# pdeljanov/Symphonia

Hardware: AMD Instinct MI355X
Metric: decoded audio frames/sec (batch IMDCT+OLA) (higher is better)
Workload: dtype f32

## Files before the change

### bindings/rust/symaccel_sys.rs

```rust
#![allow(non_camel_case_types, dead_code)]

#[repr(C)]
pub struct SymaccelCtx {
    _private: [u8; 0],
}

#[repr(C)]
pub struct SymaccelBatcher {
    _private: [u8; 0],
}

pub const SYMACCEL_OK: i32 = 0;
pub const SYMACCEL_ERR_INVALID_ARG: i32 = -1;
pub const SYMACCEL_ERR_UNSUPPORTED: i32 = -2;
pub const SYMACCEL_ERR_DEVICE: i32 = -3;
pub const SYMACCEL_ERR_OOM: i32 = -4;
pub const SYMACCEL_ERR_DECODE: i32 = -5;
pub const SYMACCEL_TABLE_AAC_KBD_LONG: u32 = 0;
pub const SYMACCEL_TABLE_AAC_KBD_SHORT: u32 = 1;
pub const SYMACCEL_TABLE_AAC_SINE_LONG: u32 = 2;
pub const SYMACCEL_TABLE_AAC_SINE_SHORT: u32 = 3;
pub const SYMACCEL_TABLE_MP3_SYNTH_D: u32 = 4;
pub const SYMACCEL_TABLE_MP3_IMDCT_WIN: u32 = 5;
pub const SYMACCEL_TABLE_VORBIS_FLOOR1_DB: u32 = 6;
// ... 334 lines not shown
    pub fn symaccel_vorbis_synth_fr_device(ctx: *mut SymaccelCtx, bs0_exp: i32, bs1_exp: i32, d_floor: *const f32, d_residue: *const f32, spec_stride: usize, d_block_flag: *const u8, d_prev_flag_io: *mut i32, d_overlap_io: *mut f32, d_pcm: *mut f32, pcm_stride: usize, n_chains: usize, blocks_per_chain: usize) -> i32;
    pub fn symaccel_vorbis_synth(ctx: *mut SymaccelCtx, bs0_exp: i32, bs1_exp: i32, h_spectra: *const f32, spec_stride: usize, h_block_flag: *const u8, h_prev_flag_io: *mut i32, h_overlap_io: *mut f32, h_pcm: *mut f32, pcm_stride: usize, n_chains: usize, blocks_per_chain: usize) -> i32;
    pub fn symaccel_vorbis_synth_pp_device(ctx: *mut SymaccelCtx, bs0_exp: i32, bs1_exp: i32, d_spectra: *const f32, d_residue: *const f32, spec_stride: usize, d_block_flag: *const u8, d_prev_flag_in: *const i32, d_prev_flag_out: *mut i32, d_overlap_in: *const f32, d_overlap_out: *mut f32, d_pcm: *mut f32, pcm_stride: usize, n_chains: usize, blocks_per_chain: usize) -> i32;
    pub fn symaccel_vorbis_synth_fy_pp_device(ctx: *mut SymaccelCtx, bs0_exp: i32, bs1_exp: i32, d_floor_y: *const u8, d_residue: *const f32, spec_stride: usize, d_block_flag: *const u8, d_prev_flag_in: *const i32, d_prev_flag_out: *mut i32, d_overlap_in: *const f32, d_overlap_out: *mut f32, d_pcm: *mut f32, pcm_stride: usize, n_chains: usize, blocks_per_chain: usize) -> i32;
    pub fn symaccel_vorbis_synth_fy_device(ctx: *mut SymaccelCtx, bs0_exp: i32, bs1_exp: i32, d_floor_y: *const u8, d_residue: *const f32, spec_stride: usize, d_block_flag: *const u8, d_prev_flag_io: *mut i32, d_overlap_io: *mut f32, d_pcm: *mut f32, pcm_stride: usize, n_chains: usize, blocks_per_chain: usize) -> i32;
    pub fn symaccel_vorbis_decode(ctx: *mut SymaccelCtx, bs0_exp: i32, bs1_exp: i32, h_residue: *const f32, spec_stride: usize, h_block_flag: *const u8, h_floor: *const u8, h_posts: *const u32, posts_stride: usize, h_floors: *const SymaccelVorbisFloor1Cfg, n_floors: usize, channels_per_stream: usize, h_coupling: *const u8, h_coupling_first: *const u32, h_prev_flag_io: *mut i32, h_overlap_io: *mut f32, h_pcm: *mut f32, pcm_stride: usize, n_chains: usize, blocks_per_chain: usize) -> i32;
    pub fn symaccel_vorbis_inverse_coupling_device(ctx: *mut SymaccelCtx, d_residue: *mut f32, n: usize, mag_index: *const u32, ang_index: *const u32, n_pairs: usize) -> i32;
    pub fn symaccel_vorbis_dot_product_device(ctx: *mut SymaccelCtx, d_floor: *mut f32, d_residue: *const f32, total: usize) -> i32;
    pub fn symaccel_vorbis_deinterleave2_device(ctx: *mut SymaccelCtx, d_type2: *const f32, d_planar: *mut f32, n_ch: i32, n2: usize, count: usize) -> i32;
    pub fn symaccel_vorbis_floor1_device(ctx: *mut SymaccelCtx, x_list: *const u32, n_posts: i32, multiplier: i32, d_y: *const u32, n: u32, d_floor: *mut f32, count: usize) -> i32;
    pub fn symaccel_vorbis_floor1_dot_device(ctx: *mut SymaccelCtx, x_list: *const u32, n_posts: i32, multiplier: i32, d_y: *const u32, n: u32, d_residue: *const f32, d_spectrum: *mut f32, count: usize) -> i32;
    pub fn symaccel_vorbis_floor1_dot_at_device(ctx: *mut SymaccelCtx, x_list: *const u32, n_posts: i32, multiplier: i32, d_y: *const u32, n: u32, d_line_offsets: *const u32, d_residue: *const f32, d_spectrum: *mut f32, count: usize) -> i32;
    pub fn symaccel_vorbis_floor1_y_device(ctx: *mut SymaccelCtx, x_list: *const u32, n_posts: i32, multiplier: i32, d_y: *const u32, n: u32, d_line_offsets: *const u32, d_floor_y: *mut u8, count: usize) -> i32;
    pub fn symaccel_vorbis_floor1_y_jobs_device(ctx: *mut SymaccelCtx, jobs: *const SymaccelVorbisFloor1Job, n_jobs: usize, d_floor_y: *mut u8) -> i32;
    pub fn symaccel_vorbis_floor1_status_device(ctx: *mut SymaccelCtx, n_posts: i32, d_y: *const u32, count: usize, d_status: *mut i8) -> i32;
    pub fn symaccel_host_vorbis_bark_map(n: u32, floor0_rate: u16, floor0_bark_map_size: u16, h_map: *mut i32) -> i32;
    pub fn symaccel_host_vorbis_floor0_coeffs(h_coeffs: *mut f32, order: i32) -> i32;
    pub fn symaccel_host_vorbis_floor0(h_coeffs: *const f32, order: i32, h_map: *const i32, n: u32, floor0_bark_map_size: u16, amplitude_bits: u8, amplitude_offset: u8, amplitude: u64, h_floor: *mut f32) -> i32;
    pub fn symaccel_flac_restore_device(ctx: *mut SymaccelCtx, d_buf: *mut i32, d_desc: *const SymaccelFlacDesc, d_coeffs: *const i32, n_blocks: usize, blocksize: usize) -> i32;
    pub fn symaccel_flac_restore(ctx: *mut SymaccelCtx, h_buf: *mut i32, h_desc: *const SymaccelFlacDesc, h_coeffs: *const i32, n_blocks: usize, blocksize: usize) -> i32;
    pub fn symaccel_flac_restore_pipelined(ctx: *mut SymaccelCtx, h_buf: *mut i32, h_desc: *const SymaccelFlacDesc, h_coeffs: *const i32, n_blocks: usize, blocksize: usize, chunk_blocks: usize) -> i32;
    pub fn symaccel_flac_block_status_device(ctx: *mut SymaccelCtx, d_desc: *const SymaccelFlacDesc, n_blocks: usize, blocksize: usize, d_status: *mut i8) -> i32;
    pub fn symaccel_flac_restore_stereo_device(ctx: *mut SymaccelCtx, d_buf: *mut i32, d_desc: *const SymaccelFlacDesc, d_coeffs: *const i32, d_pair_mode: *const u8, out_shift: u32, n_blocks: usize, blocksize: usize) -> i32;
    pub fn symaccel_flac_restore_strided_device(ctx: *mut SymaccelCtx, d_buf: *mut i32, d_desc: *const SymaccelFlacDesc, d_coeffs: *const i32, d_pair_mode: *const u8, out_shift: u32, n_blocks: usize, blocksize: usize, stride: usize) -> i32;
    pub fn symaccel_row_stride(blocksize: usize) -> usize;
    pub fn symaccel_flac_decorrelate_device(ctx: *mut SymaccelCtx, d_mode: *const u8, d_ch0: *mut i32, d_ch1: *mut i32, n_pairs: usize, blocksize: usize, out_shift: u32) -> i32;
    pub fn symaccel_flac_decorrelate(ctx: *mut SymaccelCtx, h_mode: *const u8, h_ch0: *mut i32, h_ch1: *mut i32, n_pairs: usize, blocksize: usize, out_shift: u32) -> i32;
    pub fn symaccel_md5_init(state: *mut SymaccelMd5State) -> i32;
    pub fn symaccel_md5_update(state: *mut SymaccelMd5State, bytes: *const core::ffi::c_void, n: usize) -> i32;
    pub fn symaccel_md5_digest(state: *const SymaccelMd5State, digest: *mut u8) -> i32;
    pub fn symaccel_flac_md5_device(ctx: *mut SymaccelCtx, d_jobs: *const SymaccelFlacMd5Job, n_jobs: usize) -> i32;
    pub fn symaccel_flac_md5_finish_device(ctx: *mut SymaccelCtx, d_jobs: *const SymaccelFlacMd5Job, n_jobs: usize, out_shift: u32) -> i32;
    pub fn symaccel_flac_md5(ctx: *mut SymaccelCtx, h_rows: *const i32, row_pitch: usize, h_frames: *const SymaccelFlacMd5Frame, n_frames: usize, nch: i32, bytes_per_sample: i32, h_state_io: *mut SymaccelMd5State, h_checkpoints: *mut SymaccelMd5State) -> i32;
    pub fn symaccel_alac_predict_device(ctx: *mut SymaccelCtx, d_buf: *mut i32, d_desc: *const SymaccelAlacDesc, d_coeffs: *const i32, n_blocks: usize, blocksize: usize) -> i32;
    pub fn symaccel_alac_predict(ctx: *mut SymaccelCtx, h_buf: *mut i32, h_desc: *const SymaccelAlacDesc, h_coeffs: *const i32, n_blocks: usize, blocksize: usize) -> i32;
    pub fn symaccel_alac_block_status_device(ctx: *mut SymaccelCtx, d_desc: *const SymaccelAlacDesc, n_blocks: usize, d_status: *mut i8) -> i32;
    pub fn symaccel_alac_predict_stereo_device(ctx: *mut SymaccelCtx, d_buf: *mut i32, d_desc: *const SymaccelAlacDesc, d_coeffs: *const i32, d_pair_weight: *const i32, d_pair_shift: *const u8, n_blocks: usize, blocksize: usize) -> i32;
    pub fn symaccel_alac_predict_strided_device(ctx: *mut SymaccelCtx, d_buf: *mut i32, d_desc: *const SymaccelAlacDesc, d_coeffs: *const i32, d_pair_weight: *const i32, d_pair_shift: *const u8, n_blocks: usize, blocksize: usize, stride: usize) -> i32;
    pub fn symaccel_alac_mid_side_device(ctx: *mut SymaccelCtx, d_weight: *const i32, d_shift: *const u8, d_ch0: *mut i32, d_ch1: *mut i32, n_pairs: usize, blocksize: usize) -> i32;
    pub fn symaccel_alac_mid_side(ctx: *mut SymaccelCtx, h_weight: *const i32, h_shift: *const u8, h_ch0: *mut i32, h_ch1: *mut i32, n_pairs: usize, blocksize: usize) -> i32;
    pub fn symaccel_sample_bytes(fmt: i32) -> usize;
    pub fn symaccel_pcm_convert_device(ctx: *mut SymaccelCtx, d_src: *const core::ffi::c_void, src_fmt: i32, plane_stride: usize, n_groups: usize, channels: usize, n_frames: usize, d_dst: *mut core::ffi::c_void, dst_fmt: i32, dst_group_bytes: usize) -> i32;
    pub fn symaccel_pcm_convert(ctx: *mut SymaccelCtx, h_src: *const core::ffi::c_void, src_fmt: i32, plane_stride: usize, n_groups: usize, channels: usize, n_frames: usize, h_dst: *mut core::ffi::c_void, dst_fmt: i32, dst_group_bytes: usize) -> i32;
    pub fn symaccel_adpcm_block_bytes(codec: i32, channels: usize, frames_per_block: usize) -> usize;
    pub fn symaccel_adpcm_decode_device(ctx: *mut SymaccelCtx, d_bytes: *const core::ffi::c_void, block_pitch: usize, n_blocks: usize, codec: i32, channels: usize, frames_per_block: usize, d_pcm: *mut core::ffi::c_void, out_fmt: i32, d_status: *mut u8) -> i32;
    pub fn symaccel_adpcm_decode(ctx: *mut SymaccelCtx, h_bytes: *const core::ffi::c_void, block_pitch: usize, n_blocks: usize, codec: i32, channels: usize, frames_per_block: usize, h_pcm: *mut core::ffi::c_void, out_fmt: i32, h_status: *mut u8) -> i32;
    pub fn symaccel_pcm_coded_bytes(codec: i32) -> usize;
    pub fn symaccel_pcm_native_bytes(codec: i32) -> usize;
    pub fn symaccel_pcm_decode_device(ctx: *mut SymaccelCtx, d_bytes: *const core::ffi::c_void, packet_pitch: usize, n_packets: usize, codec: i32, channels: usize, shift: u32, frames: usize, d_pcm: *mut core::ffi::c_void, out_fmt: i32) -> i32;
    pub fn symaccel_pcm_decode(ctx: *mut SymaccelCtx, h_bytes: *const core::ffi::c_void, packet_pitch: usize, n_packets: usize, codec: i32, channels: usize, shift: u32, frames: usize, h_pcm: *mut core::ffi::c_void, out_fmt: i32) -> i32;
    pub fn symaccel_batcher_create(ctx: *mut SymaccelCtx, flush_bytes: usize, out: *mut *mut SymaccelBatcher) -> i32;
    pub fn symaccel_batcher_destroy(b: *mut SymaccelBatcher) -> i32;
    pub fn symaccel_batcher_configure(b: *mut SymaccelBatcher, lanes: i32, hint_bytes: usize) -> i32;
    pub fn symaccel_batcher_last_error(b: *mut SymaccelBatcher, buf: *mut core::ffi::c_char, capacity: usize) -> i32;
    pub fn symaccel_batcher_reserve(b: *mut SymaccelBatcher, kind: i32, param: i32, n_chains: usize, units_per_chain: usize, slot: *mut SymaccelBatchSlot, ticket: *mut u64) -> i32;
    pub fn symaccel_batcher_commit(b: *mut SymaccelBatcher, ticket: u64) -> i32;
    pub fn symaccel_batcher_wait(b: *mut SymaccelBatcher, ticket: u64, slot: *mut SymaccelBatchSlot) -> i32;
    pub fn symaccel_batcher_release(b: *mut SymaccelBatcher, ticket: u64) -> i32;
    pub fn symaccel_batcher_submit(b: *mut SymaccelBatcher, kind: i32, param: i32, n_chains: usize, units_per_chain: usize, input: *mut *const core::ffi::c_void, state_io: *mut *mut core::ffi::c_void, out: *mut core::ffi::c_void, ticket: *mut u64) -> i32;
    pub fn symaccel_batcher_reserve_fmt(b: *mut SymaccelBatcher, kind: i32, param: i32, n_chains: usize, units_per_chain: usize, out_fmt: i32, channels: i32, slot: *mut SymaccelBatchSlot, ticket: *mut u64) -> i32;
    pub fn symaccel_batcher_submit_fmt(b: *mut SymaccelBatcher, kind: i32, param: i32, n_chains: usize, units_per_chain: usize, input: *mut *const core::ffi::c_void, state_io: *mut *mut core::ffi::c_void, out: *mut core::ffi::c_void, out_fmt: i32, channels: i32, ticket: *mut u64) -> i32;
    pub fn symaccel_batcher_reserve_io(b: *mut SymaccelBatcher, kind: i32, param: i32, n_chains: usize, units_per_chain: usize, in_fmt: i32, out_fmt: i32, channels: i32, slot: *mut SymaccelBatchSlot, ticket: *mut u64) -> i32;
    pub fn symaccel_batcher_submit_io(b: *mut SymaccelBatcher, kind: i32, param: i32, n_chains: usize, units_per_chain: usize, input: *mut *const core::ffi::c_void, state_io: *mut *mut core::ffi::c_void, out: *mut core::ffi::c_void, in_fmt: i32, out_fmt: i32, channels: i32, ticket: *mut u64) -> i32;
    pub fn symaccel_host_narrow_s16(src: *const i32, dst: *mut i16, n: usize) -> i32;
    pub fn symaccel_host_pack_row(src: *const i32, dst: *mut core::ffi::c_void, n: usize) -> i32;
    pub fn symaccel_batcher_submit_aac_synth(b: *mut SymaccelBatcher, coeffs: *const f32, side: *const u8, delay_io: *mut f32, pcm: *mut f32, n_chains: usize, frames_per_chain: usize, ticket: *mut u64) -> i32;
    pub fn symaccel_batcher_submit_mp3_synth(b: *mut SymaccelBatcher, xr: *const f32, side: *const SymaccelMp3Side, sample_rate_idx: i32, overlap_io: *mut f32, vvec_io: *mut f32, vfront_io: *mut i32, pcm: *mut f32, n_chains: usize, granules_per_chain: usize, ticket: *mut u64) -> i32;
    pub fn symaccel_batcher_submit_mp3_decode(b: *mut SymaccelBatcher, quant: *const i16, rq_desc: *const SymaccelMp3Requant, st_desc: *const SymaccelMp3Stereo, side: *const SymaccelMp3Side, sample_rate_idx: i32, overlap_io: *mut f32, vvec_io: *mut f32, vfront_io: *mut i32, pcm: *mut f32, n_chains: usize, granules_per_chain: usize, ticket: *mut u64) -> i32;
    pub fn symaccel_batcher_aac_bands(b: *mut SymaccelBatcher, swb_long: *const u16, n_swb_long: i32, swb_short: *const u16, n_swb_short: i32, bands: *mut i32) -> i32;
    pub fn symaccel_batcher_submit_aac_decode(b: *mut SymaccelBatcher, bands: i32, coeffs: *const f32, side: *const u8, pair_chains: *const i32, js_desc: *const SymaccelAacJsFrame, n_pairs: usize, tns: *const SymaccelAacTnsFilter, n_tns: usize, delay_io: *mut f32, pcm: *mut f32, n_chains: usize, frames_per_chain: usize, ticket: *mut u64) -> i32;
    pub fn symaccel_batcher_submit_vorbis_synth(b: *mut SymaccelBatcher, bs0_exp: i32, bs1_exp: i32, spectra: *const f32, block_flag: *const u8, prev_flag_io: *mut i32, overlap_io: *mut f32, pcm: *mut f32, n_chains: usize, blocks_per_chain: usize, ticket: *mut u64) -> i32;
    pub fn symaccel_batcher_vorbis_floor(b: *mut SymaccelBatcher, cfg: *const SymaccelVorbisFloor1Cfg, index: *mut i32) -> i32;
    pub fn symaccel_batcher_submit_vorbis_decode(b: *mut SymaccelBatcher, bs0_exp: i32, bs1_exp: i32, residue: *const f32, block_flag: *const u8, floor: *const u8, posts: *const u32, coupling: *const u8, coupling_first: *const u32, prev_flag_io: *mut i32, overlap_io: *mut f32, pcm: *mut f32, n_chains: usize, blocks_per_chain: usize, ticket: *mut u64) -> i32;
    pub fn symaccel_batcher_submit_flac_restore(b: *mut SymaccelBatcher, buf_io: *mut i32, desc: *const SymaccelFlacDesc, coeffs: *const i32, pair_mode: *const u8, out_shift: u32, n_blocks: usize, blocksize: usize, ticket: *mut u64) -> i32;
    pub fn symaccel_batcher_submit_flac_verify(b: *mut SymaccelBatcher, buf_io: *mut i32, desc: *const SymaccelFlacDesc, coeffs: *const i32, frames: *const SymaccelFlacMd5Frame, n_frames: usize, nch: i32, blocksize: usize, finish: i32, out_shift: u32, md5_states_io: *mut SymaccelMd5State, ticket: *mut u64) -> i32;
    pub fn symaccel_batcher_submit_alac_predict(b: *mut SymaccelBatcher, buf_io: *mut i32, desc: *const SymaccelAlacDesc, coeffs: *const i32, pair_weight: *const i32, pair_shift: *const u8, n_blocks: usize, blocksize: usize, ticket: *mut u64) -> i32;
    pub fn symaccel_batcher_submit_adpcm_decode(b: *mut SymaccelBatcher, bytes: *const u8, codec: i32, channels: usize, n_blocks: usize, block_bytes: usize, pcm: *mut i32, ticket: *mut u64) -> i32;
    pub fn symaccel_batcher_submit_pcm_decode(b: *mut SymaccelBatcher, bytes: *const u8, codec: i32, channels: usize, shift: u32, n_packets: usize, frames: usize, pcm: *mut core::ffi::c_void, ticket: *mut u64) -> i32;
    pub fn symaccel_batcher_collect(b: *mut SymaccelBatcher, ticket: u64) -> i32;
    pub fn symaccel_batcher_abandon(b: *mut SymaccelBatcher, ticket: u64) -> i32;
    pub fn symaccel_batcher_flush(b: *mut SymaccelBatcher) -> i32;
    pub fn symaccel_batcher_hint(b: *mut SymaccelBatcher) -> i32;
    pub fn symaccel_batcher_plane_bytes(kind: i32, param: i32, units_per_chain: usize, input_bytes: *mut usize, state_bytes: *mut usize, out_bytes: *mut usize) -> i32;
    pub fn symaccel_batcher_get_stats(b: *mut SymaccelBatcher, out: *mut SymaccelBatcherStats) -> i32;
    pub fn symaccel_shard_range(n_streams: usize, world: i32, rank: i32, first: *mut usize, count: *mut usize) -> i32;
    pub fn symaccel_scatter_streams(ctx: *mut SymaccelCtx, comm: *mut core::ffi::c_void, world: i32, rank: i32, root: i32, d_all: *const core::ffi::c_void, d_mine: *mut core::ffi::c_void, n_streams: usize, bytes_per_stream: usize) -> i32;
    pub fn symaccel_gather_streams(ctx: *mut SymaccelCtx, comm: *mut core::ffi::c_void, world: i32, rank: i32, root: i32, d_mine: *const core::ffi::c_void, d_all: *mut core::ffi::c_void, n_streams: usize, bytes_per_stream: usize) -> i32;
    pub fn symaccel_exchange_pipelined(ctx: *mut SymaccelCtx, comm: *mut core::ffi::c_void, world: i32, rank: i32, root: i32, d_all_in: *const core::ffi::c_void, d_mine_in: *mut core::ffi::c_void, in_bytes_per_stream: usize, d_all_out: *mut core::ffi::c_void, d_mine_out: *mut core::ffi::c_void, out_bytes_per_stream: usize, n_streams: usize, n_chunks: i32, step: SymaccelStepFn, user: *mut core::ffi::c_void) -> i32;
    pub fn symaccel_comm_unique_id(id: *mut SymaccelUniqueId) -> i32;
    pub fn symaccel_comm_init(ctx: *mut SymaccelCtx, id: *const SymaccelUniqueId, world: i32, rank: i32, comm: *mut *mut core::ffi::c_void) -> i32;
    pub fn symaccel_comm_destroy(comm: *mut core::ffi::c_void) -> i32;
    pub fn symaccel_multi_set_transport(transport: *const SymaccelTransport) -> i32;
    pub fn symaccel_probe_copy_device(ctx: *mut SymaccelCtx, d_src: *const core::ffi::c_void, d_dst: *mut core::ffi::c_void, bytes: usize, frames_per_wavefront: u32, flags: u32) -> i32;
    pub fn symaccel_table_f32(ctx: *const SymaccelCtx, table: i32, dst: *mut f32, capacity: usize) -> i32;
    pub fn symaccel_imdct_twiddles(n: i32, scale: f64, dst: *mut f32) -> i32;
    pub fn symaccel_fft_twiddles(n: i32, dst: *mut f32) -> i32;
}
```

### include/symaccel.h

```cpp
#ifndef SYMACCEL_H
#define SYMACCEL_H

#include <stddef.h>
#include <stdint.h>

#ifdef __cplusplus
extern "C" {
#endif

#define SYMACCEL_ABI_VERSION 8

typedef enum symaccel_status {
    SYMACCEL_OK = 0,
    SYMACCEL_ERR_INVALID_ARG = -1,
    SYMACCEL_ERR_UNSUPPORTED = -2,
    SYMACCEL_ERR_DEVICE = -3,
    SYMACCEL_ERR_OOM = -4,
    SYMACCEL_ERR_DECODE = -5,
} symaccel_status;

typedef struct symaccel_ctx symaccel_ctx;

int symaccel_abi_version(void);
const char *symaccel_strerror(int status);
// ... 418 lines not shown
size_t symaccel_pcm_native_bytes(int codec);
int symaccel_pcm_decode_device(symaccel_ctx *ctx, const void *d_bytes, size_t packet_pitch, size_t n_packets, int codec, size_t channels,
                               uint32_t shift, size_t frames, void *d_pcm, int out_fmt);
int symaccel_pcm_decode(symaccel_ctx *ctx, const void *h_bytes, size_t packet_pitch, size_t n_packets, int codec, size_t channels,
                        uint32_t shift, size_t frames, void *h_pcm, int out_fmt);

#define SYMACCEL_BATCH_AAC_SYNTH 1
#define SYMACCEL_BATCH_MP3_SYNTH 2
#define SYMACCEL_BATCH_MP3_DECODE 3
#define SYMACCEL_BATCH_VORBIS_SYNTH 4
#define SYMACCEL_BATCH_AAC_DECODE 5
#define SYMACCEL_BATCH_VORBIS_DECODE 6
#define SYMACCEL_BATCH_FLAC_RESTORE 7
#define SYMACCEL_BATCH_ALAC_PREDICT 8
#define SYMACCEL_BATCH_ADPCM_DECODE 9
#define SYMACCEL_BATCH_MPA12_DECODE 10
#define SYMACCEL_BATCH_PCM_DECODE 11
#define SYMACCEL_BATCH_MAX_INPUTS 6
typedef struct symaccel_batcher symaccel_batcher;
typedef struct symaccel_batch_slot {
    void *input[6];
    void *state[3];
    void *out;
    size_t input_bytes[6];
    size_t state_bytes[3];
    size_t out_bytes;
} symaccel_batch_slot;
typedef struct symaccel_batcher_stats {
    uint64_t submissions;
    uint64_t launches;
    uint64_t chunks;
    uint64_t chains_launched;
    uint64_t max_chains_per_launch;
    uint64_t staging_bytes;
    uint64_t pending;
    uint64_t failed_tickets;
    uint64_t lanes;
    uint64_t mutex_wait_ns;
    uint64_t mutex_contended;
    uint64_t launch_host_ns;
    uint64_t lane_wait_ns;
    uint64_t launch_api_ns;
    uint64_t group_allocs;
    uint64_t flag_wait_ns;
    uint64_t slots_peak;
    uint64_t blocks;
    uint64_t commit_to_launch_ns;
    uint64_t waits, waits_blocked;
    uint64_t launch_to_done_ns, launches_timed;
} symaccel_batcher_stats;
int symaccel_batcher_create(symaccel_ctx *ctx, size_t flush_bytes, symaccel_batcher **out);
int symaccel_batcher_destroy(symaccel_batcher *b);
int symaccel_batcher_configure(symaccel_batcher *b, int lanes, size_t hint_bytes);
int symaccel_batcher_last_error(symaccel_batcher *b, char *buf, size_t capacity);
int symaccel_batcher_reserve(symaccel_batcher *b, int kind, int param, size_t n_chains, size_t units_per_chain,
                             symaccel_batch_slot *slot, uint64_t *ticket);
int symaccel_batcher_commit(symaccel_batcher *b, uint64_t ticket);
int symaccel_batcher_wait(symaccel_batcher *b, uint64_t ticket, symaccel_batch_slot *slot);
int symaccel_batcher_release(symaccel_batcher *b, uint64_t ticket);
int symaccel_batcher_submit(symaccel_batcher *b, int kind, int param, size_t n_chains, size_t units_per_chain,
                            const void **input, void **state_io, void *out, uint64_t *ticket);
int symaccel_batcher_reserve_fmt(symaccel_batcher *b, int kind, int param, size_t n_chains, size_t units_per_chain, int out_fmt,
                                 int channels, symaccel_batch_slot *slot, uint64_t *ticket);
int symaccel_batcher_submit_fmt(symaccel_batcher *b, int kind, int param, size_t n_chains, size_t units_per_chain, const void **input,
                                void **state_io, void *out, int out_fmt, int channels, uint64_t *ticket);
#define SYMACCEL_IN_FMT_ROWS 32
int symaccel_batcher_reserve_io(symaccel_batcher *b, int kind, int param, size_t n_chains, size_t units_per_chain, int in_fmt, int out_fmt,
                                int channels, symaccel_batch_slot *slot, uint64_t *ticket);
int symaccel_batcher_submit_io(symaccel_batcher *b, int kind, int param, size_t n_chains, size_t units_per_chain, const void **input,
                               void **state_io, void *out, int in_fmt, int out_fmt, int channels, uint64_t *ticket);
int symaccel_host_narrow_s16(const int32_t *src, int16_t *dst, size_t n);
int symaccel_host_pack_row(const int32_t *src, void *dst, size_t n);
int symaccel_batcher_submit_aac_synth(symaccel_batcher *b, const float *coeffs, const uint8_t *side, float *delay_io, float *pcm,
                                      size_t n_chains, size_t frames_per_chain, uint64_t *ticket);
int symaccel_batcher_submit_mp3_synth(symaccel_batcher *b, const float *xr, const symaccel_mp3_side *side, int sample_rate_idx,
                                      float *overlap_io, float *vvec_io, int32_t *vfront_io, float *pcm, size_t n_chains,
                                      size_t granules_per_chain, uint64_t *ticket);
int symaccel_batcher_submit_mp3_decode(symaccel_batcher *b, const int16_t *quant, const symaccel_mp3_requant *rq_desc,
                                       const symaccel_mp3_stereo *st_desc, const symaccel_mp3_side *side, int sample_rate_idx,
                                       float *overlap_io, float *vvec_io, int32_t *vfront_io, float *pcm, size_t n_chains,
                                       size_t granules_per_chain, uint64_t *ticket);
int symaccel_batcher_aac_bands(symaccel_batcher *b, const uint16_t *swb_long, int n_swb_long, const uint16_t *swb_short, int n_swb_short,
                               int *bands);
int symaccel_batcher_submit_aac_decode(symaccel_batcher *b, int bands, const float *coeffs, const uint8_t *side,
                                       const int32_t *pair_chains, const symaccel_aac_js_frame *js_desc, size_t n_pairs,
                                       const symaccel_aac_tns_filter *tns, size_t n_tns, float *delay_io, float *pcm, size_t n_chains,
                                       size_t frames_per_chain, uint64_t *ticket);
int symaccel_batcher_submit_vorbis_synth(symaccel_batcher *b, int bs0_exp, int bs1_exp, const float *spectra, const uint8_t *block_flag,
                                         int32_t *prev_flag_io, float *overlap_io, float *pcm, size_t n_chains, size_t blocks_per_chain,
                                         uint64_t *ticket);
int symaccel_batcher_vorbis_floor(symaccel_batcher *b, const symaccel_vorbis_floor1_cfg *cfg, int *index);
int symaccel_batcher_submit_vorbis_decode(symaccel_batcher *b, int bs0_exp, int bs1_exp, const float *residue, const uint8_t *block_flag,
                                          const uint8_t *floor, const uint32_t *posts, const uint8_t *coupling,
                                          const uint32_t *coupling_first, int32_t *prev_flag_io, float *overlap_io, float *pcm,
                                          size_t n_chains, size_t blocks_per_chain, uint64_t *ticket);
int symaccel_batcher_submit_flac_restore(symaccel_batcher *b, int32_t *buf_io, const symaccel_flac_desc *desc, const int32_t *coeffs,
                                         const uint8_t *pair_mode, uint32_t out_shift, size_t n_blocks, size_t blocksize, uint64_t *ticket);
int symaccel_batcher_submit_flac_verify(symaccel_batcher *b, int32_t *buf_io, const symaccel_flac_desc *desc, const int32_t *coeffs,
                                        const symaccel_flac_md5_frame *frames, size_t n_frames, int nch, size_t blocksize, int finish,
                                        uint32_t out_shift, symaccel_md5_state *md5_states_io, uint64_t *ticket);
int symaccel_batcher_submit_alac_predict(symaccel_batcher *b, int32_t *buf_io, const symaccel_alac_desc *desc, const int32_t *coeffs,
                                         const int32_t *pair_weight, const uint8_t *pair_shift, size_t n_blocks, size_t blocksize,
                                         uint64_t *ticket);
int symaccel_batcher_submit_adpcm_decode(symaccel_batcher *b, const uint8_t *bytes, int codec, size_t channels, size_t n_blocks,
                                         size_t block_bytes, int32_t *pcm, uint64_t *ticket);
int symaccel_batcher_submit_pcm_decode(symaccel_batcher *b, const uint8_t *bytes, int codec, size_t channels, uint32_t shift,
// ... 64 lines not shown
```

### symphonia_amd/_ffi.py

```python
import ctypes as C
import json
import os
import sys
from pathlib import Path

import numpy as np

HERE = Path(__file__).resolve().parent
DEFAULT_SO = HERE / "libsymaccel.so"

OK = 0
ERR_INVALID_ARG = -1
ERR_UNSUPPORTED = -2
ERR_DEVICE = -3
ERR_OOM = -4
ERR_DECODE = -5

TABLE_AAC_KBD_LONG, TABLE_AAC_KBD_SHORT, TABLE_AAC_SINE_LONG, TABLE_AAC_SINE_SHORT = 0, 1, 2, 3
TABLE_MP3_SYNTH_D, TABLE_MP3_IMDCT_WIN, TABLE_VORBIS_FLOOR1_DB, TABLE_MP3_CONSTS = 4, 5, 6, 7
TABLE_MP3_POW43, TABLE_MP3_POW2AB, TABLE_MPA12 = 8, 9, 10

FMT_U8, FMT_S8, FMT_U16, FMT_S16, FMT_U24, FMT_S24, FMT_U32, FMT_S32, FMT_F32 = range(1, 10)
IN_FMT_ROWS = 32

ADPCM_MS, ADPCM_IMA_WAV, ADPCM_IMA_QT = 1, 2, 3

PCM_CODEC_NAMES = ("s32le", "s32be", "s24le", "s24be", "s16le", "s16be", "s8", "u32le", "u32be", "u24le", "u24be", "u16le", "u16be", "u8",
                   "f32le", "f32be", "f64le", "f64be", "alaw", "mulaw")
(PCM_S32LE, PCM_S32BE, PCM_S24LE, PCM_S24BE, PCM_S16LE, PCM_S16BE, PCM_S8, PCM_U32LE, PCM_U32BE, PCM_U24LE, PCM_U24BE, PCM_U16LE, PCM_U16BE,
 PCM_U8, PCM_F32LE, PCM_F32BE, PCM_F64LE, PCM_F64BE, PCM_ALAW, PCM_MULAW) = range(1, 21)

ABI_SYMBOLS = [
    "symaccel_abi_version", "symaccel_strerror", "symaccel_last_error", "symaccel_ctx_create",
    "symaccel_ctx_destroy", "symaccel_ctx_set_stream", "symaccel_sync", "symaccel_ctx_set_segment",
    "symaccel_fft_c32_device", "symaccel_fft_c32", "symaccel_ifft_c32_device", "symaccel_ifft_c32", "symaccel_imdct_f32_device", "symaccel_imdct_f32",
    "symaccel_aac_synth_device", "symaccel_aac_synth", "symaccel_aac_joint_stereo_device", "symaccel_aac_tns_device", "symaccel_mp3_synth_device", "symaccel_mp3_synth", "symaccel_mpa_polyphase_device", "symaccel_mpa_polyphase",
    "symaccel_mp3_requantize_device", "symaccel_mp3_requantize", "symaccel_mp3_stereo_device", "symaccel_mp3_requantize_stereo_device",
    "symaccel_vorbis_synth_device", "symaccel_vorbis_synth_fr_device", "symaccel_vorbis_synth", "symaccel_vorbis_inverse_coupling_device",
    "symaccel_vorbis_dot_product_device", "symaccel_vorbis_deinterleave2_device",
    "symaccel_vorbis_floor1_device", "symaccel_vorbis_floor1_dot_device", "symaccel_vorbis_floor1_y_device", "symaccel_vorbis_floor1_dot_at_device", "symaccel_vorbis_floor1_y_jobs_device",
    "symaccel_vorbis_synth_fy_pp_device", "symaccel_vorbis_synth_fy_device", "symaccel_flac_restore_device", "symaccel_flac_restore", "symaccel_flac_restore_stereo_device",
    "symaccel_flac_decorrelate_device", "symaccel_flac_decorrelate", "symaccel_alac_predict_device",
    "symaccel_alac_predict", "symaccel_alac_predict_stereo_device", "symaccel_alac_mid_side_device", "symaccel_alac_mid_side", "symaccel_table_f32", "symaccel_imdct_twiddles",
    "symaccel_fft_twiddles",
    "symaccel_host_alloc", "symaccel_host_free", "symaccel_host_register", "symaccel_host_unregister",
    "symaccel_aac_synth_pipelined", "symaccel_mp3_synth_pipelined", "symaccel_flac_restore_pipelined",
    "symaccel_host_aac_pulse", "symaccel_host_vorbis_bark_map", "symaccel_host_vorbis_floor0_coeffs", "symaccel_host_vorbis_floor0",
    "symaccel_flac_block_status_device", "symaccel_alac_block_status_device", "symaccel_vorbis_floor1_status_device", "symaccel_aac_tns_status_device",
    "symaccel_aac_synth_pp_device", "symaccel_aac_synth_js_pp_device", "symaccel_aac_synth_js_device", "symaccel_mp3_synth_pp_device", "symaccel_vorbis_synth_pp_device", "symaccel_mpa_polyphase_pp_device",
    "symaccel_probe_copy_device",
    "symaccel_shard_range", "symaccel_scatter_streams", "symaccel_gather_streams", "symaccel_exchange_pipelined", "symaccel_comm_unique_id", "symaccel_comm_init",
    "symaccel_comm_destroy", "symaccel_multi_set_transport", "symaccel_mp3_decode_pipelined",
    "symaccel_mp3_decode_pp_device", "symaccel_mp3_decode_device",
    "symaccel_aac_joint_stereo_list_device", "symaccel_aac_decode_pipelined", "symaccel_vorbis_decode",
    "symaccel_batcher_create", "symaccel_batcher_destroy", "symaccel_batcher_reserve", "symaccel_batcher_commit", "symaccel_batcher_wait",
    "symaccel_batcher_release", "symaccel_batcher_submit", "symaccel_batcher_collect", "symaccel_batcher_abandon",
    "symaccel_batcher_submit_aac_synth", "symaccel_batcher_submit_mp3_synth", "symaccel_batcher_submit_mp3_decode", "symaccel_batcher_submit_vorbis_synth", "symaccel_batcher_aac_bands", "symaccel_batcher_submit_aac_decode", "symaccel_batcher_flush", "symaccel_batcher_hint", "symaccel_batcher_plane_bytes",
    "symaccel_batcher_get_stats", "symaccel_batcher_configure", "symaccel_batcher_last_error", "symaccel_batcher_vorbis_floor",
    "symaccel_batcher_submit_vorbis_decode", "symaccel_batcher_submit_flac_restore", "symaccel_batcher_submit_alac_predict",
    "symaccel_flac_restore_strided_device", "symaccel_alac_predict_strided_device", "symaccel_row_stride",
    "symaccel_md5_init", "symaccel_md5_update", "symaccel_md5_digest", "symaccel_flac_md5_device", "symaccel_flac_md5",
    "symaccel_flac_md5_finish_device", "symaccel_batcher_submit_flac_verify",
    "symaccel_sample_bytes", "symaccel_pcm_convert_device", "symaccel_pcm_convert",
    "symaccel_batcher_reserve_fmt", "symaccel_batcher_submit_fmt",
    "symaccel_batcher_reserve_io", "symaccel_batcher_submit_io", "symaccel_host_narrow_s16", "symaccel_host_pack_row",
    "symaccel_adpcm_block_bytes", "symaccel_adpcm_decode_device", "symaccel_adpcm_decode",
    "symaccel_batcher_submit_adpcm_decode",
    "symaccel_pcm_coded_bytes", "symaccel_pcm_native_bytes", "symaccel_pcm_decode_device", "symaccel_pcm_decode",
    "symaccel_batcher_submit_pcm_decode",
    "symaccel_mpa12_record_bytes", "symaccel_mpa12_decode_device", "symaccel_mpa12_decode_pp_device", "symaccel_mpa12_decode",
]

_vp, _sz, _i, _d, _u32 = C.c_void_p, C.c_size_t, C.c_int, C.c_double, C.c_uint32


class VorbisFloor1Job(C.Structure):
    _fields_ = [("x_list", C.c_void_p), ("n_posts", C.c_int), ("multiplier", C.c_int), ("d_y", C.c_void_p), ("n", C.c_uint32),
                ("d_line_offsets", C.c_void_p), ("count", C.c_size_t)]


class SymaccelError(RuntimeError):
    def __init__(self, status, message):
        super().__init__("%s (status %d)" % (message, status))
        self.status = status


def _links_hip(path):
    try:
        return b"libamdhip64" in Path(path).read_bytes()
    except OSError:
        return False


class Library:
    def __init__(self, path=None):
        path = Path(path) if path is not None else DEFAULT_SO
        if not path.exists():
            raise FileNotFoundError(
                "%s is missing: build it with `python -m symphonia_amd.build` (hipcc, gfx950). "
                "symphonia_amd has no CPU fallback." % path)
        self.path = path
        self.torch_preload = None
        if "torch" not in sys.modules and not os.environ.get("SYMACCEL_NO_TORCH_PRELOAD") and _links_hip(path):
            import warnings
            try:
                import torch
                self.torch_preload = "imported torch before %s (one HIP runtime per process)" % path.name
            except Exception as e:
                self.torch_preload = "torch could not be imported before %s: %s: %s" % (path.name, type(e).__name__, e)
                warnings.warn("symphonia_amd: " + self.torch_preload)
            if os.environ.get("SYMACCEL_VERBOSE"):
# ... 2 lines not shown
        d = self.dll
        d.symaccel_strerror.restype = C.c_char_p
        d.symaccel_strerror.argtypes = [_i]
        d.symaccel_last_error.restype = C.c_char_p
        d.symaccel_last_error.argtypes = [_vp]
        d.symaccel_ctx_create.argtypes = [_i, C.POINTER(_vp)]
        d.symaccel_ctx_destroy.argtypes = [_vp]
        d.symaccel_ctx_destroy.restype = None
        d.symaccel_ctx_set_stream.argtypes = [_vp, _vp]
        d.symaccel_sync.argtypes = [_vp]
        d.symaccel_ctx_set_segment.argtypes = [_vp, _i]
        d.symaccel_fft_c32_device.argtypes = [_vp, _i, _vp, _vp, _sz]
        d.symaccel_fft_c32.argtypes = [_vp, _i, _vp, _vp, _sz]
        d.symaccel_ifft_c32_device.argtypes = [_vp, _i, _vp, _vp, _sz]
        d.symaccel_ifft_c32.argtypes = [_vp, _i, _vp, _vp, _sz]
        d.symaccel_flac_decorrelate.argtypes = [_vp, _vp, _vp, _vp, _sz, _sz, _u32]
        d.symaccel_imdct_f32_device.argtypes = [_vp, _i, _d, _vp, _vp, _sz]
        d.symaccel_imdct_f32.argtypes = [_vp, _i, _d, _vp, _vp, _sz]
        d.symaccel_aac_synth_device.argtypes = [_vp, _vp, _vp, _vp, _vp, _sz, _sz]
        d.symaccel_aac_synth.argtypes = [_vp, _vp, _vp, _vp, _vp, _sz, _sz]
        d.symaccel_mp3_synth_device.argtypes = [_vp, _vp, _vp, _i, _vp, _vp, _vp, _vp, _sz, _sz]
        d.symaccel_mp3_synth.argtypes = [_vp, _vp, _vp, _i, _vp, _vp, _vp, _vp, _sz, _sz]
        d.symaccel_mpa_polyphase_device.argtypes = [_vp, _i, _vp, _vp, _vp, _vp, _sz, _sz]
        d.symaccel_mpa_polyphase.argtypes = [_vp, _i, _vp, _vp, _vp, _vp, _sz, _sz]
        d.symaccel_aac_joint_stereo_device.argtypes = [_vp, _vp, _sz, _vp, _vp, _sz, _vp, _i, _vp, _i]
        d.symaccel_aac_tns_device.argtypes = [_vp, _vp, _sz, _vp, _sz]
        d.symaccel_aac_joint_stereo_list_device.argtypes = [_vp, _vp, _sz, _vp, _vp, _sz, _vp, _i, _vp, _i, _vp, _sz]
        d.symaccel_batcher_create.argtypes = [_vp, _sz, C.POINTER(_vp)]
        d.symaccel_batcher_destroy.argtypes = [_vp]
        d.symaccel_batcher_reserve.argtypes = [_vp, _i, _i, _sz, _sz, _vp, C.POINTER(C.c_uint64)]
        d.symaccel_batcher_commit.argtypes = [_vp, C.c_uint64]
        d.symaccel_batcher_wait.argtypes = [_vp, C.c_uint64, _vp]
        d.symaccel_batcher_release.argtypes = [_vp, C.c_uint64]
        d.symaccel_batcher_submit.argtypes = [_vp, _i, _i, _sz, _sz, _vp, _vp, _vp, C.POINTER(C.c_uint64)]
        d.symaccel_batcher_reserve_fmt.argtypes = [_vp, _i, _i, _sz, _sz, _i, _i, _vp, C.POINTER(C.c_uint64)]
        d.symaccel_batcher_submit_fmt.argtypes = [_vp, _i, _i, _sz, _sz, _vp, _vp, _vp, _i, _i, C.POINTER(C.c_uint64)]
        d.symaccel_batcher_reserve_io.argtypes = [_vp, _i, _i, _sz, _sz, _i, _i, _i, _vp, C.POINTER(C.c_uint64)]
        d.symaccel_batcher_submit_io.argtypes = [_vp, _i, _i, _sz, _sz, _vp, _vp, _vp, _i, _i, _i, C.POINTER(C.c_uint64)]
        d.symaccel_host_narrow_s16.argtypes = [_vp, _vp, _sz]
        d.symaccel_host_pack_row.argtypes = [_vp, _vp, _sz]
        d.symaccel_batcher_collect.argtypes = [_vp, C.c_uint64]
        d.symaccel_batcher_abandon.argtypes = [_vp, C.c_uint64]
        d.symaccel_batcher_submit_aac_synth.argtypes = [_vp, _vp, _vp, _vp, _vp, _sz, _sz, C.POINTER(C.c_uint64)]
        d.symaccel_batcher_submit_mp3_synth.argtypes = [_vp, _vp, _vp, _i, _vp, _vp, _vp, _vp, _sz, _sz, C.POINTER(C.c_uint64)]
        d.symaccel_batcher_submit_mp3_decode.argtypes = [_vp, _vp, _vp, _vp, _vp, _i, _vp, _vp, _vp, _vp, _sz, _sz, C.POINTER(C.c_uint64)]
        d.symaccel_batcher_flush.argtypes = [_vp]
        d.symaccel_batcher_hint.argtypes = [_vp]
        d.symaccel_batcher_plane_bytes.argtypes = [_i, _i, _sz, _vp, _vp, _vp]
        d.symaccel_batcher_aac_bands.argtypes = [_vp, _vp, _i, _vp, _i, C.POINTER(_i)]
        d.symaccel_batcher_submit_aac_decode.argtypes = [_vp, _i, _vp, _vp, _vp, _vp, _sz, _vp, _sz, _vp, _vp, _sz, _sz, C.POINTER(C.c_uint64)]
        d.symaccel_batcher_submit_vorbis_synth.argtypes = [_vp, _i, _i, _vp, _vp, _vp, _vp, _vp, _sz, _sz, C.POINTER(C.c_uint64)]
        d.symaccel_batcher_get_stats.argtypes = [_vp, _vp]
        d.symaccel_batcher_configure.argtypes = [_vp, _i, _sz]
        d.symaccel_batcher_last_error.argtypes = [_vp, _vp, _sz]
        d.symaccel_batcher_vorbis_floor.argtypes = [_vp, _vp, C.POINTER(_i)]
        d.symaccel_batcher_submit_vorbis_decode.argtypes = [_vp, _i, _i, _vp, _vp, _vp, _vp, _vp, _vp, _vp, _vp, _vp, _sz, _sz, C.POINTER(C.c_uint64)]
        d.symaccel_batcher_submit_flac_restore.argtypes = [_vp, _vp, _vp, _vp, _vp, _u32, _sz, _sz, C.POINTER(C.c_uint64)]
        d.symaccel_batcher_submit_alac_predict.argtypes = [_vp, _vp, _vp, _vp, _vp, _vp, _sz, _sz, C.POINTER(C.c_uint64)]
        d.symaccel_batcher_submit_adpcm_decode.argtypes = [_vp, _vp, _i, _sz, _sz, _sz, _vp, C.POINTER(C.c_uint64)]
        d.symaccel_batcher_submit_pcm_decode.argtypes = [_vp, _vp, _i, _sz, C.c_uint, _sz, _sz, _vp, C.POINTER(C.c_uint64)]
        d.symaccel_aac_decode_pipelined.argtypes = [_vp, _vp, _vp, _vp, _vp, _sz, _vp, _i, _vp, _i, _vp, _sz, _vp, _vp, _sz, _sz, _sz]
        d.symaccel_mp3_stereo_device.argtypes = [_vp, _vp, _sz, _vp, _vp, _i, _sz]
        d.symaccel_mp3_requantize_stereo_device.argtypes = [_vp, _vp, _vp, _sz, _vp, _vp, _i, _vp, _sz]
        d.symaccel_mp3_requantize_device.argtypes = [_vp, _vp, _vp, _i, _vp, _sz]
        d.symaccel_mp3_requantize.argtypes = [_vp, _vp, _vp, _i, _vp, _sz]
        d.symaccel_vorbis_synth_device.argtypes = [_vp, _i, _i, _vp, _sz, _vp, _vp, _vp, _vp, _sz, _sz, _sz]
        d.symaccel_vorbis_synth_fr_device.argtypes = [_vp, _i, _i, _vp, _vp, _sz, _vp, _vp, _vp, _vp, _sz, _sz, _sz]
        d.symaccel_vorbis_synth.argtypes = [_vp, _i, _i, _vp, _sz, _vp, _vp, _vp, _vp, _sz, _sz, _sz]
        d.symaccel_vorbis_decode.argtypes = [_vp, _i, _i, _vp, _sz, _vp, _vp, _vp, _sz, _vp, _sz, _sz, _vp, _vp, _vp, _vp, _vp, _sz, _sz, _sz]
        d.symaccel_vorbis_inverse_coupling_device.argtypes = [_vp, _vp, _sz, _vp, _vp, _sz]
        d.symaccel_vorbis_dot_product_device.argtypes = [_vp, _vp, _vp, _sz]
        d.symaccel_vorbis_deinterleave2_device.argtypes = [_vp, _vp, _vp, _i, _sz, _sz]
        d.symaccel_vorbis_floor1_device.argtypes = [_vp, _vp, _i, _i, _vp, _u32, _vp, _sz]
        d.symaccel_vorbis_floor1_dot_device.argtypes = [_vp, _vp, _i, _i, _vp, C.c_uint32, _vp, _vp, _sz]
        d.symaccel_vorbis_floor1_y_device.argtypes = [_vp, _vp, _i, _i, _vp, C.c_uint32, _vp, _vp, _sz]
        d.symaccel_vorbis_floor1_y_jobs_device.argtypes = [_vp, _vp, _sz, _vp]
        d.symaccel_vorbis_floor1_dot_at_device.argtypes = [_vp, _vp, _i, _i, _vp, C.c_uint32, _vp, _vp, _vp, _sz]
        d.symaccel_vorbis_synth_fy_pp_device.argtypes = [_vp, _i, _i, _vp, _vp, _sz, _vp, _vp, _vp, _vp, _vp, _vp, _sz, _sz, _sz]
        d.symaccel_vorbis_synth_fy_device.argtypes = [_vp, _i, _i, _vp, _vp, _sz, _vp, _vp, _vp, _vp, _sz, _sz, _sz]
        d.symaccel_flac_restore_device.argtypes = [_vp, _vp, _vp, _vp, _sz, _sz]
        d.symaccel_flac_restore_stereo_device.argtypes = [_vp, _vp, _vp, _vp, _vp, _u32, _sz, _sz]
        d.symaccel_flac_restore_strided_device.argtypes = [_vp, _vp, _vp, _vp, _vp, _u32, _sz, _sz, _sz]
        d.symaccel_alac_predict_strided_device.argtypes = [_vp, _vp, _vp, _vp, _vp, _vp, _sz, _sz, _sz]
        d.symaccel_row_stride.argtypes = [_sz]
        d.symaccel_row_stride.restype = _sz
        d.symaccel_flac_restore.argtypes = [_vp, _vp, _vp, _vp, _sz, _sz]
        d.symaccel_flac_decorrelate_device.argtypes = [_vp, _vp, _vp, _vp, _sz, _sz, _u32]
        d.symaccel_alac_predict_device.argtypes = [_vp, _vp, _vp, _vp, _sz, _sz]
        d.symaccel_alac_predict_stereo_device.argtypes = [_vp, _vp, _vp, _vp, _vp, _vp, _sz, _sz]
        d.symaccel_alac_predict.argtypes = [_vp, _vp, _vp, _vp, _sz, _sz]
        d.symaccel_mp3_decode_pipelined.argtypes = [_vp, _vp, _vp, _vp, _vp, _sz, _vp, _i, _vp, _vp, _vp, _vp, _sz, _sz, _sz]
        d.symaccel_mp3_decode_pp_device.argtypes = [_vp, _vp, _vp, _vp, _vp, _sz, _vp, _i, _vp, _vp, _vp, _vp, _vp, _vp, _vp, _sz, _sz]
        d.symaccel_mp3_decode_device.argtypes = [_vp, _vp, _vp, _vp, _vp, _sz, _vp, _i, _vp, _vp, _vp, _vp, _sz, _sz]
        d.symaccel_shard_range.argtypes = [_sz, _i, _i, C.POINTER(_sz), C.POINTER(_sz)]
        d.symaccel_scatter_streams.argtypes = [_vp, _vp, _i, _i, _i, _vp, _vp, _sz, _sz]
        d.symaccel_gather_streams.argtypes = [_vp, _vp, _i, _i, _i, _vp, _vp, _sz, _sz]
        d.symaccel_exchange_pipelined.argtypes = [_vp, _vp, _i, _i, _i, _vp, _vp, _sz, _vp, _vp, _sz, _sz, _i, _vp, _vp]
        d.symaccel_comm_unique_id.argtypes = [_vp]
        d.symaccel_comm_init.argtypes = [_vp, _vp, _i, _i, C.POINTER(_vp)]
        d.symaccel_comm_destroy.argtypes = [_vp]
        d.symaccel_multi_set_transport.argtypes = [_vp]
        d.symaccel_probe_copy_device.argtypes = [_vp, _vp, _vp, _sz, _u32, _u32]
        d.symaccel_alac_mid_side_device.argtypes = [_vp, _vp, _vp, _vp, _vp, _sz, _sz]
        d.symaccel_alac_mid_side.argtypes = [_vp, _vp, _vp, _vp, _vp, _sz, _sz]
        d.symaccel_aac_synth_pp_device.argtypes = [_vp, _vp, _vp, _vp, _vp, _vp, _sz, _sz]
        d.symaccel_aac_synth_js_pp_device.argtypes = [_vp, _vp, _vp, _vp, _vp, _sz, _vp, _i, _vp, _i, _vp, _vp, _vp, _sz, _sz]
# ... 90 lines not shown
```

### symphonia_amd/backend.py

```python
import ctypes as C

import numpy as np

from . import _ffi
from ._ffi import SymaccelError


def _is_torch(x):
    return type(x).__module__.startswith("torch")


def _ptr(x):
    if x is None:
        return None
    if _is_torch(x):
        return x.data_ptr()
    return x.ctypes.data


def _np(a, dtype):
    return np.ascontiguousarray(a, dtype=dtype)


class Context:
# ... 937 lines not shown

    def __del__(self):
        try:
            self.close()
        except Exception:
            pass

    def _check(self, st):
        return self.ctx.lib.check(st, self.ctx.handle)

    def submit(self, kind, param, inputs, states, out, out_format=0, channels=0, n_chains=None, units=None, in_fmt=0):
        shaped = out if not out_format else inputs[0]
        n_chains, units = int(shaped.shape[0] if n_chains is None else n_chains), int(shaped.shape[1] if units is None else units)
        ins = (C.c_void_p * 6)(*[a.ctypes.data if a is not None else None for a in list(inputs) + [None] * (6 - len(inputs))])
        sts = (C.c_void_p * 3)(*[a.ctypes.data for a in list(states)] + [None] * (3 - len(states)))
        for a in list(inputs) + list(states) + [out]:
            assert a is None or a.flags["C_CONTIGUOUS"]
        t = C.c_uint64()
        if in_fmt:
            self._check(self.dll.symaccel_batcher_submit_io(self.handle, int(kind), int(param), n_chains, units, ins, sts, out.ctypes.data,
                                                            input_format(in_fmt), sample_format(out_format) if out_format else 0, int(channels), C.byref(t)))
        elif out_format:
            self._check(self.dll.symaccel_batcher_submit_fmt(self.handle, int(kind), int(param), n_chains, units, ins, sts, out.ctypes.data,
                                                             sample_format(out_format), int(channels), C.byref(t)))
        else:
            self._check(self.dll.symaccel_batcher_submit(self.handle, int(kind), int(param), n_chains, units, ins, sts, out.ctypes.data, C.byref(t)))
        return int(t.value)

    def collect(self, ticket):
        self._check(self.dll.symaccel_batcher_collect(self.handle, int(ticket)))

    def aac_bands(self, swb_long, swb_short):
        lo, sh = np.ascontiguousarray(swb_long, np.uint16), np.ascontiguousarray(swb_short, np.uint16)
        out = C.c_int(-1)
        self._check(self.dll.symaccel_batcher_aac_bands(self.handle, lo.ctypes.data, len(lo) - 1, sh.ctypes.data, len(sh) - 1, C.byref(out)))
        return int(out.value)

    def submit_aac_decode(self, bands, coeffs, side, pairs, js_desc, tns, delay_io, pcm):
        n_chains, frames = int(coeffs.shape[0]), int(coeffs.shape[1])
        n_pairs = 0 if pairs is None else len(pairs)
        n_tns = 0 if tns is None else len(tns)
        keep = [np.ascontiguousarray(pairs, np.int32) if n_pairs else None, np.ascontiguousarray(js_desc) if n_pairs else None,
                np.ascontiguousarray(tns) if n_tns else None]
        t = C.c_uint64()
        self._check(self.dll.symaccel_batcher_submit_aac_decode(
            self.handle, int(bands), coeffs.ctypes.data, side.ctypes.data, keep[0].ctypes.data if n_pairs else None,
            keep[1].ctypes.data if n_pairs else None, n_pairs, keep[2].ctypes.data if n_tns else None, n_tns, delay_io.ctypes.data,
            pcm.ctypes.data, n_chains, frames, C.byref(t)))
        return int(t.value)

    def configure(self, lanes=0, hint_bytes=0):
        self._check(self.dll.symaccel_batcher_configure(self.handle, int(lanes), int(hint_bytes)))

    def last_error(self):
        buf = C.create_string_buffer(512)
        self._check(self.dll.symaccel_batcher_last_error(self.handle, buf, 512))
        return buf.value.decode(errors="replace")

    def vorbis_floor(self, multiplier, x_list):
        cfg = np.zeros(1, VORBIS_FLOOR1_DTYPE)
        cfg["multiplier"], cfg["n_posts"] = int(multiplier), len(x_list)
        cfg["x_list"][0, :len(x_list)] = np.asarray(x_list, np.uint32)
        out = C.c_int(-1)
        self._check(self.dll.symaccel_batcher_vorbis_floor(self.handle, cfg.ctypes.data, C.byref(out)))
        return int(out.value)

    def submit_vorbis_decode(self, bs0_exp, bs1_exp, residue, flags, floor, posts, coupling, coupling_first, prev_flag_io, overlap_io, pcm):
        n_chains, blocks = int(flags.shape[0]), int(flags.shape[1])
        for a in (residue, flags, floor, posts, coupling_first, prev_flag_io, overlap_io, pcm):
            assert a.flags["C_CONTIGUOUS"]
        keep = np.ascontiguousarray(coupling, np.uint8) if coupling is not None and len(coupling) else None
        t = C.c_uint64()
        self._check(self.dll.symaccel_batcher_submit_vorbis_decode(
            self.handle, int(bs0_exp), int(bs1_exp), residue.ctypes.data, flags.ctypes.data, floor.ctypes.data, posts.ctypes.data,
            keep.ctypes.data if keep is not None else None, coupling_first.ctypes.data, prev_flag_io.ctypes.data, overlap_io.ctypes.data,
            pcm.ctypes.data, n_chains, blocks, C.byref(t)))
        return int(t.value)

    def submit_flac_restore(self, buf_io, desc, coeffs, pair_mode=None, out_shift=0):
        n_blocks, blocksize = int(buf_io.shape[0]), int(buf_io.shape[1])
        for a in (buf_io, desc, coeffs):
            assert a.flags["C_CONTIGUOUS"]
        t = C.c_uint64()
        self._check(self.dll.symaccel_batcher_submit_flac_restore(
            self.handle, buf_io.ctypes.data, desc.ctypes.data, coeffs.ctypes.data, pair_mode.ctypes.data if pair_mode is not None else None,
            int(out_shift), n_blocks, blocksize, C.byref(t)))
        return int(t.value)

    def submit_flac_verify(self, buf_io, desc, coeffs, frames, nch, states_io, finish=False, out_shift=0):
        n_blocks, blocksize = int(buf_io.shape[0]), int(buf_io.shape[1])
        assert frames.dtype == FLAC_MD5_FRAME_DTYPE and states_io.dtype == MD5_STATE_DTYPE and len(states_io) == len(frames)
        assert n_blocks == len(frames) * int(nch)
        for a in (buf_io, desc, coeffs, frames, states_io):
            assert a.flags["C_CONTIGUOUS"]
        t = C.c_uint64()
        self._check(self.dll.symaccel_batcher_submit_flac_verify(
            self.handle, buf_io.ctypes.data, desc.ctypes.data, coeffs.ctypes.data, frames.ctypes.data, len(frames), int(nch), blocksize,
            int(bool(finish)), int(out_shift), states_io.ctypes.data, C.byref(t)))
        return int(t.value)

    def submit_alac_predict(self, buf_io, desc, coeffs, pair_weight=None, pair_shift=None):
        n_blocks, blocksize = int(buf_io.shape[0]), int(buf_io.shape[1])
        for a in (buf_io, desc, coeffs):
            assert a.flags["C_CONTIGUOUS"]
        t = C.c_uint64()
        self._check(self.dll.symaccel_batcher_submit_alac_predict(
# ... 72 lines not shown
```

### symphonia_amd/csrc/aac.hip

```cpp
#include <type_traits>

#include "imdct_wave.h"

namespace symaccel {

namespace {

#ifndef SYM_AAC_VARIANT
#define SYM_AAC_VARIANT 0
#endif
#if SYM_AAC_VARIANT == 1
constexpr int kWaves = 6;
#define SYM_AAC_WAVES_PER_SIMD 3
#else
constexpr int kWaves = 4;
#endif
constexpr int kTabTw = 0;
constexpr int kTabKbd = 1024;
constexpr int kTabSine = 2048;
constexpr int kTabKbdShort = 3072;
constexpr int kTabSineShort = 3200;
constexpr int kTabFloats = 3328;

enum : int { ONLY_LONG = 0, LONG_START = 1, EIGHT_SHORT = 2, LONG_STOP = 3 };
constexpr int kP0 = 512 - 64;
constexpr int kP1 = 512 + 64;

__device__ __forceinline__ void pcm_short4(const float *H, int q0, const float *short_win, const float *prev_short_win,
                                           float (&acc)[4]) {
    const int w = q0 >> 7, i0 = q0 & 127;
    bool have = false;
    if (w >= 1) {
        float a[4];
        ys4(H, w - 1, 128 + i0, a);
        const float4 wr = *reinterpret_cast<const float4 *>(short_win + 124 - i0);
        a[0] *= wr.w; a[1] *= wr.z; a[2] *= wr.y; a[3] *= wr.x;
#pragma unroll
        for (int q = 0; q < 4; ++q) acc[q] = (w - 1 == 0) ? a[q] : (0.0f + a[q]);
        have = true;
    }
    if (w <= 7) {
        float bq[4];
        ys4(H, w, i0, bq);
        const float4 wf = *reinterpret_cast<const float4 *>((w == 0 ? prev_short_win : short_win) + i0);
        bq[0] *= wf.x; bq[1] *= wf.y; bq[2] *= wf.z; bq[3] *= wf.w;
#pragma unroll
        for (int q = 0; q < 4; ++q) acc[q] = have ? (acc[q] + bq[q]) : bq[q];
    }
}

__device__ __forceinline__ void stop_window4(const float *psw, int j0, float *w) {
    float4 v = make_float4(1.0f, 1.0f, 1.0f, 1.0f);
    if (j0 >= kP0 && j0 < kP1) v = *reinterpret_cast<const float4 *>(psw + j0 - kP0);
    w[0] = v.x; w[1] = v.y; w[2] = v.z; w[3] = v.w;
}
__device__ __forceinline__ void start_window4(const float *sw, int j0, float *w) {
    float4 v = make_float4(1.0f, 1.0f, 1.0f, 1.0f);
    if (j0 >= kP0 && j0 < kP1) {
        const float4 r = *reinterpret_cast<const float4 *>(sw + 124 - (j0 - kP0));
        v = make_float4(r.w, r.z, r.y, r.x);
    }
    w[0] = v.x; w[1] = v.y; w[2] = v.z; w[3] = v.w;
}

#if defined(SYM_AAC_WAVES_PER_SIMD) && !defined(SYM_AAC_MIN_WAVES)
#define SYM_AAC_MIN_WAVES SYM_AAC_WAVES_PER_SIMD
#endif
#ifndef SYM_AAC_MIN_WAVES
#define SYM_AAC_MIN_WAVES 2
#endif
#ifndef SYM_AAC_PREFETCH
#define SYM_AAC_PREFETCH 1
#endif
#ifndef SYM_AAC_QUAD
#define SYM_AAC_QUAD 1
#endif
__device__ __forceinline__ float2 ld_line(const float2 *p) { return ld_stream(p); }
__device__ __forceinline__ void st_slot(float *frame, int m2, const float (&v)[8]) {
    float4 *o4 = reinterpret_cast<float4 *>(frame);
    st_stream(o4 + m2, make_float4(v[0], v[1], v[2], v[3]));
    st_stream(o4 + 255 - m2, make_float4(v[4], v[5], v[6], v[7]));
}


#if !SYM_AAC_QUAD
#include "experiments/aac_wave_walk.h"
#endif



constexpr int kSlotOff = kShortRowsEnd;
static_assert(kSlotOff + 1024 <= kWaveLds, "delay slot must fit the per-wave LDS behind the short-window rows");

enum : int { kStepHalo = 0, kStepFull = 1, kStepRagged = 2 };
template <int V> using step_kind = std::integral_constant<int, V>;

__device__ __forceinline__ void settle_prefetch(const float2 (&line)[8]) {
#if defined(__HIP_DEVICE_COMPILE__)
    __builtin_amdgcn_sched_barrier(0);
    asm volatile("" : : "v"(line[0].x), "v"(line[0].y), "v"(line[1].x), "v"(line[1].y), "v"(line[2].x), "v"(line[2].y), "v"(line[3].x), "v"(line[3].y),
                        "v"(line[4].x), "v"(line[4].y), "v"(line[5].x), "v"(line[5].y), "v"(line[6].x), "v"(line[6].y), "v"(line[7].x), "v"(line[7].y));
#endif
}

struct AacJsArgs {
    const int2 *chain;
    const int32_t *pair_chains;
    const symaccel_aac_js_frame *desc;
    AacBandMaps maps;
    unsigned n_chains;
};

#if SYM_AAC_QUAD == 2
#include "experiments/aac_quad_probe.h"
#endif

template <bool JS>
__global__ __launch_bounds__(256, SYM_AAC_MIN_WAVES) void aac_synth_quad_kernel(
    DevTables tb, const float *__restrict__ coeffs, const uint8_t *__restrict__ side,
    const float *__restrict__ delay_in, float *__restrict__ delay_out, float *__restrict__ pcm,
    unsigned frames_per_chain, unsigned seg_steps, unsigned segs_per_chain, AacJsArgs js) {
    __shared__ __attribute__((aligned(16))) float tabs[kTabFloats];
    __shared__ __attribute__((aligned(16))) float wave_lds[4][kWaveLds];
    constexpr int CH = JS ? 2 : 1;
    __shared__ __attribute__((aligned(16))) float carry[CH][2][1024];
    if constexpr (!JS) {
        if (js.chain && js.chain[blockIdx.x / segs_per_chain].x >= 0) return;
    }
    for (int i = (int)threadIdx.x; i < 1024; i += 256) {
        tabs[kTabTw + i] = reinterpret_cast<const float *>(tb.aac_tw_long)[i];
        tabs[kTabKbd + i] = tb.aac_kbd_long[i];
        tabs[kTabSine + i] = tb.aac_sine_long[i];
        if (i < 128) {
            tabs[kTabKbdShort + i] = tb.aac_kbd_short[i];
            tabs[kTabSineShort + i] = tb.aac_sine_short[i];
        }
    }
    const int lane = (int)threadIdx.x & 63, wave = __builtin_amdgcn_readfirstlane((int)threadIdx.x >> 6);
    float *ldsf = wave_lds[wave];
    c32 *lds = reinterpret_cast<c32 *>(ldsf);
    const c32 *tw = reinterpret_cast<const c32 *>(tabs + kTabTw);
    const unsigned unit = blockIdx.x / segs_per_chain, seg = blockIdx.x % segs_per_chain;
    const unsigned chain = JS ? (unsigned)js.pair_chains[2 * unit] : unit, chain1 = JS ? (unsigned)js.pair_chains[2 * unit + 1] : unit;
    if constexpr (JS) {
        if (chain >= js.n_chains || chain1 >= js.n_chains || chain == chain1) return;
    }
    const long t_begin = (long)seg * seg_steps * 4;
    const long t_end = t_begin + (long)seg_steps * 4 < (long)frames_per_chain ? t_begin + (long)seg_steps * 4 : (long)frames_per_chain;
    if (t_end <= t_begin) return;
    const size_t chain_base0 = (size_t)chain * frames_per_chain, chain_base1 = (size_t)chain1 * frames_per_chain;
    LaneTables lt;
    load_lane_tables(tb, lane, lt);

    const bool has_halo = t_begin > 0;
    if (!has_halo && wave == 3) {
#pragma unroll
        for (int ch = 0; ch < CH; ++ch) {
            const float4 *src = reinterpret_cast<const float4 *>(delay_in + (size_t)(ch ? chain1 : chain) * 1024);
#pragma unroll
            for (int q = 0; q < 4; ++q) reinterpret_cast<float4 *>(carry[ch][1])[lane + 64 * q] = src[lane + 64 * q];
        }
    }
    const long t_first = (wave == 3 && has_halo) ? t_begin - 1 : t_begin + wave;
    float2 line[8];
    unsigned sb_next = 0;
    float2 line1[8];
    uint32_t dq[3] = {0u, 0u, 0u};
    unsigned sb1_next = 0;
    uint32_t sfb_long[2] = {0u, 0u};
    unsigned sfb_short = 0;
    auto fetch1 = [&](long tf, int ln) {
        if constexpr (JS) {
            const float2 *ps = reinterpret_cast<const float2 *>(coeffs + (chain_base1 + (size_t)tf) * 1024);
            const uint32_t *d = reinterpret_cast<const uint32_t *>(js.desc + (size_t)unit * frames_per_chain + (size_t)tf);
#pragma unroll
            for (int s = 0; s < 8; ++s) line1[s] = ld_line(ps + ln + 64 * s);
            dq[0] = d[ln];
            dq[1] = d[ln + 64];
            dq[2] = ln < 33 ? d[ln + 128] : 0u;
            sb1_next = side[chain_base1 + (size_t)tf];
        }
    };
    if constexpr (JS) {
#pragma unroll
        for (int s = 0; s < 8; ++s) sfb_long[s >> 2] |= (uint32_t)js.maps.long4[(lane >> 1) + 32 * s] << (8 * (s & 3));
        sfb_short = js.maps.short4[(lane >> 1) & 31];
    }
    if (t_first < t_end) {
        const float2 *src = reinterpret_cast<const float2 *>(coeffs + (chain_base0 + (size_t)t_first) * 1024);
#pragma unroll
        for (int s = 0; s < 8; ++s) line[s] = ld_line(src + lane + 64 * s);
        sb_next = side[chain_base0 + (size_t)t_first];
        fetch1(t_first, lane);
    } else {
#pragma unroll
        for (int s = 0; s < 8; ++s) line[s] = make_float2(0.0f, 0.0f);
        if constexpr (JS) {
#pragma unroll
            for (int s = 0; s < 8; ++s) line1[s] = make_float2(0.0f, 0.0f);
        }
    }
    __syncthreads();

    const int lane_of_wave = lane;
    auto step = [&](auto kind_c, int i, long t, bool active) __attribute__((always_inline)) {
        constexpr int KIND = decltype(kind_c)::value;
        int lane = lane_of_wave;
        if constexpr (JS) {
#if defined(__HIP_DEVICE_COMPILE__)
            asm volatile("" : "+v"(lane));
#endif
        }
        const unsigned sb0 = (unsigned)__builtin_amdgcn_readfirstlane((int)sb_next);
        const unsigned sb1 = JS ? (unsigned)__builtin_amdgcn_readfirstlane((int)sb1_next) : 0u;
        if constexpr (JS) {
            if (active) {
                uint32_t *dl = reinterpret_cast<uint32_t *>(ldsf);
                dl[lane] = dq[0];
                dl[lane + 64] = dq[1];
                if (lane < 33) dl[lane + 128] = dq[2];
                wave_sync();
                const unsigned hdr = dl[0];
                const bool one = (hdr & 255u) == 1u;
                const int max_sfb = (int)((hdr >> 8) & 255u);
                const uint8_t *mode = reinterpret_cast<const uint8_t *>(dl + 1);
                const float *scale = reinterpret_cast<const float *>(dl + 33);
#pragma unroll
                for (int s = 0; s < 8; ++s) {
                    const float2 l = line[s], r = line1[s];
                    const int sfb = one ? (int)((sfb_long[s >> 2] >> (8 * (s & 3))) & 255u) : (int)sfb_short;
                    const int slot = one ? sfb : 16 * s + sfb;
                    const bool coded = sfb < max_sfb && slot < 128;
                    const int sl = slot < 127 ? slot : 127;
                    const unsigned m = mode[sl];
                    const float sc = scale[sl];
                    const bool ms = coded && m == SYMACCEL_AAC_JS_MS, is = coded && m == SYMACCEL_AAC_JS_INTENSITY;
                    line[s] = ms ? make_float2(l.x + r.x, l.y + r.y) : l;
                    line1[s] = ms ? make_float2(l.x - r.x, l.y - r.y) : (is ? make_float2(sc * l.x, sc * l.y) : r);
                }
                wave_sync();
            }
        }
        const long tn = KIND == kStepHalo ? t_begin + 3 : (t + 4 < t_end ? t + 4 : t);
        const bool fetch = KIND == kStepFull || (KIND == kStepHalo && tn < t_end);
#pragma unroll 1
        for (int ch = 0; ch < CH; ++ch) {
        if constexpr (JS) {
#if defined(__HIP_DEVICE_COMPILE__)
            asm volatile("" : "+v"(lane));
#endif
        }
        const unsigned sb = ch ? sb1 : sb0;
        const size_t chain_base = ch ? chain_base1 : chain_base0;
        const int seq = (int)(sb & 3u);
        const int shape = (int)((sb >> 2) & 1u), prev_shape = (int)((sb >> 3) & 1u);
        float *my_slot = wave == 3 ? carry[ch][i & 1] : ldsf + kSlotOff;
        float *prev_slot = wave == 0 ? carry[ch][(i + 1) & 1] : wave_lds[wave > 0 ? wave - 1 : 0] + kSlotOff;
        float xw[2][8];
        auto ln_at = [&](int s) -> float2 {
            if constexpr (JS) return ch ? line1[s] : line[s];
            else return line[s];
        };
        auto long_tail = [&](auto seq_c) __attribute__((always_inline)) {
            constexpr int SEQ = decltype(seq_c)::value;
            const float *wprev = tabs + (prev_shape ? kTabKbd : kTabSine);
            const float *wcur = tabs + (shape ? kTabKbd : kTabSine);
#pragma unroll
            for (int h = 0; h < 2; ++h) {
                const int m2 = lane + 64 * h;
                float x[8], x2[8];
                post_slot(lds, tw, m2, x, x2);
                float wo[8];
                if constexpr (SEQ == LONG_STOP) {
                    const float *psw = tabs + (prev_shape ? kTabKbdShort : kTabSineShort);
                    stop_window4(psw, 4 * m2, wo);
                    stop_window4(psw, 1020 - 4 * m2, wo + 4);
                } else {
                    load_slot(wprev, m2, wo);
                }
#pragma unroll
                for (int q = 0; q < 8; ++q) xw[h][q] = x[q] * wo[q];
                float wd[8], nd[8];
                if constexpr (SEQ == LONG_START) {
                    const float *sw = tabs + (shape ? kTabKbdShort : kTabSineShort);
                    start_window4(sw, 4 * m2, wd);
                    start_window4(sw, 1020 - 4 * m2, wd + 4);
                } else {
                    float wr[8];
                    if (SEQ == ONLY_LONG && shape == prev_shape) {
#pragma unroll
                        for (int q = 0; q < 8; ++q) wr[q] = wo[q];
                    } else {
                        load_slot(wcur, m2, wr);
                    }
#pragma unroll
                    for (int q = 0; q < 8; ++q) wd[q] = wr[7 - q];
                }
#pragma unroll
                for (int q = 0; q < 8; ++q) {
                    const int j = q < 4 ? 4 * m2 + q : 1020 - 4 * m2 + (q - 4);
                    const float v = x2[q] * wd[q];
                    nd[q] = (SEQ == LONG_START && j >= kP1) ? 0.0f : v;
                }
                store_slot(my_slot, m2, nd);
            }
        };

        if (active) {
            c32 z[8];
            if (seq != EIGHT_SHORT) {
                const int mirror = (63 - lane) * 4;
#pragma unroll
                for (int s = 0; s < 8; ++s) {
                    const float mirrored = __int_as_float(__builtin_amdgcn_ds_bpermute(mirror, __float_as_int(ln_at(7 - s).y)));
                    z[s] = pre_twiddle(ln_at(s).x, mirrored, tw[lane + 64 * s]);
                }
            } else {
#pragma unroll
                for (int s = 0; s < 8; ++s) {
                    ldsf[short_row(s) + 2 * lane] = ln_at(s).x;
                    ldsf[short_row(s) + 2 * lane + 1] = ln_at(s).y;
                }
                wave_sync();
            }
            if (fetch) {
                if (ch == 0) {
                    sb_next = side[chain_base0 + (size_t)tn];
                    const float2 *src = reinterpret_cast<const float2 *>(coeffs + (chain_base0 + (size_t)tn) * 1024);
#pragma unroll
                    for (int s = 0; s < 8; ++s) line[s] = ld_line(src + lane + 64 * s);
                }
                if (ch == CH - 1) fetch1(tn, lane);
            }
            if (seq != EIGHT_SHORT) {
                fft512_wave(z, lane, lds, lt);
                if (seq == ONLY_LONG) long_tail(step_kind<ONLY_LONG>{});
                else if (seq == LONG_START) long_tail(step_kind<LONG_START>{});
                else long_tail(step_kind<LONG_STOP>{});
            } else {
                imdct_short_wave(lane, ldsf, tb.aac_tw_short, lt);
                const float *sw = tabs + (shape ? kTabKbdShort : kTabSineShort);
                const float *psw = tabs + (prev_shape ? kTabKbdShort : kTabSineShort);
#pragma unroll 1
                for (int e = 0; e < 4; ++e) {
                    const int j0 = 4 * lane + 256 * e;
                    float nd[4] = {0.0f, 0.0f, 0.0f, 0.0f};
                    if (j0 < kP1) pcm_short4(ldsf, j0 + kP1, sw, psw, nd);
                    *reinterpret_cast<float4 *>(my_slot + j0) = make_float4(nd[0], nd[1], nd[2], nd[3]);
                }
            }
        }
        if constexpr (KIND == kStepHalo) {
            wave_sync();
        } else {
        wg_sync_lds();

        if (active) {
            float *frame_out = pcm + (chain_base + (size_t)t) * 1024;
            float dst[2][8];
            if (seq != EIGHT_SHORT) {
#pragma unroll
                for (int h = 0; h < 2; ++h) {
                    const int m2 = lane + 64 * h;
                    float dl[8];
                    load_slot(prev_slot, m2, dl);
#pragma unroll
                    for (int q = 0; q < 8; ++q) dst[h][q] = dl[q] + xw[h][q];
                    if (seq == LONG_STOP) {
#pragma unroll
                        for (int q = 0; q < 8; ++q) {
                            const int j = q < 4 ? 4 * m2 + q : 1020 - 4 * m2 + (q - 4);
                            dst[h][q] = j < kP0 ? dl[q] : dst[h][q];
                        }
                    }
                }
            } else {
                const float *sw = tabs + (shape ? kTabKbdShort : kTabSineShort);
                const float *psw = tabs + (prev_shape ? kTabKbdShort : kTabSineShort);
#pragma unroll 1
                for (int e = 0; e < 4; ++e) {
                    const int j0 = 4 * lane + 256 * e;
                    const float4 d = *reinterpret_cast<const float4 *>(prev_slot + j0);
                    float o[4] = {d.x, d.y, d.z, d.w};
                    if (j0 >= kP0) {
                        float ps[4];
                        pcm_short4(ldsf, j0 - kP0, sw, psw, ps);
#pragma unroll
                        for (int q = 0; q < 4; ++q) o[q] = o[q] + ps[q];
                    }
                    *reinterpret_cast<float4 *>(prev_slot + j0) = make_float4(o[0], o[1], o[2], o[3]);
                }
                wave_sync();
#pragma unroll
                for (int h = 0; h < 2; ++h) load_slot(prev_slot, lane + 64 * h, dst[h]);
            }
#pragma unroll
            for (int h = 0; h < 2; ++h) st_slot(frame_out, lane + 64 * h, dst[h]);
            if constexpr (KIND == kStepFull && !JS) settle_prefetch(line);
            if (t + 1 == (long)frames_per_chain) {
                float4 *d = reinterpret_cast<float4 *>(delay_out + (size_t)(ch ? chain1 : chain) * 1024);
#pragma unroll
                for (int q = 0; q < 4; ++q) d[lane + 64 * q] = reinterpret_cast<const float4 *>(my_slot)[lane + 64 * q];
            }
        }
        wg_sync_lds();
        }
        }
    };

    if (has_halo && wave == 3) step(step_kind<kStepHalo>{}, -1, t_begin - 1, true);
    if constexpr (!JS) settle_prefetch(line);
    const int n_full = (int)((t_end - t_begin) >> 2);
    long t = t_begin + wave;
#pragma unroll 1
    for (int i = 0; i < n_full; ++i, t += 4) step(step_kind<kStepFull>{}, i, t, true);
    if ((t_end - t_begin) & 3) step(step_kind<kStepRagged>{}, n_full, t, t < t_end);
}

__global__ void aac_js_index_kernel(const int32_t *__restrict__ pair_chains, unsigned n_pairs, unsigned n_chains, int2 *__restrict__ chain_index) {
    const unsigned i = blockIdx.x * blockDim.x + threadIdx.x;
    if (i < 2 * n_pairs && (unsigned)pair_chains[i] < n_chains && (unsigned)pair_chains[i ^ 1u] < n_chains)
        chain_index[pair_chains[i]] = make_int2(pair_chains[i ^ 1u], (int)i);
}

}

int launch_aac(symaccel_ctx *ctx, const float *d_coeffs, const uint8_t *d_side, const float *d_delay_in,
               float *d_delay_out, float *d_pcm, size_t n_chains, size_t frames_per_chain, const AacBandMaps *maps,
               const int32_t *d_pair_chains, const symaccel_aac_js_frame *d_js_desc, size_t n_pairs, void *d_js_scratch) {
    if (frames_per_chain > 0x7fffffffu) return SYMACCEL_ERR_INVALID_ARG;
#if SYM_AAC_QUAD
    {
        const size_t steps_per_chain = (frames_per_chain + 3) / 4;
        unsigned seg_steps;
        if (ctx->segment > 0) seg_steps = (unsigned)((ctx->segment + 3) / 4);
        else seg_steps = choose_segment(ctx, n_chains, steps_per_chain, SYM_AAC_MIN_WAVES, 1, 1, 1);
        if (seg_steps > steps_per_chain) seg_steps = (unsigned)steps_per_chain;
        const size_t segs = (steps_per_chain + seg_steps - 1) / seg_steps;
        const size_t grid = n_chains * segs;
        if (grid > 0x7fffffffu) return SYMACCEL_ERR_INVALID_ARG;
        AacJsArgs js{nullptr, nullptr, nullptr, AacBandMaps{}, (unsigned)n_chains};
        if (n_pairs == 0 || !maps) {
            hipLaunchKernelGGL(aac_synth_quad_kernel<false>, dim3((unsigned)grid), dim3(256), 0, ctx->stream, ctx->dev, d_coeffs, d_side,
                               d_delay_in, d_delay_out, d_pcm, (unsigned)frames_per_chain, seg_steps, (unsigned)segs, js);
        } else {
            if (n_pairs * frames_per_chain > 0x7fffffffu) return SYMACCEL_ERR_INVALID_ARG;
            const bool unpaired = 2 * n_pairs < n_chains;
            int2 *chain_index = unpaired ? reinterpret_cast<int2 *>(d_js_scratch) : nullptr;
            if (unpaired) {
                SYM_GPU(ctx, hipMemsetAsync(chain_index, 0xff, n_chains * sizeof(int2), ctx->stream));
                hipLaunchKernelGGL(aac_js_index_kernel, dim3((unsigned)((2 * n_pairs + 255) / 256)), dim3(256), 0, ctx->stream, d_pair_chains,
                                   (unsigned)n_pairs, (unsigned)n_chains, chain_index);
                SYM_GPU(ctx, hipGetLastError());
            }
            js = AacJsArgs{chain_index, d_pair_chains, d_js_desc, *maps, (unsigned)n_chains};
            unsigned pseg_steps;
            if (ctx->segment > 0) pseg_steps = (unsigned)((ctx->segment + 3) / 4);
            else pseg_steps = choose_segment(ctx, n_pairs, steps_per_chain, SYM_AAC_MIN_WAVES, 1, 1, 1);
            if (pseg_steps > steps_per_chain) pseg_steps = (unsigned)steps_per_chain;
            const size_t psegs = (steps_per_chain + pseg_steps - 1) / pseg_steps;
            if (n_pairs * psegs > 0x7fffffffu) return SYMACCEL_ERR_INVALID_ARG;
            hipLaunchKernelGGL(aac_synth_quad_kernel<true>, dim3((unsigned)(n_pairs * psegs)), dim3(256), 0, ctx->stream, ctx->dev, d_coeffs, d_side,
                               d_delay_in, d_delay_out, d_pcm, (unsigned)frames_per_chain, pseg_steps, (unsigned)psegs, js);
            SYM_GPU(ctx, hipGetLastError());
            if (unpaired)
                hipLaunchKernelGGL(aac_synth_quad_kernel<false>, dim3((unsigned)grid), dim3(256), 0, ctx->stream, ctx->dev, d_coeffs, d_side,
                                   d_delay_in, d_delay_out, d_pcm, (unsigned)frames_per_chain, seg_steps, (unsigned)segs, js);
        }
        SYM_GPU(ctx, hipGetLastError());
// ... 9 lines not shown
```

### symphonia_amd/csrc/batch_copy.hip

```cpp
#include <hip/hip_runtime.h>

#include <algorithm>
#include <cstdlib>

#include "pcm_convert.h"
#include "symaccel_internal.h"

namespace symaccel {

namespace {

template <bool NT>
__device__ __forceinline__ void batch_copy_piece(const BatchCopyDesc d, const unsigned tid) {
    const uintptr_t s = reinterpret_cast<uintptr_t>(d.src), t = reinterpret_cast<uintptr_t>(d.dst);
    if (((s | t | d.bytes) & 15u) == 0) {
        const uint4 *src = reinterpret_cast<const uint4 *>(d.src);
        uint4 *dst = reinterpret_cast<uint4 *>(d.dst);
        const unsigned n = d.bytes / 16u;
        uint4 v[4];
#pragma unroll
        for (int k = 0; k < 4; ++k)
            if (tid + 256u * k < n) {
                if constexpr (NT) {
                    const unsigned *p = reinterpret_cast<const unsigned *>(src + tid + 256u * k);
// ... 236 lines not shown
    a.tile_frames = pcm_tile_frames((unsigned)channels, pcm_sample_bytes(dst_fmt));
    a.n_groups = n_groups;
    a.tiles_per_group = (n_frames + a.tile_frames - 1) / a.tile_frames;
    const size_t cap = (size_t)ctx->n_cus * 8, gx = std::min(a.tiles_per_group, cap);
    const dim3 grid((unsigned)gx, (unsigned)std::min<size_t>(n_groups, std::max<size_t>(1, cap / gx)));
    if (src_fmt == SYMACCEL_FMT_F32) pcm_convert_launch<SYMACCEL_FMT_F32>(dst_fmt, grid, stream, a);
    else pcm_convert_launch<SYMACCEL_FMT_S32>(dst_fmt, grid, stream, a);
    SYM_GPU(ctx, hipGetLastError());
    return SYMACCEL_OK;
}

namespace {

__global__ void batch_flag_kernel(unsigned long long *flag, unsigned long long seq) {
    __builtin_amdgcn_fence(__ATOMIC_RELEASE, "");
    __atomic_store_n(flag, seq, __ATOMIC_RELAXED);
}

}

int launch_batch_flag(symaccel_ctx *ctx, hipStream_t stream, uint64_t *h_flag, uint64_t seq) {
    hipLaunchKernelGGL(batch_flag_kernel, dim3(1), dim3(1), 0, stream, reinterpret_cast<unsigned long long *>(h_flag), (unsigned long long)seq);
    SYM_GPU(ctx, hipGetLastError());
    return SYMACCEL_OK;
}

int launch_batch_copy(symaccel_ctx *ctx, hipStream_t stream, const BatchCopyDesc *descs, size_t n, bool scatter, size_t pcm_plane_stride, bool widening) {
    if (n == 0) return SYMACCEL_OK;
    if (n > 0x7fffffffu) return SYMACCEL_ERR_INVALID_ARG;
    static const unsigned caps[2] = {
        [] { const char *e = std::getenv("SYMACCEL_BATCH_COPY_WGS_G"); if (!e) e = std::getenv("SYMACCEL_BATCH_COPY_WGS"); return e ? (unsigned)std::atoi(e) : 64u; }(),
        [] { const char *e = std::getenv("SYMACCEL_BATCH_COPY_WGS_S"); if (!e) e = std::getenv("SYMACCEL_BATCH_COPY_WGS"); return e ? (unsigned)std::atoi(e) : 64u; }()};
    const unsigned cap = caps[scatter ? 1 : 0];
    const unsigned grid = cap ? (unsigned)std::min<size_t>(n, cap) : (unsigned)n;
    static const bool nt = [] {
        const char *e = std::getenv("SYMACCEL_BATCH_COPY_NT");
        return e && std::atoi(e) != 0;
    }();
    if (pcm_plane_stride) hipLaunchKernelGGL(batch_scatter_convert_kernel, dim3(grid), dim3(256), 0, stream, descs, (unsigned)n, pcm_plane_stride);
    else if (widening && !scatter) hipLaunchKernelGGL(batch_gather_widen_kernel, dim3(grid), dim3(256), 0, stream, descs, (unsigned)n);
    else if (nt && scatter) hipLaunchKernelGGL((batch_copy_kernel<true, 1>), dim3(grid), dim3(256), 0, stream, descs, (unsigned)n);
    else if (nt) hipLaunchKernelGGL((batch_copy_kernel<true, 0>), dim3(grid), dim3(256), 0, stream, descs, (unsigned)n);
    else if (scatter) hipLaunchKernelGGL((batch_copy_kernel<false, 1>), dim3(grid), dim3(256), 0, stream, descs, (unsigned)n);
    else hipLaunchKernelGGL((batch_copy_kernel<false, 0>), dim3(grid), dim3(256), 0, stream, descs, (unsigned)n);
    SYM_GPU(ctx, hipGetLastError());
    return SYMACCEL_OK;
}

}

#include "adpcm.hip"

#include "pcm_decode.hip"
```

### symphonia_amd/csrc/batcher.cpp

```cpp
#include <algorithm>
#include <chrono>
#include <condition_variable>
#include <cstdlib>
#include <cstring>
#include <memory>
#include <mutex>
#include <thread>
#include <vector>

#include "batcher_lists.h"

using namespace symaccel;
using namespace symaccel::batch;

namespace {

bool plane_sizes(int kind, int param, size_t units, PlaneSizes *ps) {
    *ps = PlaneSizes();
    switch (kind) {
    case SYMACCEL_BATCH_AAC_SYNTH:
    case SYMACCEL_BATCH_AAC_DECODE:
        ps->n_in = 2;
        ps->in[0] = units * 4096;
        ps->in[1] = units;
// ... 154 lines not shown
    l.bytes = off;
    return l;
}

size_t slot_class(size_t bytes) {
    if (bytes <= 4096) return 4096;
    size_t top = (size_t)1 << (63 - __builtin_clzll((unsigned long long)bytes));
    const size_t step = top >> 3;
    return (bytes + step - 1) & ~(step - 1);
}

struct Group;
using Clock = std::chrono::steady_clock;

struct Ticket {
    Group *group = nullptr;
    uint32_t gen = 0;
    uint32_t first_chain = 0, n_chains = 0;
    bool live = false, committed = false;
    Clock::time_point committed_at{};
    int status = SYMACCEL_OK;
    char *slot = nullptr;
    size_t slot_bytes = 0;
    void *user_state[kMaxState] = {nullptr, nullptr, nullptr};
    void *user_out = nullptr;
    int out_fmt = 0;
    uint32_t channels = 0;
    size_t out_valid = 0;
    int in_fmt = 0;
};

enum class GroupState { Free, Open, Closed, Launching, Launched };

struct Lane;

struct Block {
    char *d_base = nullptr;
    size_t d_bytes = 0;
    char *h_desc = nullptr;
    size_t h_desc_bytes = 0;
    hipEvent_t ev_in[2] = {nullptr, nullptr}, ev_k[2] = {nullptr, nullptr};
    uint64_t *h_flag = nullptr;
    uint64_t seq = 0;
    Group *owner = nullptr;
};

inline uint64_t read_flag(const uint64_t *flag) { return __atomic_load_n(flag, __ATOMIC_ACQUIRE); }

struct LaunchKnobs {
    bool row_pad = true;
    size_t dma_bytes = 0;
    size_t chunk_div = 2;
    size_t chunk_min = (size_t)8192 << 10;
};

struct Group {
    int kind = 0, param = 0;
    size_t units = 0;
    PlaneSizes ps;
    size_t cap_chains = 0;
    size_t chains = 0, tickets = 0, uncommitted = 0, live = 0;
    Clock::time_point launched_at{};
    GroupState state = GroupState::Free;
    int status = SYMACCEL_OK;
    std::vector<uint32_t> ticket_ids;
    std::vector<TicketView> views;
    Lane *lane = nullptr;
    Block *block = nullptr;
    bool completed = false;
    const uint64_t *done_flag = nullptr;
    uint64_t done_seq = 0;
    char *d_in[kMaxIn] = {}, *d_state_in[kMaxState] = {}, *d_state_out[kMaxState] = {}, *d_out = nullptr;
    size_t row_pitch = 0;
    LaunchKnobs knobs;
    std::vector<VorbisUsed> used;
    Mp3Lists mp3;
    AacLists aac;
    VorbisLists vb;
    FlacVerifyLists fv;
};

struct Lane {
    symaccel_ctx *ctx = nullptr;
    bool owned = false;
    std::mutex mu;
};

inline uint64_t ns_since(Clock::time_point t0) { return (uint64_t)std::chrono::duration_cast<std::chrono::nanoseconds>(Clock::now() - t0).count(); }

}

struct symaccel_batcher {
    symaccel_ctx *ctx = nullptr;
    size_t flush_bytes = 0;
    std::mutex mu;
    std::condition_variable cv;
    std::vector<std::unique_ptr<Group>> groups;
    std::vector<Ticket> tickets;
    std::vector<uint32_t> free_tickets;
    symaccel_batcher_stats stats{};
    std::string last_error;
    LaunchKnobs knobs;
    size_t hint_bytes = 0;
    size_t busy_groups = 4, busy_hint_bytes = (size_t)48 << 20;
    std::vector<std::unique_ptr<Lane>> lanes;
    size_t want_lanes = 2, next_lane = 0;
    std::vector<std::unique_ptr<Block>> blocks;
    struct Slab {
        char *base;
        size_t bytes, used;
    };
    std::vector<Slab> slabs;
    uint64_t slots_live = 0;
    bool growing = false;
    std::vector<std::pair<size_t, std::vector<char *>>> free_slots;
    struct Bands {
        std::vector<uint16_t> swb_long, swb_short;
        AacBandMaps maps;
    };
    std::vector<Bands> bands;
    std::vector<symaccel_vorbis_floor1_cfg> floors;
};

namespace {

// ... 87 lines not shown
        if (w[c] < 2 || w[c] > 4) return false;
    return true;
}

int check_flac(size_t units, int param, const TicketView &v) {
    if (!row_widths_ok(v)) return SYMACCEL_ERR_INVALID_ARG;
    const FlacVerifyParam vp = flac_verify_param(param);
    if (vp.verify) {
        const symaccel_flac_md5_frame *fr = v.in<const symaccel_flac_md5_frame>(3);
        for (size_t f = 0; f < v.n_chains / vp.nch; ++f)
            if (fr[f].block_len > units || fr[f].pair_mode > 3 || (fr[f].pair_mode != 0 && vp.nch != 2) || fr[f].bytes_per_sample < 1 || fr[f].bytes_per_sample > 4)
                return SYMACCEL_ERR_INVALID_ARG;
    }
    const symaccel_flac_desc *d = v.in<const symaccel_flac_desc>(1);
    for (size_t c = 0; c < v.n_chains; ++c) {
        if (d[c].kind > SYMACCEL_FLAC_LPC || d[c].order > units || d[c].shift > 31 || d[c].wasted_bits > 31) return SYMACCEL_ERR_INVALID_ARG;
        if (d[c].kind == SYMACCEL_FLAC_FIXED && d[c].order > 4) return SYMACCEL_ERR_INVALID_ARG;
        if (d[c].kind == SYMACCEL_FLAC_LPC && (d[c].order < 1 || d[c].order > 32)) return SYMACCEL_ERR_INVALID_ARG;
    }
    if (pair_param(param).pairs) {
        const uint8_t *pm = v.in<const uint8_t>(3);
        for (size_t p = 0; p < v.n_chains / 2; ++p)
            if (pm[p] > 3) return SYMACCEL_ERR_INVALID_ARG;
    }
    return SYMACCEL_OK;
}

int check_alac(int param, const TicketView &v) {
    if (!row_widths_ok(v)) return SYMACCEL_ERR_INVALID_ARG;
    const symaccel_alac_desc *d = v.in<const symaccel_alac_desc>(1);
    for (size_t c = 0; c < v.n_chains; ++c) {
        if (d[c].mode > 0 && d[c].mode < 15) return SYMACCEL_ERR_DECODE;
        if (d[c].lpc_order > 31 || d[c].shift > 31 || d[c].bps < 1 || d[c].bps > 32) return SYMACCEL_ERR_INVALID_ARG;
    }
    if (pair_param(param).pairs) {
        const uint8_t *sh = v.in<const uint8_t>(4);
        for (size_t p = 0; p < v.n_chains / 2; ++p)
            if (sh[p] > 31) return SYMACCEL_ERR_INVALID_ARG;
    }
    return SYMACCEL_OK;
}

int check_adpcm(size_t units, int param, const TicketView &v) {
    const AdpcmParam ap = adpcm_param(param);
    const uint8_t *b = v.in<const uint8_t>(0);
    for (size_t c = 0; c < v.n_chains; ++c, b += units)
        for (int k = 0; k < ap.nch; ++k) {
            if (ap.codec == SYMACCEL_ADPCM_MS && b[k] > 6) return SYMACCEL_ERR_UNSUPPORTED;
            if (ap.codec == SYMACCEL_ADPCM_IMA_WAV && b[4 * k + 2] > 88) return SYMACCEL_ERR_DECODE;
        }
    return SYMACCEL_OK;
}

int check_mpa12(size_t units, int param, TicketView &v) {
    const size_t rb = symaccel_mpa12_record_bytes(param);
    uint8_t *r = v.in<uint8_t>(1);
    bool bad = false;
    for (size_t k = 0; k < v.n_chains * units && !bad; ++k, r += rb)
        for (size_t i = 0; i < rb && !bad; ++i)
            bad = i >= 32 ? r[i] > 63 : (param == SYMACCEL_MPA_LAYER1 ? r[i] == 1 || r[i] > 15 : r[i] > (uint8_t)kMpa12Classes);
    if (!bad) return SYMACCEL_OK;
    std::memset(v.slot + v.lay.in[1], 0, v.lay.in_bytes[1]);
    return SYMACCEL_ERR_INVALID_ARG;
}

void prepare_views(Group *g) {
    const PlaneSizes &ps = g->ps;
    const VorbisParam vp = vorbis_param(g->param, g->units);
    if (vorbis_kind(g->kind)) g->used.resize(g->chains);
    for (TicketView &v : g->views) {
        v.lay = slot_layout(ps, v.n_chains);
        if (vorbis_kind(g->kind)) {
            VorbisUsed *used = g->used.data() + v.first_chain;
            for (size_t c = 0; c < v.n_chains; ++c) used[c] = vorbis_used(v.in<const uint8_t>(1) + c * g->units, g->units, v.state<const int32_t>(0)[c], vp.e0, vp.e1);
            v.used = used;
        }
        if (!v.out_fmt) continue;
        const size_t fb = (size_t)v.channels * symaccel_sample_bytes(v.out_fmt);
        v.out_valid = (v.n_chains / v.channels) * (ps.out_per_chain() / 4) * fb;
        if (!vorbis_kind(g->kind)) continue;
        v.out_valid = 0;
        for (size_t c = 0; c < v.n_chains; ++c) {
            if (c % v.channels == 0) v.out_valid += v.used[c].samples * fb;
            else if (v.used[c].samples != v.used[c - c % v.channels].samples) v.fmt_status = SYMACCEL_ERR_INVALID_ARG;
        }
        if (v.fmt_status != SYMACCEL_OK) std::memset(v.slot + v.lay.in[0], 0, v.lay.in_bytes[0]);
    }
}

void validate_and_count(Group *g) {
    if (g->kind == SYMACCEL_BATCH_AAC_DECODE) g->aac.count(g->views, g->ps, g->units, g->param);
    if (g->kind == SYMACCEL_BATCH_VORBIS_DECODE) g->vb.count(g->views, g->ps, g->units, g->chains);
    for (TicketView &v : g->views) {
        if (g->kind == SYMACCEL_BATCH_FLAC_RESTORE) v.status = check_flac(g->units, g->param, v);
        if (g->kind == SYMACCEL_BATCH_ALAC_PREDICT) v.status = check_alac(g->param, v);
        if (g->kind == SYMACCEL_BATCH_ADPCM_DECODE) v.status = check_adpcm(g->units, g->param, v);
        if (g->kind == SYMACCEL_BATCH_MPA12_DECODE) v.status = check_mpa12(g->units, g->param, v);
        if (v.status == SYMACCEL_OK) v.status = v.fmt_status;
        if (g->kind == SYMACCEL_BATCH_FLAC_RESTORE && flac_verify_param(g->param).verify && v.status != SYMACCEL_OK) {
            symaccel_md5_state *st = v.state<symaccel_md5_state>(0);
            for (size_t f = 1; f < v.n_chains / g->ps.state_div; ++f) st[f] = st[0];
        }
    }
    g->row_pitch = serial_kind(g->kind) && g->knobs.row_pad && symaccel_row_stride(g->units) * 4 != g->ps.in[0] ? symaccel_row_stride(g->units) * 4 : 0;
}

size_t piece_bound(const Group *g) {
    const PlaneSizes &ps = g->ps;
    size_t bound = 0;
    for (const TicketView &v : g->views) {
        for (int i = 0; i < ps.n_in; ++i)
            if (!ps.in_host_only[i]) bound += pieces_of(plane_bytes(ps, i, v.n_chains));
        for (int i = 0; i < ps.n_state; ++i) bound += 2 * pieces_of(ps.state[i] * (v.n_chains / ps.state_div));
        bound += pieces_of(ps.out_per_chain() * v.n_chains);
        if (v.out_fmt) {
            const size_t tile = pcm_tile_frames(v.channels, (unsigned)symaccel_sample_bytes(v.out_fmt));
            bound += (v.n_chains / v.channels) * ((ps.out_per_chain() / 4 + tile - 1) / tile + 1);
        }
        if (g->kind == SYMACCEL_BATCH_AAC_DECODE) bound += pieces_of(ps.in[2] * v.n_chains);
    }
    bound += g->tickets + 8;
    if (g->kind == SYMACCEL_BATCH_FLAC_RESTORE && flac_verify_param(g->param).verify) bound += 2 * g->tickets + 8;
    if (g->row_pitch) bound += 2 * g->chains;
    for (const TicketView &v : g->views)
        if (v.in_fmt == SYMACCEL_IN_FMT_ROWS) bound += v.n_chains;
    if (vorbis_kind(g->kind)) bound += 2 * g->chains;
    if (g->kind == SYMACCEL_BATCH_AAC_DECODE) bound += 3 * g->tickets + 8;
    if (g->kind == SYMACCEL_BATCH_VORBIS_DECODE) {
        const auto &b = g->vb.bytes;
        bound += 6 * (g->tickets + 8) + pieces_of(b.boff) + pieces_of(b.kill) + pieces_of(b.first) + pieces_of(b.steps) + pieces_of(b.ys) + pieces_of(b.offs);
    }
    return bound;
}

size_t grown(const Group *g, size_t bytes, size_t slack) {
    return std::max(bytes + bytes / 4, (bytes / std::max<size_t>(1, g->chains) + 1) * std::max(g->cap_chains, g->chains) + slack);
}

void request_block(Group *g, size_t bound, BatchCopyDesc **descs, Carver &dev, Carver &host) {
    const PlaneSizes &ps = g->ps;
    host.want(descs, bound * sizeof(BatchCopyDesc));
    for (int i = 0; i < ps.n_in; ++i) {
        g->d_in[i] = nullptr;
        if (ps.in_host_only[i]) continue;
        dev.want(&g->d_in[i], ps.in_per_ticket[i] ? ps.in[i] * g->tickets : (i == 0 && g->row_pitch ? g->row_pitch : ps.in[i]) * ((g->chains + ps.in_div[i] - 1) / ps.in_div[i]));
    }
    for (int i = 0; i < ps.n_state; ++i) {
        dev.want(&g->d_state_in[i], ps.state[i] * (g->chains / ps.state_div));
        dev.want(&g->d_state_out[i], ps.state[i] * (g->chains / ps.state_div));
    }
    if (ps.in_place) g->d_out = g->d_in[0];
    else dev.want(&g->d_out, ps.out * g->chains);
    g->mp3.request(dev, host, g->tickets);
    if (g->kind == SYMACCEL_BATCH_AAC_DECODE) g->aac.request(dev, host, g->chains, g->units);
    if (g->kind == SYMACCEL_BATCH_FLAC_RESTORE && flac_verify_param(g->param).verify) g->fv.request(dev, host, g->tickets);
    if (g->kind == SYMACCEL_BATCH_VORBIS_DECODE) g->vb.request(dev, host, g->chains, vorbis_param(g->param, g->units).cap);
}

int carve_block(symaccel_ctx *ctx, Group *g, size_t bound, BatchCopyDesc **descs, uint64_t *n_allocs) {
    Block *blk = g->block;
    Carver dev, host;
    request_block(g, bound, descs, dev, host);
    if (dev.total > blk->d_bytes) {
        if (blk->d_base) SYM_GPU(ctx, hipFree(blk->d_base));
        blk->d_base = nullptr;
        blk->d_bytes = 0;
        void *d = nullptr;
        const size_t want = grown(g, dev.total, (size_t)1 << 20);
        SYM_TRY(ctx_alloc(ctx, &d, want, false));
        blk->d_base = static_cast<char *>(d);
        blk->d_bytes = want;
        *n_allocs += 1;
    }
    if (host.total > blk->h_desc_bytes) {
        if (blk->h_desc) (void)hipHostFree(blk->h_desc);
        blk->h_desc = nullptr;
        blk->h_desc_bytes = 0;
        void *h = nullptr;
        const size_t want = grown(g, host.total, 65536);
        if (hipHostMalloc(&h, want, hipHostMallocDefault) != hipSuccess) {
            (void)hipGetLastError();
            return SYMACCEL_ERR_OOM;
        }
        blk->h_desc = static_cast<char *>(h);
        blk->h_desc_bytes = want;
        *n_allocs += 1;
    }
    Carver dev_mem{blk->d_base}, host_mem{blk->h_desc};
    request_block(g, bound, descs, dev_mem, host_mem);
    for (hipEvent_t *e : {&blk->ev_in[0], &blk->ev_in[1], &blk->ev_k[0], &blk->ev_k[1]})
        if (!*e) SYM_GPU(ctx, hipEventCreateWithFlags(e, hipEventDisableTiming));
    return SYMACCEL_OK;
}

Chunk next_chunk(const Group *g, size_t t0) {
    const PlaneSizes &ps = g->ps;
    const size_t per_chain = std::max<size_t>(1, in_bytes_per_chain(ps));
    const size_t chunk_bytes = std::min<size_t>((size_t)32 << 20, std::max<size_t>(g->knobs.chunk_min, g->chains * per_chain / g->knobs.chunk_div));
    const size_t chunk_chains = std::max<size_t>(1, chunk_bytes / per_chain);
    Chunk ch{};
    ch.c0 = g->views[t0].first_chain;
    ch.t0 = t0;
    size_t t1 = t0;
    while (t1 < g->tickets && (ch.nc == 0 || ch.nc + g->views[t1].n_chains <= chunk_chains)) ch.nc += g->views[t1++].n_chains;
    ch.nt = t1 - t0;
    for (int i = 0; i < ps.n_in; ++i)
        if (g->d_in[i]) ch.in[i] = g->d_in[i] + (ps.in_per_ticket[i] ? t0 * ps.in[i] : (ch.c0 / ps.in_div[i]) * (i == 0 && g->row_pitch ? g->row_pitch : ps.in[i]));
    for (int i = 0; i < ps.n_state; ++i) {
        ch.si[i] = g->d_state_in[i] + ch.c0 / ps.state_div * ps.state[i];
        ch.so[i] = g->d_state_out[i] + ch.c0 / ps.state_div * ps.state[i];
    }
    ch.out = ps.in_place ? ch.in[0] : g->d_out + ch.c0 * ps.out;
    return ch;
}

void gather_vorbis_spectra(const Group *g, const TicketView &t, Pieces &pw) {
    for (size_t c = 0; c < t.n_chains; ++c)
        pw.bulk(t.slot + t.lay.in[0] + c * g->ps.in[0], g->d_in[0] + ((size_t)t.first_chain + c) * g->ps.in[0], t.used[c].lines * 4);
}
void gather_rows(const Group *g, const TicketView &t, Pieces &pw) {
    for (size_t c = 0; c < t.n_chains; ++c) pw.bulk(t.slot + t.lay.in[0] + c * g->ps.in[0], g->d_in[0] + ((size_t)t.first_chain + c) * g->row_pitch, g->ps.in[0]);
}

void gather_narrow(const Group *g, const TicketView &t, Pieces &pw) {
    const size_t row = g->ps.in[0];
    const char *src = t.slot + t.lay.in[0];
    if (!g->row_pitch) return pw.widen(src, g->d_in[0] + (size_t)t.first_chain * row, row * t.n_chains);
    for (size_t c = 0; c < t.n_chains; ++c) pw.widen(src + c * (row / 2), g->d_in[0] + ((size_t)t.first_chain + c) * g->row_pitch, row);
}

bool gather_row_widths(const Group *g, const TicketView &t, Pieces &pw) {
    const size_t row = g->ps.in[0], pitch = g->row_pitch ? g->row_pitch : row;
    const uint8_t *w = t.row_bytes();
    bool widening = false;
    for (size_t c = 0; c < t.n_chains; ++c) {
        const char *src = t.slot + t.lay.in[0] + c * row;
        char *dst = g->d_in[0] + ((size_t)t.first_chain + c) * pitch;
        if (w[c] == 2 || w[c] == 3) pw.widen(src, dst, row, w[c]), widening = true;
        else pw.add(src, dst, row);
    }
    return widening;
}

bool build_gather(Group *g, const Chunk &ch, Pieces &pw) {
    bool widening = false;
    const PlaneSizes &ps = g->ps;
    const bool verify = g->kind == SYMACCEL_BATCH_FLAC_RESTORE && flac_verify_param(g->param).verify;
    for (size_t ti = ch.t0; ti < ch.t0 + ch.nt; ++ti) {
        const TicketView &t = g->views[ti];
        for (int i = 0; i < ps.n_in; ++i) {
            if (ps.in_host_only[i]) continue;
            if (i == 0 && t.in_fmt == SYMACCEL_IN_FMT_ROWS) widening |= gather_row_widths(g, t, pw);
            else if (i == 0 && t.in_fmt) gather_narrow(g, t, pw), widening = true;
            else if (i == 0 && vorbis_kind(g->kind)) gather_vorbis_spectra(g, t, pw);
            else if (i == 0 && g->row_pitch) gather_rows(g, t, pw);
            else pw.bulk(t.slot + t.lay.in[i], g->d_in[i] + (ps.in_per_ticket[i] ? ti : (size_t)t.first_chain / ps.in_div[i]) * ps.in[i], t.lay.in_bytes[i]);
        }
        for (int i = 0; i < ps.n_state; ++i) pw.add(t.slot + t.lay.state[i], g->d_state_in[i] + (size_t)t.first_chain / ps.state_div * ps.state[i], verify ? ps.state[i] : t.lay.state_bytes[i]);
// ... 53 lines not shown
                                   (float *)so[0], (int32_t *)so[1], (float *)ch.out, ch.nc, g->units);
    default: return SYMACCEL_ERR_INVALID_ARG;
    }
}

bool scatter_converted(const Group *g, const TicketView &t, size_t plane_pitch, Pieces &pw) {
    const unsigned tile = pcm_tile_frames(t.channels, (unsigned)symaccel_sample_bytes(t.out_fmt));
    const size_t fb = (size_t)t.channels * symaccel_sample_bytes(t.out_fmt);
    char *dst = t.slot + t.lay.out;
    for (size_t c = 0; t.status == SYMACCEL_OK && c < t.n_chains; c += t.channels) {
        const size_t samples = t.used ? t.used[c].samples : g->ps.out_per_chain() / 4;
        const char *src = g->d_out + ((size_t)t.first_chain + c) * plane_pitch;
        for (size_t f0 = 0; f0 < samples; f0 += tile) {
            const size_t nf = std::min<size_t>(tile, samples - f0);
            pw.piece(src + f0 * 4, dst + f0 * fb, nf * fb, batch_piece_convert(serial_kind(g->kind), nf, t.channels, t.out_fmt));
        }
        dst += samples * fb;
    }
    return t.status == SYMACCEL_OK && t.n_chains != 0;
}

void build_scatter(const Group *g, const Chunk &ch, Pieces &pw, size_t *pcm_stride) {
    const PlaneSizes &ps = g->ps;
    const size_t plane_pitch = g->row_pitch ? g->row_pitch : ps.out_per_chain();
    const bool verify = g->kind == SYMACCEL_BATCH_FLAC_RESTORE && flac_verify_param(g->param).verify;
    bool converting = false;
    for (size_t ti = ch.t0; ti < ch.t0 + ch.nt; ++ti) {
        const TicketView &t = g->views[ti];
        if (t.out_fmt) {
            converting |= scatter_converted(g, t, plane_pitch, pw);
        } else if (vorbis_kind(g->kind)) {
            for (size_t c = 0; c < t.n_chains; ++c) pw.bulk(g->d_out + ((size_t)t.first_chain + c) * ps.out, t.slot + t.lay.out + c * ps.out, t.used[c].samples * 4);
        } else if (g->row_pitch) {
            for (size_t c = 0; c < t.n_chains; ++c) pw.bulk(g->d_out + ((size_t)t.first_chain + c) * g->row_pitch, t.slot + t.lay.out + c * ps.in[0], ps.in[0]);
        } else {
            pw.bulk(g->d_out + (size_t)t.first_chain * plane_pitch, t.slot + t.lay.out, t.lay.out_bytes);
        }
        if (verify && t.status != SYMACCEL_OK) continue;
        for (int i = 0; i < ps.n_state; ++i) pw.add(g->d_state_out[i] + (size_t)t.first_chain / ps.state_div * ps.state[i], t.slot + t.lay.state[i], t.lay.state_bytes[i]);
    }
    *pcm_stride = converting ? plane_pitch / 4 : 0;
}

int enqueue_copies(symaccel_ctx *ctx, hipStream_t s, Pieces &pw, const BatchCopyDesc *first, bool scatter, size_t pcm_stride, bool widening = false) {
    if (pw.overflow) {
        ctx->last_error = "batcher: a launch needs more copy pieces than piece_bound() counted";
        return SYMACCEL_ERR_DEVICE;
    }
    for (const Pieces::Dma &m : pw.dma) SYM_GPU(ctx, hipMemcpyAsync(m.dst, m.src, m.bytes, scatter ? hipMemcpyDeviceToHost : hipMemcpyHostToDevice, s));
    pw.dma.clear();
    return launch_batch_copy(ctx, s, first, (size_t)(pw.w - first), scatter, pcm_stride, widening);
}

int launch_group_inner(Lane *lane, Group *g, uint64_t *n_chunks, uint64_t *api_ns, uint64_t *n_allocs) {
    symaccel_ctx *ctx = lane->ctx;
    if (!ctx->stage_in) SYM_GPU(ctx, hipStreamCreate(&ctx->stage_in));
    if (!ctx->stage_out) SYM_GPU(ctx, hipStreamCreate(&ctx->stage_out));
    prepare_views(g);
    validate_and_count(g);
    const size_t bound = piece_bound(g);
    BatchCopyDesc *descs = nullptr;
    SYM_TRY(carve_block(ctx, g, bound, &descs, n_allocs));
    Block *blk = g->block;
    Pieces pw{descs, descs + bound, g->knobs.dma_bytes};
    for (size_t t0 = 0, k = 0; t0 < g->tickets; ++k) {
        const Chunk ch = next_chunk(g, t0);
        const int e = (int)(k & 1);
        const BatchCopyDesc *g0 = pw.w;
        const bool widening = build_gather(g, ch, pw);
        const Clock::time_point api0 = Clock::now();
        SYM_TRY(enqueue_copies(ctx, ctx->stage_in, pw, g0, false, 0, widening));
        SYM_GPU(ctx, hipEventRecord(blk->ev_in[e], ctx->stage_in));
        SYM_GPU(ctx, hipStreamWaitEvent(ctx->stream, blk->ev_in[e], 0));
        SYM_TRY(launch_chunk(ctx, g, ch));
        SYM_GPU(ctx, hipEventRecord(blk->ev_k[e], ctx->stream));
        SYM_GPU(ctx, hipStreamWaitEvent(ctx->stage_out, blk->ev_k[e], 0));
        *api_ns += ns_since(api0);
        const BatchCopyDesc *s0 = pw.w;
        size_t pcm_stride = 0;
        build_scatter(g, ch, pw, &pcm_stride);
        const Clock::time_point api1 = Clock::now();
        SYM_TRY(enqueue_copies(ctx, ctx->stage_out, pw, s0, true, pcm_stride));
        *api_ns += ns_since(api1);
        *n_chunks += 1;
        t0 += ch.nt;
    }
    return SYMACCEL_OK;
}

Block *pick_block(symaccel_batcher *b, Group *g) {
    Block *found = nullptr;
    for (auto &up : b->blocks) {
        Block *k = up.get();
        if (k->owner == nullptr) {
            found = k;
            break;
        }
        Group *o = k->owner;
        if (o->state == GroupState::Launched && (o->completed || read_flag(k->h_flag) >= k->seq)) {
            o->completed = true;
            o->block = nullptr;
            found = k;
            break;
        }
    }
    if (!found) {
        void *h = nullptr;
        if (hipHostMalloc(&h, 64, hipHostMallocDefault) != hipSuccess) {
            (void)hipGetLastError();
            return nullptr;
        }
        std::memset(h, 0, 64);
// ... 198 lines not shown
            std::this_thread::sleep_for(std::chrono::microseconds(20));
            if ((spins & 1023) == 0 && std::chrono::duration<double>(Clock::now() - t0).count() > kFlagTimeout) {
                Locked l(b);
                b->last_error = "the completion flag of a batch never arrived";
                return SYMACCEL_ERR_DEVICE;
            }
        }
    }
    Locked l(b);
    const uint64_t waited = ns_since(t0);
    b->stats.waits += 1;
    if (waited > 2000) {
        b->stats.waits_blocked += 1;
        if (!g->completed) b->stats.launch_to_done_ns += ns_since(g->launched_at), b->stats.launches_timed += 1;
    }
    g->completed = true;
    b->stats.flag_wait_ns += waited;
    return SYMACCEL_OK;
}

}

extern "C" {

int symaccel_batcher_create(symaccel_ctx *ctx, size_t flush_bytes, symaccel_batcher **out) {
    if (!ctx || !out) return SYMACCEL_ERR_INVALID_ARG;
    *out = nullptr;
    symaccel_batcher *b = new (std::nothrow) symaccel_batcher();
    if (!b) return SYMACCEL_ERR_OOM;
    b->ctx = ctx;
    b->flush_bytes = flush_bytes ? flush_bytes : (size_t)64 << 20;
    b->hint_bytes = std::min<size_t>((size_t)4 << 20, b->flush_bytes / 8);
    if (const char *e = std::getenv("SYMACCEL_BATCHER_HINT_MB"))
        if (std::atoi(e) > 0) b->hint_bytes = (size_t)std::atoi(e) << 20;
    if (const char *e = std::getenv("SYMACCEL_BATCHER_BUSY_GROUPS"))
        b->busy_groups = (size_t)std::max(0, std::atoi(e));
    if (const char *e = std::getenv("SYMACCEL_BATCHER_BUSY_HINT_MB"))
        if (std::atoi(e) > 0) b->busy_hint_bytes = (size_t)std::atoi(e) << 20;
    if (const char *e = std::getenv("SYMACCEL_BATCHER_LANES"))
        if (std::atoi(e) > 0) b->want_lanes = std::min(8, std::atoi(e));
    if (const char *e = std::getenv("SYMACCEL_BATCH_ROW_PAD")) b->knobs.row_pad = std::atol(e) != 0;
    if (const char *e = std::getenv("SYMACCEL_BATCH_DMA_KB")) b->knobs.dma_bytes = (size_t)std::atol(e) << 10;
    if (const char *e = std::getenv("SYMACCEL_BATCH_CHUNKS")) b->knobs.chunk_div = (size_t)std::min(64L, std::max(1L, std::atol(e)));
    if (const char *e = std::getenv("SYMACCEL_BATCH_CHUNK_MIN_KB")) b->knobs.chunk_min = (size_t)std::max(64L, std::atol(e)) << 10;
    *out = b;
    return SYMACCEL_OK;
}

int symaccel_batcher_configure(symaccel_batcher *b, int lanes, size_t hint_bytes) {
    if (!b || lanes < 0 || lanes > 8) return SYMACCEL_ERR_INVALID_ARG;
    Locked l(b);
    if (lanes) b->want_lanes = (size_t)lanes;
    if (hint_bytes) b->hint_bytes = hint_bytes;
    return SYMACCEL_OK;
}

int symaccel_batcher_destroy(symaccel_batcher *b) {
    if (!b) return SYMACCEL_OK;
    {
        DeviceGuard dev(b->ctx);
        for (auto &ln : b->lanes) {
            std::unique_lock<std::mutex> lane_lock(ln->mu);
            if (ln->ctx->stage_in) (void)hipStreamSynchronize(ln->ctx->stage_in);
            if (ln->ctx->stream) (void)hipStreamSynchronize(ln->ctx->stream);
            if (ln->ctx->stage_out) (void)hipStreamSynchronize(ln->ctx->stage_out);
        }
        for (auto &k : b->blocks) block_free(k.get());
        for (auto &sl : b->slabs) (void)hipHostFree(sl.base);
    }
    for (auto &ln : b->lanes)
        if (ln->owned) symaccel_ctx_destroy(ln->ctx);
    delete b;
    return SYMACCEL_OK;
}

int symaccel_batcher_reserve(symaccel_batcher *b, int kind, int param, size_t n_chains, size_t units_per_chain, symaccel_batch_slot *slot,
                             uint64_t *ticket) {
    return symaccel_batcher_reserve_fmt(b, kind, param, n_chains, units_per_chain, 0, 0, slot, ticket);
}

int symaccel_batcher_reserve_fmt(symaccel_batcher *b, int kind, int param, size_t n_chains, size_t units_per_chain, int out_fmt, int channels,
                                 symaccel_batch_slot *slot, uint64_t *ticket) {
    return symaccel_batcher_reserve_io(b, kind, param, n_chains, units_per_chain, 0, out_fmt, channels, slot, ticket);
}

int symaccel_batcher_reserve_io(symaccel_batcher *b, int kind, int param, size_t n_chains, size_t units_per_chain, int in_fmt, int out_fmt,
                                int channels, symaccel_batch_slot *slot, uint64_t *ticket) {
    if (in_fmt != 0 && ((in_fmt != SYMACCEL_FMT_S16 && in_fmt != SYMACCEL_IN_FMT_ROWS) || !serial_kind(kind))) return SYMACCEL_ERR_INVALID_ARG;
    if (!b || !slot || !ticket || n_chains == 0 || n_chains > 0x7fffffffu) return SYMACCEL_ERR_INVALID_ARG;
    if (units_per_chain == 0 && kind != SYMACCEL_BATCH_PCM_DECODE) return SYMACCEL_ERR_INVALID_ARG;
    if (kind == SYMACCEL_BATCH_ADPCM_DECODE) {
        if (param < 0 || (param >> 16) || (out_fmt != 0 && (symaccel_sample_bytes(out_fmt) == 0 || channels != adpcm_param(param).nch))) return SYMACCEL_ERR_INVALID_ARG;
        param |= out_fmt << 16;
        out_fmt = channels = 0;
    }
    if (kind == SYMACCEL_BATCH_PCM_DECODE) {
        if (param < 0 || (param >> 24) || (out_fmt != 0 && (symaccel_sample_bytes(out_fmt) == 0 || channels != pcmdec_param(param).nch))) return SYMACCEL_ERR_INVALID_ARG;
        param |= out_fmt << 24;
        out_fmt = channels = 0;
    }
    if (out_fmt != 0 && (symaccel_sample_bytes(out_fmt) == 0 || channels < 1 || channels > 8 || n_chains % (size_t)channels != 0)) return SYMACCEL_ERR_INVALID_ARG;
    PlaneSizes ps;
    if (kind == SYMACCEL_BATCH_AAC_SYNTH) param = 0;
    if (!plane_sizes(kind, param, units_per_chain, &ps)) return SYMACCEL_ERR_INVALID_ARG;
    if ((kind == SYMACCEL_BATCH_MP3_SYNTH || kind == SYMACCEL_BATCH_MP3_DECODE) && (param < 0 || param > 8)) return SYMACCEL_ERR_INVALID_ARG;
    if (kind == SYMACCEL_BATCH_MP3_DECODE && n_chains > 2) return SYMACCEL_ERR_INVALID_ARG;
// ... 508 lines not shown
```

### symphonia_amd/csrc/ctx.cpp

```cpp
#include <cstring>
#include <new>

#include "symaccel_internal.h"

using namespace symaccel;

namespace symaccel {

int ctx_fail(symaccel_ctx *ctx, hipError_t err, const char *where) {
    if (ctx) {
        ctx->last_error = std::string(where) + ": " + hipGetErrorString(err);
    }
    return err == hipErrorOutOfMemory ? SYMACCEL_ERR_OOM : SYMACCEL_ERR_DEVICE;
}

int ctx_alloc(symaccel_ctx *ctx, void **out, size_t bytes, bool tracked) {
    *out = nullptr;
    if (bytes == 0) bytes = 16;
    SYM_GPU(ctx, hipMalloc(out, bytes));
    if (tracked) ctx->allocations.push_back(*out);
    return SYMACCEL_OK;
}

int ctx_sink(symaccel_ctx *ctx, void **out) {
    if (!ctx->sink) SYM_TRY(ctx_alloc(ctx, &ctx->sink, kSinkBytes, false));
    *out = ctx->sink;
    return SYMACCEL_OK;
}

int ctx_scratch(symaccel_ctx *ctx, size_t bytes, void **out) {
    if (bytes > ctx->scratch_bytes) {
        if (ctx->scratch) {
            SYM_GPU(ctx, hipStreamSynchronize(ctx->stream));
            SYM_GPU(ctx, hipFree(ctx->scratch));
            ctx->scratch = nullptr;
            ctx->scratch_bytes = 0;
        }
        size_t want = bytes + bytes / 4 + 4096;
        SYM_TRY(ctx_alloc(ctx, &ctx->scratch, want, false));
        ctx->scratch_bytes = want;
    }
    *out = ctx->scratch;
    return SYMACCEL_OK;
}

int ctx_upload(symaccel_ctx *ctx, const void *src, size_t bytes, const void **out) {
    void *d = nullptr;
    SYM_TRY(ctx_alloc(ctx, &d, bytes));
    SYM_GPU(ctx, hipMemcpy(d, src, bytes, hipMemcpyHostToDevice));
    *out = d;
    return SYMACCEL_OK;
}

unsigned choose_segment(const symaccel_ctx *ctx, size_t n_chains, size_t frames_per_chain, unsigned waves_per_cu,
                        unsigned items_per_wave, unsigned halo, unsigned min_seg) {
    if (frames_per_chain == 0) return 1;
    if (ctx->segment > 0) {
        unsigned s = (unsigned)ctx->segment < min_seg ? min_seg : (unsigned)ctx->segment;
        return s > frames_per_chain ? (unsigned)frames_per_chain : s;
    }
    const double slots = (double)ctx->n_cus * waves_per_cu * items_per_wave;
    const unsigned lo = min_seg, hi = frames_per_chain < 256 ? (unsigned)frames_per_chain : 256u;
    if (hi <= lo) return hi < 1 ? 1 : hi;
    unsigned best = hi;
    double best_cost = 1e300;
    for (unsigned seg = lo; seg <= hi; ++seg) {
        const double items = (double)n_chains * (double)((frames_per_chain + seg - 1) / seg);
        const double rounds = items <= slots ? 1.0 : (double)(size_t)((items + slots - 1) / slots);
        const double fill = items < slots ? 0.5 + 0.5 * items / slots : 1.0;
        const double cost = rounds * (double)(seg + halo) * fill;
        if (cost < best_cost * 0.999 || (cost <= best_cost * 1.001 && seg > best)) {
            if (cost < best_cost) best_cost = cost;
            best = seg;
        }
    }
    return best;
}

int get_imdct_plan(symaccel_ctx *ctx, int n, double scale, const ImdctPlan **out) {
    uint64_t bits;
    std::memcpy(&bits, &scale, 8);
    auto key = std::make_pair(n, bits);
    auto it = ctx->imdct_plans.find(key);
    if (it == ctx->imdct_plans.end()) {
        std::vector<cpx> tw((size_t)n / 2);
        make_imdct_twiddles(n, scale, tw.data());
        const void *d = nullptr;
        SYM_TRY(ctx_upload(ctx, tw.data(), tw.size() * sizeof(cpx), &d));
        it = ctx->imdct_plans.emplace(key, ImdctPlan{n, (cpx *)d}).first;
    }
    *out = &it->second;
    return SYMACCEL_OK;
}

int get_vorbis_window(symaccel_ctx *ctx, int bs, const float **out) {
    auto it = ctx->vorbis_windows.find(bs);
    if (it == ctx->vorbis_windows.end()) {
        std::vector<float> w((size_t)bs / 2);
        make_vorbis_window(bs, w.data());
        const void *d = nullptr;
        SYM_TRY(ctx_upload(ctx, w.data(), w.size() * sizeof(float), &d));
        it = ctx->vorbis_windows.emplace(bs, (float *)d).first;
    }
    *out = it->second;
    return SYMACCEL_OK;
}

namespace {

void build_reorder_tables(const HostTables &t, std::vector<int32_t> &map, std::vector<int32_t> &end) {
    map.assign(9 * 2 * 576, 0);
    end.assign(9 * 2 * 577, 0);
    for (int sr = 0; sr < 9; ++sr) {
        for (int mixed = 0; mixed < 2; ++mixed) {
// ... 1428 lines not shown
```

### symphonia_amd/csrc/symaccel_internal.h

```cpp
#pragma once

#include <cstddef>
#include <cstdint>
#include <map>
#include <string>
#include <utility>
#include <vector>

#include "../../include/symaccel.h"
#include <hip/hip_runtime.h>

namespace symaccel {

struct cpx {
    float re, im;
};

constexpr int kMp3Pow2abMinE = -1300, kMp3Pow2abLen = 1346;
constexpr int kMp3Unscaled = 39;

struct HostTables {
    std::vector<float> aac_kbd_long, aac_kbd_short, aac_sine_long, aac_sine_short;
    std::vector<cpx> aac_tw_long, aac_tw_short;
    std::vector<cpx> fft_merge;
// ... 56 lines not shown
    MP3C_COS1 = 260,
    MP3C_SYNTH_D = 264,
    MP3C_TOTAL = 776
};

constexpr int kMpa12Classes = 17;
enum Mpa12Layout {
    MPA12_FACTOR = 0,
    MPA12_SCF = 16,
    MPA12_CLASS = 80,
    MPA12_TOTAL = 131
};
constexpr int mpa12_n_frames(int layer) { return layer == SYMACCEL_MPA_LAYER1 ? 12 : layer == SYMACCEL_MPA_LAYER2 ? 36 : 0; }

struct ImdctPlan {
    int n;
    cpx *d_twiddle;
};

}

struct symaccel_ctx {
    int device = 0;
    hipStream_t stream = nullptr;
    hipStream_t own_stream = nullptr;
    int segment = 0;
    int n_cus = 256;
    std::string last_error;
    symaccel::DevTables dev{};
    std::vector<void *> allocations;
    std::map<std::pair<int, uint64_t>, symaccel::ImdctPlan> imdct_plans;
    std::map<int, float *> vorbis_windows;
    void *scratch = nullptr;
    size_t scratch_bytes = 0;
    hipStream_t stage_in = nullptr, stage_out = nullptr;
    hipEvent_t stage_events[6] = {nullptr, nullptr, nullptr, nullptr, nullptr, nullptr};
    void *stage_arena = nullptr;
    size_t stage_arena_bytes = 0;
    void *sink = nullptr;
    void *alac_flags = nullptr;
    size_t alac_flags_bytes = 0;
};

namespace symaccel {

int ctx_fail(symaccel_ctx *ctx, hipError_t err, const char *where);
int ctx_alloc(symaccel_ctx *ctx, void **out, size_t bytes, bool tracked = true);
int ctx_scratch(symaccel_ctx *ctx, size_t bytes, void **out);
constexpr size_t kSinkBytes = 2u << 20;
int ctx_sink(symaccel_ctx *ctx, void **out);
int ctx_upload(symaccel_ctx *ctx, const void *src, size_t bytes, const void **out);
int get_imdct_plan(symaccel_ctx *ctx, int n, double scale, const ImdctPlan **out);
unsigned choose_segment(const symaccel_ctx *ctx, size_t n_chains, size_t frames_per_chain, unsigned waves_per_cu,
                        unsigned items_per_wave, unsigned halo, unsigned min_seg);
int get_vorbis_window(symaccel_ctx *ctx, int bs, const float **out);

class DeviceGuard {
public:
    explicit DeviceGuard(symaccel_ctx *ctx) {
        if (hipGetDevice(&prev_) != hipSuccess) prev_ = -1;
        if (prev_ != ctx->device) {
            const hipError_t e = hipSetDevice(ctx->device);
            if (e != hipSuccess) {
                status_ = ctx_fail(ctx, e, "hipSetDevice");
                prev_ = -1;
            } else {
                switched_ = true;
            }
        }
    }
    ~DeviceGuard() {
        if (switched_ && prev_ >= 0) (void)hipSetDevice(prev_);
    }
    DeviceGuard(const DeviceGuard &) = delete;
    DeviceGuard &operator=(const DeviceGuard &) = delete;
    bool ok() const { return status_ == SYMACCEL_OK; }
    int status() const { return status_; }

private:
    int prev_ = -1;
    int status_ = SYMACCEL_OK;
    bool switched_ = false;
};

#define SYM_TRY(expr)                                                   \
    do {                                                                \
        int _st = (expr);                                               \
        if (_st != SYMACCEL_OK) return _st;                             \
    } while (0)
#define SYM_GPU(ctx, expr)                                              \
    do {                                                                \
        hipError_t _e = (expr);                                         \
        if (_e != hipSuccess) return ::symaccel::ctx_fail((ctx), _e, #expr); \
    } while (0)

struct AacBandMaps {
    uint8_t long4[256];
    uint8_t short4[32];
};

int launch_fft_big_wave(symaccel_ctx *ctx, int n, const float *d_in, float *d_out, size_t count, bool inverse);
int launch_fft4096_wg(symaccel_ctx *ctx, const float *d_in, float *d_out, size_t count, bool inverse);
int launch_imdct8192_wg(symaccel_ctx *ctx, const cpx *d_twiddle, const float *d_spec, float *d_out, size_t count);
int launch_imdct_big_wave(symaccel_ctx *ctx, const cpx *d_twiddle, int nf, const float *d_spec, float *d_out, size_t count);
int launch_fft(symaccel_ctx *ctx, int n, const float *d_in, float *d_out, size_t count, bool inverse = false);
int launch_imdct(symaccel_ctx *ctx, const ImdctPlan &plan, const float *d_spec, float *d_out, size_t count);
int launch_aac(symaccel_ctx *ctx, const float *d_coeffs, const uint8_t *d_side, const float *d_delay_in,
               float *d_delay_out, float *d_pcm, size_t n_chains, size_t frames_per_chain, const AacBandMaps *maps = nullptr,
               const int32_t *d_pair_chains = nullptr, const symaccel_aac_js_frame *d_js_desc = nullptr, size_t n_pairs = 0,
               void *d_js_scratch = nullptr);
inline size_t aac_js_scratch_bytes(size_t n_chains, size_t n_pairs, size_t frames_per_chain) {
    (void)n_pairs;
    (void)frames_per_chain;
    return ((n_chains * 8 + 255) & ~(size_t)255) + 256;
}
struct Mp3State {
    float *overlap;
    float *vvec;
    int32_t *vfront;
    static constexpr size_t kOverlap = 576 * 4, kVvec = 1024 * 4, kVfront = 4;
    static size_t bytes(size_t n_chains) { return n_chains * (kOverlap + kVvec + kVfront); }
    static Mp3State carve(void *base, size_t n_chains) {
        char *p = static_cast<char *>(base);
        return {(float *)p, (float *)(p + n_chains * kOverlap), (int32_t *)(p + n_chains * (kOverlap + kVvec))};
    }
};
int launch_mp3(symaccel_ctx *ctx, const float *d_xr, const symaccel_mp3_side *d_side, int sr,
               const float *d_overlap_in, const float *d_vvec_in, const int32_t *d_vfront_in,
               float *d_overlap_out, float *d_vvec_out, int32_t *d_vfront_out, float *d_pcm,
               size_t n_chains, size_t granules_per_chain);
int launch_vorbis(symaccel_ctx *ctx, int bs0_exp, int bs1_exp, const float *d_spectra, const float *d_residue,
                  size_t spec_stride,
                  const uint8_t *d_block_flag, const int32_t *d_prev_in, int32_t *d_prev_out,
                  const float *d_overlap_in, float *d_overlap_out, float *d_pcm, size_t pcm_stride,
                  size_t n_chains, size_t blocks_per_chain, void *d_offsets, const uint8_t *d_floor_y = nullptr);
int launch_vorbis_wave(symaccel_ctx *ctx, const cpx *tw_short, const cpx *tw_long, const float *win_short,
                       const float *win_long, const float *d_spectra, const float *d_residue, size_t spec_stride,
                       const uint8_t *d_block_flag,
                       const int32_t *d_prev_in, int32_t *d_prev_out, const float *d_overlap_in, float *d_overlap_out,
                       float *d_pcm, size_t pcm_stride, size_t n_chains, unsigned nb, unsigned seg, int floor_mode);
#ifndef SYM_VORBIS_WG
#define SYM_VORBIS_WG 1
#endif
#ifndef SYM_VORBIS_WG_SHARED
#define SYM_VORBIS_WG_SHARED 1
#endif
int launch_vorbis_wg(symaccel_ctx *ctx, int bs0_exp, int bs1_exp, const cpx *tw_short, const cpx *tw_long, const float *win_short,
                     const float *win_long, const float *d_spectra, const float *d_residue, size_t spec_stride, const uint8_t *d_block_flag,
                     const int32_t *d_prev_in, int32_t *d_prev_out, const float *d_overlap_in, float *d_overlap_out, float *d_pcm,
                     size_t pcm_stride, size_t n_chains, unsigned nb, unsigned seg, int floor_mode);
int launch_vorbis_wave2(symaccel_ctx *ctx, int bs0_exp, int bs1_exp, const cpx *tw_short, const cpx *tw_long, const float *win_short,
                        const float *win_long, const float *d_spectra, const float *d_residue, size_t spec_stride,
                        const uint8_t *d_block_flag, const int32_t *d_prev_in, int32_t *d_prev_out, const float *d_overlap_in,
                        float *d_overlap_out, float *d_pcm, size_t pcm_stride, size_t n_chains, unsigned nb, unsigned seg, int floor_mode);
int launch_vorbis_coupling(symaccel_ctx *ctx, float *d_mag, float *d_ang, size_t n);
int launch_vorbis_prepare(symaccel_ctx *ctx, float *d_residue, size_t spec_stride, unsigned channels_per_stream, size_t n_streams,
                          size_t blocks, const uint32_t *d_block_off, const uint8_t *d_steps, const uint32_t *d_step_first,
                          const uint8_t *d_kill);
int launch_vorbis_dot(symaccel_ctx *ctx, float *d_floor, const float *d_residue, size_t total);
int launch_vorbis_deinterleave(symaccel_ctx *ctx, const float *d_type2, float *d_planar, int n_ch, size_t n2,
                               size_t count);
int launch_vorbis_floor1(symaccel_ctx *ctx, const uint32_t *h_setup, int n_posts, int multiplier,
                         const uint32_t *d_y, uint32_t n, float *d_floor, size_t count, const float *d_residue = nullptr,
// ... 165 lines not shown
```

Measured before the change: 337.9 million.

## Add row-pointer AAC walk path that reads host slots directly, skipping staging copies

Moves the AAC kernel body into a shared header and adds a batch path where AAC synth groups build a per-chain table of pointers (coeffs, side, delay, pcm) into the ticket slots. A persistent walk kernel with a capped workgroup count then reads and writes those slots directly instead of staging planes through device buffers with batch copies. When chains are split into segments, delay state is snapshotted on the host so segment halos stay consistent. A new API knob sets the walk workgroup count. This aims to remove staging copy launches and traffic, at the cost of fewer workgroups and possibly slower direct access to host-mapped memory.

```diff
diff --git a/bindings/rust/symaccel_sys.rs b/bindings/rust/symaccel_sys.rs
--- a/bindings/rust/symaccel_sys.rs
+++ b/bindings/rust/symaccel_sys.rs
@@ -410,6 +410,7 @@
     pub fn symaccel_batcher_create(ctx: *mut SymaccelCtx, flush_bytes: usize, out: *mut *mut SymaccelBatcher) -> i32;
     pub fn symaccel_batcher_destroy(b: *mut SymaccelBatcher) -> i32;
     pub fn symaccel_batcher_configure(b: *mut SymaccelBatcher, lanes: i32, hint_bytes: usize) -> i32;
+    pub fn symaccel_batcher_set_walk_workgroups(b: *mut SymaccelBatcher, workgroups: i32) -> i32;
     pub fn symaccel_batcher_last_error(b: *mut SymaccelBatcher, buf: *mut core::ffi::c_char, capacity: usize) -> i32;
     pub fn symaccel_batcher_reserve(b: *mut SymaccelBatcher, kind: i32, param: i32, n_chains: usize, units_per_chain: usize, slot: *mut SymaccelBatchSlot, ticket: *mut u64) -> i32;
     pub fn symaccel_batcher_commit(b: *mut SymaccelBatcher, ticket: u64) -> i32;
diff --git a/include/symaccel.h b/include/symaccel.h
--- a/include/symaccel.h
+++ b/include/symaccel.h
@@ -494,6 +494,7 @@
 int symaccel_batcher_create(symaccel_ctx *ctx, size_t flush_bytes, symaccel_batcher **out);
 int symaccel_batcher_destroy(symaccel_batcher *b);
 int symaccel_batcher_configure(symaccel_batcher *b, int lanes, size_t hint_bytes);
+int symaccel_batcher_set_walk_workgroups(symaccel_batcher *b, int workgroups);
 int symaccel_batcher_last_error(symaccel_batcher *b, char *buf, size_t capacity);
 int symaccel_batcher_reserve(symaccel_batcher *b, int kind, int param, size_t n_chains, size_t units_per_chain,
                              symaccel_batch_slot *slot, uint64_t *ticket);
diff --git a/symphonia_amd/_ffi.py b/symphonia_amd/_ffi.py
--- a/symphonia_amd/_ffi.py
+++ b/symphonia_amd/_ffi.py
@@ -56,7 +56,7 @@
     "symaccel_batcher_create", "symaccel_batcher_destroy", "symaccel_batcher_reserve", "symaccel_batcher_commit", "symaccel_batcher_wait",
     "symaccel_batcher_release", "symaccel_batcher_submit", "symaccel_batcher_collect", "symaccel_batcher_abandon",
     "symaccel_batcher_submit_aac_synth", "symaccel_batcher_submit_mp3_synth", "symaccel_batcher_submit_mp3_decode", "symaccel_batcher_submit_vorbis_synth", "symaccel_batcher_aac_bands", "symaccel_batcher_submit_aac_decode", "symaccel_batcher_flush", "symaccel_batcher_hint", "symaccel_batcher_plane_bytes",
-    "symaccel_batcher_get_stats", "symaccel_batcher_configure", "symaccel_batcher_last_error", "symaccel_batcher_vorbis_floor",
+    "symaccel_batcher_get_stats", "symaccel_batcher_configure", "symaccel_batcher_set_walk_workgroups", "symaccel_batcher_last_error", "symaccel_batcher_vorbis_floor",
     "symaccel_batcher_submit_vorbis_decode", "symaccel_batcher_submit_flac_restore", "symaccel_batcher_submit_alac_predict",
     "symaccel_flac_restore_strided_device", "symaccel_alac_predict_strided_device", "symaccel_row_stride",
     "symaccel_md5_init", "symaccel_md5_update", "symaccel_md5_digest", "symaccel_flac_md5_device", "symaccel_flac_md5",
@@ -165,6 +165,8 @@
         d.symaccel_batcher_submit_vorbis_synth.argtypes = [_vp, _i, _i, _vp, _vp, _vp, _vp, _vp, _sz, _sz, C.POINTER(C.c_uint64)]
         d.symaccel_batcher_get_stats.argtypes = [_vp, _vp]
         d.symaccel_batcher_configure.argtypes = [_vp, _i, _sz]
+        if hasattr(d, "symaccel_batcher_set_walk_workgroups"):
+            d.symaccel_batcher_set_walk_workgroups.argtypes = [_vp, _i]
         d.symaccel_batcher_last_error.argtypes = [_vp, _vp, _sz]
         d.symaccel_batcher_vorbis_floor.argtypes = [_vp, _vp, C.POINTER(_i)]
         d.symaccel_batcher_submit_vorbis_decode.argtypes = [_vp, _i, _i, _vp, _vp, _vp, _vp, _vp, _vp, _vp, _vp, _vp, _sz, _sz, C.POINTER(C.c_uint64)]
diff --git a/symphonia_amd/backend.py b/symphonia_amd/backend.py
--- a/symphonia_amd/backend.py
+++ b/symphonia_amd/backend.py
@@ -1013,6 +1013,9 @@
     def configure(self, lanes=0, hint_bytes=0):
         self._check(self.dll.symaccel_batcher_configure(self.handle, int(lanes), int(hint_bytes)))
 
+    def set_walk_workgroups(self, workgroups):
+        self._check(self.dll.symaccel_batcher_set_walk_workgroups(self.handle, int(workgroups)))
+
     def last_error(self):
         buf = C.create_string_buffer(512)
         self._check(self.dll.symaccel_batcher_last_error(self.handle, buf, 512))
diff --git a/symphonia_amd/csrc/aac.hip b/symphonia_amd/csrc/aac.hip
--- a/symphonia_amd/csrc/aac.hip
+++ b/symphonia_amd/csrc/aac.hip
@@ -1,118 +1,11 @@
-#include <type_traits>
-
-#include "imdct_wave.h"
+#include "aac_walk.h"
 
 namespace symaccel {
 
 namespace {
 
-#ifndef SYM_AAC_VARIANT
-#define SYM_AAC_VARIANT 0
-#endif
-#if SYM_AAC_VARIANT == 1
-constexpr int kWaves = 6;
-#define SYM_AAC_WAVES_PER_SIMD 3
-#else
-constexpr int kWaves = 4;
-#endif
-constexpr int kTabTw = 0;
-constexpr int kTabKbd = 1024;
-constexpr int kTabSine = 2048;
-constexpr int kTabKbdShort = 3072;
-constexpr int kTabSineShort = 3200;
-constexpr int kTabFloats = 3328;
-
-enum : int { ONLY_LONG = 0, LONG_START = 1, EIGHT_SHORT = 2, LONG_STOP = 3 };
-constexpr int kP0 = 512 - 64;
-constexpr int kP1 = 512 + 64;
-
-__device__ __forceinline__ void pcm_short4(const float *H, int q0, const float *short_win, const float *prev_short_win,
-                                           float (&acc)[4]) {
-    const int w = q0 >> 7, i0 = q0 & 127;
-    bool have = false;
-    if (w >= 1) {
-        float a[4];
-        ys4(H, w - 1, 128 + i0, a);
-        const float4 wr = *reinterpret_cast<const float4 *>(short_win + 124 - i0);
-        a[0] *= wr.w; a[1] *= wr.z; a[2] *= wr.y; a[3] *= wr.x;
-#pragma unroll
-        for (int q = 0; q < 4; ++q) acc[q] = (w - 1 == 0) ? a[q] : (0.0f + a[q]);
-        have = true;
-    }
-    if (w <= 7) {
-        float bq[4];
-        ys4(H, w, i0, bq);
-        const float4 wf = *reinterpret_cast<const float4 *>((w == 0 ? prev_short_win : short_win) + i0);
-        bq[0] *= wf.x; bq[1] *= wf.y; bq[2] *= wf.z; bq[3] *= wf.w;
-#pragma unroll
-        for (int q = 0; q < 4; ++q) acc[q] = have ? (acc[q] + bq[q]) : bq[q];
-    }
-}
-
-__device__ __forceinline__ void stop_window4(const float *psw, int j0, float *w) {
-    float4 v = make_float4(1.0f, 1.0f, 1.0f, 1.0f);
-    if (j0 >= kP0 && j0 < kP1) v = *reinterpret_cast<const float4 *>(psw + j0 - kP0);
-    w[0] = v.x; w[1] = v.y; w[2] = v.z; w[3] = v.w;
-}
-__device__ __forceinline__ void start_window4(const float *sw, int j0, float *w) {
-    float4 v = make_float4(1.0f, 1.0f, 1.0f, 1.0f);
-    if (j0 >= kP0 && j0 < kP1) {
-        const float4 r = *reinterpret_cast<const float4 *>(sw + 124 - (j0 - kP0));
-        v = make_float4(r.w, r.z, r.y, r.x);
-    }
-    w[0] = v.x; w[1] = v.y; w[2] = v.z; w[3] = v.w;
-}
-
-#if defined(SYM_AAC_WAVES_PER_SIMD) && !defined(SYM_AAC_MIN_WAVES)
-#define SYM_AAC_MIN_WAVES SYM_AAC_WAVES_PER_SIMD
-#endif
-#ifndef SYM_AAC_MIN_WAVES
-#define SYM_AAC_MIN_WAVES 2
-#endif
-#ifndef SYM_AAC_PREFETCH
-#define SYM_AAC_PREFETCH 1
-#endif
-#ifndef SYM_AAC_QUAD
-#define SYM_AAC_QUAD 1
-#endif
-__device__ __forceinline__ float2 ld_line(const float2 *p) { return ld_stream(p); }
-__device__ __forceinline__ void st_slot(float *frame, int m2, const float (&v)[8]) {
-    float4 *o4 = reinterpret_cast<float4 *>(frame);
-    st_stream(o4 + m2, make_float4(v[0], v[1], v[2], v[3]));
-    st_stream(o4 + 255 - m2, make_float4(v[4], v[5], v[6], v[7]));
-}
-
-
 #if !SYM_AAC_QUAD
 #include "experiments/aac_wave_walk.h"
-#endif
-
-
-
-constexpr int kSlotOff = kShortRowsEnd;
-static_assert(kSlotOff + 1024 <= kWaveLds, "delay slot must fit the per-wave LDS behind the short-window rows");
-
-enum : int { kStepHalo = 0, kStepFull = 1, kStepRagged = 2 };
-template <int V> using step_kind = std::integral_constant<int, V>;
-
-__device__ __forceinline__ void settle_prefetch(const float2 (&line)[8]) {
-#if defined(__HIP_DEVICE_COMPILE__)
-    __builtin_amdgcn_sched_barrier(0);
-    asm volatile("" : : "v"(line[0].x), "v"(line[0].y), "v"(line[1].x), "v"(line[1].y), "v"(line[2].x), "v"(line[2].y), "v"(line[3].x), "v"(line[3].y),
-                        "v"(line[4].x), "v"(line[4].y), "v"(line[5].x), "v"(line[5].y), "v"(line[6].x), "v"(line[6].y), "v"(line[7].x), "v"(line[7].y));
-#endif
-}
-
-struct AacJsArgs {
-    const int2 *chain;
-    const int32_t *pair_chains;
-    const symaccel_aac_js_frame *desc;
-    AacBandMaps maps;
-    unsigned n_chains;
-};
-
-#if SYM_AAC_QUAD == 2
-#include "experiments/aac_quad_probe.h"
 #endif
 
 template <bool JS>
@@ -149,272 +42,7 @@
     const long t_end = t_begin + (long)seg_steps * 4 < (long)frames_per_chain ? t_begin + (long)seg_steps * 4 : (long)frames_per_chain;
     if (t_end <= t_begin) return;
     const size_t chain_base0 = (size_t)chain * frames_per_chain, chain_base1 = (size_t)chain1 * frames_per_chain;
-    LaneTables lt;
-    load_lane_tables(tb, lane, lt);
-
-    const bool has_halo = t_begin > 0;
-    if (!has_halo && wave == 3) {
-#pragma unroll
-        for (int ch = 0; ch < CH; ++ch) {
-            const float4 *src = reinterpret_cast<const float4 *>(delay_in + (size_t)(ch ? chain1 : chain) * 1024);
-#pragma unroll
-            for (int q = 0; q < 4; ++q) reinterpret_cast<float4 *>(carry[ch][1])[lane + 64 * q] = src[lane + 64 * q];
-        }
-    }
-    const long t_first = (wave == 3 && has_halo) ? t_begin - 1 : t_begin + wave;
-    float2 line[8];
-    unsigned sb_next = 0;
-    float2 line1[8];
-    uint32_t dq[3] = {0u, 0u, 0u};
-    unsigned sb1_next = 0;
-    uint32_t sfb_long[2] = {0u, 0u};
-    unsigned sfb_short = 0;
-    auto fetch1 = [&](long tf, int ln) {
-        if constexpr (JS) {
-            const float2 *ps = reinterpret_cast<const float2 *>(coeffs + (chain_base1 + (size_t)tf) * 1024);
-            const uint32_t *d = reinterpret_cast<const uint32_t *>(js.desc + (size_t)unit * frames_per_chain + (size_t)tf);
-#pragma unroll
-            for (int s = 0; s < 8; ++s) line1[s] = ld_line(ps + ln + 64 * s);
-            dq[0] = d[ln];
-            dq[1] = d[ln + 64];
-            dq[2] = ln < 33 ? d[ln + 128] : 0u;
-            sb1_next = side[chain_base1 + (size_t)tf];
-        }
-    };
-    if constexpr (JS) {
-#pragma unroll
-        for (int s = 0; s < 8; ++s) sfb_long[s >> 2] |= (uint32_t)js.maps.long4[(lane >> 1) + 32 * s] << (8 * (s & 3));
-        sfb_short = js.maps.short4[(lane >> 1) & 31];
-    }
-    if (t_first < t_end) {
-        const float2 *src = reinterpret_cast<const float2 *>(coeffs + (chain_base0 + (size_t)t_first) * 1024);
-#pragma unroll
-        for (int s = 0; s < 8; ++s) line[s] = ld_line(src + lane + 64 * s);
-        sb_next = side[chain_base0 + (size_t)t_first];
-        fetch1(t_first, lane);
-    } else {
-#pragma unroll
-        for (int s = 0; s < 8; ++s) line[s] = make_float2(0.0f, 0.0f);
-        if constexpr (JS) {
-#pragma unroll
-            for (int s = 0; s < 8; ++s) line1[s] = make_float2(0.0f, 0.0f);
-        }
-    }
-    __syncthreads();
-
-    const int lane_of_wave = lane;
-    auto step = [&](auto kind_c, int i, long t, bool active) __attribute__((always_inline)) {
-        constexpr int KIND = decltype(kind_c)::value;
-        int lane = lane_of_wave;
-        if constexpr (JS) {
-#if defined(__HIP_DEVICE_COMPILE__)
-            asm volatile("" : "+v"(lane));
-#endif
-        }
-        const unsigned sb0 = (unsigned)__builtin_amdgcn_readfirstlane((int)sb_next);
-        const unsigned sb1 = JS ? (unsigned)__builtin_amdgcn_readfirstlane((int)sb1_next) : 0u;
-        if constexpr (JS) {
-            if (active) {
-                uint32_t *dl = reinterpret_cast<uint32_t *>(ldsf);
-                dl[lane] = dq[0];
-                dl[lane + 64] = dq[1];
-                if (lane < 33) dl[lane + 128] = dq[2];
-                wave_sync();
-                const unsigned hdr = dl[0];
-                const bool one = (hdr & 255u) == 1u;
-                const int max_sfb = (int)((hdr >> 8) & 255u);
-                const uint8_t *mode = reinterpret_cast<const uint8_t *>(dl + 1);
-                const float *scale = reinterpret_cast<const float *>(dl + 33);
-#pragma unroll
-                for (int s = 0; s < 8; ++s) {
-                    const float2 l = line[s], r = line1[s];
-                    const int sfb = one ? (int)((sfb_long[s >> 2] >> (8 * (s & 3))) & 255u) : (int)sfb_short;
-                    const int slot = one ? sfb : 16 * s + sfb;
-                    const bool coded = sfb < max_sfb && slot < 128;
-                    const int sl = slot < 127 ? slot : 127;
-                    const unsigned m = mode[sl];
-                    const float sc = scale[sl];
-                    const bool ms = coded && m == SYMACCEL_AAC_JS_MS, is = coded && m == SYMACCEL_AAC_JS_INTENSITY;
-                    line[s] = ms ? make_float2(l.x + r.x, l.y + r.y) : l;
-                    line1[s] = ms ? make_float2(l.x - r.x, l.y - r.y) : (is ? make_float2(sc * l.x, sc * l.y) : r);
-                }
-                wave_sync();
-            }
-        }
-        const long tn = KIND == kStepHalo ? t_begin + 3 : (t + 4 < t_end ? t + 4 : t);
-        const bool fetch = KIND == kStepFull || (KIND == kStepHalo && tn < t_end);
-#pragma unroll 1
-        for (int ch = 0; ch < CH; ++ch) {
-        if constexpr (JS) {
-#if defined(__HIP_DEVICE_COMPILE__)
-            asm volatile("" : "+v"(lane));
-#endif
-        }
-        const unsigned sb = ch ? sb1 : sb0;
-        const size_t chain_base = ch ? chain_base1 : chain_base0;
-        const int seq = (int)(sb & 3u);
-        const int shape = (int)((sb >> 2) & 1u), prev_shape = (int)((sb >> 3) & 1u);
-        float *my_slot = wave == 3 ? carry[ch][i & 1] : ldsf + kSlotOff;
-        float *prev_slot = wave == 0 ? carry[ch][(i + 1) & 1] : wave_lds[wave > 0 ? wave - 1 : 0] + kSlotOff;
-        float xw[2][8];
-        auto ln_at = [&](int s) -> float2 {
-            if constexpr (JS) return ch ? line1[s] : line[s];
-            else return line[s];
-        };
-        auto long_tail = [&](auto seq_c) __attribute__((always_inline)) {
-            constexpr int SEQ = decltype(seq_c)::value;
-            const float *wprev = tabs + (prev_shape ? kTabKbd : kTabSine);
-            const float *wcur = tabs + (shape ? kTabKbd : kTabSine);
-#pragma unroll
-            for (int h = 0; h < 2; ++h) {
-                const int m2 = lane + 64 * h;
-                float x[8], x2[8];
-                post_slot(lds, tw, m2, x, x2);
-                float wo[8];
-                if constexpr (SEQ == LONG_STOP) {
-                    const float *psw = tabs + (prev_shape ? kTabKbdShort : kTabSineShort);
-                    stop_window4(psw, 4 * m2, wo);
-                    stop_window4(psw, 1020 - 4 * m2, wo + 4);
-                } else {
-                    load_slot(wprev, m2, wo);
-                }
-#pragma unroll
-                for (int q = 0; q < 8; ++q) xw[h][q] = x[q] * wo[q];
-                float wd[8], nd[8];
-                if constexpr (SEQ == LONG_START) {
-                    const float *sw = tabs + (shape ? kTabKbdShort : kTabSineShort);
-                    start_window4(sw, 4 * m2, wd);
-                    start_window4(sw, 1020 - 4 * m2, wd + 4);
-                } else {
-                    float wr[8];
-                    if (SEQ == ONLY_LONG && shape == prev_shape) {
-#pragma unroll
-                        for (int q = 0; q < 8; ++q) wr[q] = wo[q];
-                    } else {
-                        load_slot(wcur, m2, wr);
-                    }
-#pragma unroll
-                    for (int q = 0; q < 8; ++q) wd[q] = wr[7 - q];
-                }
-#pragma unroll
-                for (int q = 0; q < 8; ++q) {
-                    const int j = q < 4 ? 4 * m2 + q : 1020 - 4 * m2 + (q - 4);
-                    const float v = x2[q] * wd[q];
-                    nd[q] = (SEQ == LONG_START && j >= kP1) ? 0.0f : v;
-                }
-                store_slot(my_slot, m2, nd);
-            }
-        };
-
-        if (active) {
-            c32 z[8];
-            if (seq != EIGHT_SHORT) {
-                const int mirror = (63 - lane) * 4;
-#pragma unroll
-                for (int s = 0; s < 8; ++s) {
-                    const float mirrored = __int_as_float(__builtin_amdgcn_ds_bpermute(mirror, __float_as_int(ln_at(7 - s).y)));
-                    z[s] = pre_twiddle(ln_at(s).x, mirrored, tw[lane + 64 * s]);
-                }
-            } else {
-#pragma unroll
-                for (int s = 0; s < 8; ++s) {
-                    ldsf[short_row(s) + 2 * lane] = ln_at(s).x;
-                    ldsf[short_row(s) + 2 * lane + 1] = ln_at(s).y;
-                }
-                wave_sync();
-            }
-            if (fetch) {
-                if (ch == 0) {
-                    sb_next = side[chain_base0 + (size_t)tn];
-                    const float2 *src = reinterpret_cast<const float2 *>(coeffs + (chain_base0 + (size_t)tn) * 1024);
-#pragma unroll
-                    for (int s = 0; s < 8; ++s) line[s] = ld_line(src + lane + 64 * s);
-                }
-                if (ch == CH - 1) fetch1(tn, lane);
-            }
-            if (seq != EIGHT_SHORT) {
-                fft512_wave(z, lane, lds, lt);
-                if (seq == ONLY_LONG) long_tail(step_kind<ONLY_LONG>{});
-                else if (seq == LONG_START) long_tail(step_kind<LONG_START>{});
-                else long_tail(step_kind<LONG_STOP>{});
-            } else {
-                imdct_short_wave(lane, ldsf, tb.aac_tw_short, lt);
-                const float *sw = tabs + (shape ? kTabKbdShort : kTabSineShort);
-                const float *psw = tabs + (prev_shape ? kTabKbdShort : kTabSineShort);
-#pragma unroll 1
-                for (int e = 0; e < 4; ++e) {
-                    const int j0 = 4 * lane + 256 * e;
-                    float nd[4] = {0.0f, 0.0f, 0.0f, 0.0f};
-                    if (j0 < kP1) pcm_short4(ldsf, j0 + kP1, sw, psw, nd);
-                    *reinterpret_cast<float4 *>(my_slot + j0) = make_float4(nd[0], nd[1], nd[2], nd[3]);
-                }
-            }
-        }
-        if constexpr (KIND == kStepHalo) {
-            wave_sync();
-        } else {
-        wg_sync_lds();
-
-        if (active) {
-            float *frame_out = pcm + (chain_base + (size_t)t) * 1024;
-            float dst[2][8];
-            if (seq != EIGHT_SHORT) {
-#pragma unroll
-                for (int h = 0; h < 2; ++h) {
-                    const int m2 = lane + 64 * h;
-                    float dl[8];
-                    load_slot(prev_slot, m2, dl);
-#pragma unroll
-                    for (int q = 0; q < 8; ++q) dst[h][q] = dl[q] + xw[h][q];
-                    if (seq == LONG_STOP) {
-#pragma unroll
-                        for (int q = 0; q < 8; ++q) {
-                            const int j = q < 4 ? 4 * m2 + q : 1020 - 4 * m2 + (q - 4);
-                            dst[h][q] = j < kP0 ? dl[q] : dst[h][q];
-                        }
-                    }
-                }
-            } else {
-                const float *sw = tabs + (shape ? kTabKbdShort : kTabSineShort);
-                const float *psw = tabs + (prev_shape ? kTabKbdShort : kTabSineShort);
-#pragma unroll 1
-                for (int e = 0; e < 4; ++e) {
-                    const int j0 = 4 * lane + 256 * e;
-                    const float4 d = *reinterpret_cast<const float4 *>(prev_slot + j0);
-                    float o[4] = {d.x, d.y, d.z, d.w};
-                    if (j0 >= kP0) {
-                        float ps[4];
-                        pcm_short4(ldsf, j0 - kP0, sw, psw, ps);
-#pragma unroll
-                        for (int q = 0; q < 4; ++q) o[q] = o[q] + ps[q];
-                    }
-                    *reinterpret_cast<float4 *>(prev_slot + j0) = make_float4(o[0], o[1], o[2], o[3]);
-                }
-                wave_sync();
-#pragma unroll
-                for (int h = 0; h < 2; ++h) load_slot(prev_slot, lane + 64 * h, dst[h]);
-            }
-#pragma unroll
-            for (int h = 0; h < 2; ++h) st_slot(frame_out, lane + 64 * h, dst[h]);
-            if constexpr (KIND == kStepFull && !JS) settle_prefetch(line);
-            if (t + 1 == (long)frames_per_chain) {
-                float4 *d = reinterpret_cast<float4 *>(delay_out + (size_t)(ch ? chain1 : chain) * 1024);
-#pragma unroll
-                for (int q = 0; q < 4; ++q) d[lane + 64 * q] = reinterpret_cast<const float4 *>(my_slot)[lane + 64 * q];
-            }
-        }
-        wg_sync_lds();
-        }
-        }
-    };
-
-    if (has_halo && wave == 3) step(step_kind<kStepHalo>{}, -1, t_begin - 1, true);
-    if constexpr (!JS) settle_prefetch(line);
-    const int n_full = (int)((t_end - t_begin) >> 2);
-    long t = t_begin + wave;
-#pragma unroll 1
-    for (int i = 0; i < n_full; ++i, t += 4) step(step_kind<kStepFull>{}, i, t, true);
-    if ((t_end - t_begin) & 3) step(step_kind<kStepRagged>{}, n_full, t, t < t_end);
+#include "aac_walk_item.h"
 }
 
 __global__ void aac_js_index_kernel(const int32_t *__restrict__ pair_chains, unsigned n_pairs, unsigned n_chains, int2 *__restrict__ chain_index) {
diff --git a/symphonia_amd/csrc/aac_rows.hip b/symphonia_amd/csrc/aac_rows.hip
--- /dev/null
+++ b/symphonia_amd/csrc/aac_rows.hip
@@ -0,0 +1,86 @@
+#include "aac_walk.h"
+
+namespace symaccel {
+
+namespace {
+
+#define SYM_AAC_ROWS (SYM_AAC_QUAD == 1 && SYM_AAC_VARIANT == 0)
+#if SYM_AAC_ROWS
+#if defined(__HIP_DEVICE_COMPILE__)
+#define SYM_AAC_GLOBAL(T, p) ((T *)(__attribute__((address_space(1))) T *)(uintptr_t)(p))
+#else
+#define SYM_AAC_GLOBAL(T, p) (p)
+#endif
+__global__ __launch_bounds__(256, SYM_AAC_MIN_WAVES) void aac_rows_walk_kernel(DevTables tb, const AacRow *__restrict__ rows, unsigned n_items,
+                                                                               unsigned frames_per_chain, unsigned seg_steps, unsigned segs_per_chain) {
+    __shared__ __attribute__((aligned(16))) float tabs[kTabFloats];
+    __shared__ __attribute__((aligned(16))) float wave_lds[4][kWaveLds];
+    constexpr bool JS = false;
+    constexpr int CH = 1;
+    __shared__ __attribute__((aligned(16))) float carry[CH][2][1024];
+    for (int i = (int)threadIdx.x; i < 1024; i += 256) {
+        tabs[kTabTw + i] = reinterpret_cast<const float *>(tb.aac_tw_long)[i];
+        tabs[kTabKbd + i] = tb.aac_kbd_long[i];
+        tabs[kTabSine + i] = tb.aac_sine_long[i];
+        if (i < 128) {
+            tabs[kTabKbdShort + i] = tb.aac_kbd_short[i];
+            tabs[kTabSineShort + i] = tb.aac_sine_short[i];
+        }
+    }
+    const int lane = (int)threadIdx.x & 63, wave = __builtin_amdgcn_readfirstlane((int)threadIdx.x >> 6);
+    float *ldsf = wave_lds[wave];
+    c32 *lds = reinterpret_cast<c32 *>(ldsf);
+    const c32 *tw = reinterpret_cast<const c32 *>(tabs + kTabTw);
+    const AacJsArgs js{nullptr, nullptr, nullptr, AacBandMaps{}, 0u};
+#pragma unroll 1
+    for (unsigned item = blockIdx.x; item < n_items; item += gridDim.x) {
+        const unsigned unit = item / segs_per_chain, seg = item % segs_per_chain;
+        const long t_begin = (long)seg * seg_steps * 4;
+        const long t_end = t_begin + (long)seg_steps * 4 < (long)frames_per_chain ? t_begin + (long)seg_steps * 4 : (long)frames_per_chain;
+        if (t_end <= t_begin) continue;
+        const AacRow row = rows[unit];
+        const float *coeffs = SYM_AAC_GLOBAL(const float, row.coeffs), *delay_in = SYM_AAC_GLOBAL(const float, row.delay_in);
+        const uint8_t *side = SYM_AAC_GLOBAL(const uint8_t, row.side);
+        float *delay_out = SYM_AAC_GLOBAL(float, row.delay_out), *pcm = SYM_AAC_GLOBAL(float, row.pcm);
+        constexpr unsigned chain = 0, chain1 = 0;
+        constexpr size_t chain_base0 = 0, chain_base1 = 0;
+#include "aac_walk_item.h"
+    }
+}
+#endif
+
+}
+
+bool aac_rows_available() { return SYM_AAC_ROWS; }
+
+unsigned aac_rows_seg_steps(const symaccel_ctx *ctx, size_t n_chains, size_t frames_per_chain, unsigned workgroups) {
+    const size_t steps_per_chain = (frames_per_chain + 3) / 4;
+    unsigned seg_steps;
+    if (ctx->segment > 0) seg_steps = (unsigned)((ctx->segment + 3) / 4);
+    else if (n_chains >= workgroups) seg_steps = (unsigned)steps_per_chain;
+    else seg_steps = choose_segment(ctx, n_chains, steps_per_chain, 1, 1, 1, 16, workgroups);
+    if (seg_steps > steps_per_chain) seg_steps = (unsigned)steps_per_chain;
+    return seg_steps < 1 ? 1 : seg_steps;
+}
+
+int launch_aac_rows(symaccel_ctx *ctx, hipStream_t stream, const AacRow *rows, size_t n_chains, size_t frames_per_chain, unsigned seg_steps,
+                    unsigned workgroups) {
+#if SYM_AAC_ROWS
+    if (n_chains == 0 || frames_per_chain == 0) return SYMACCEL_OK;
+    if (frames_per_chain > 0x7fffffffu || seg_steps == 0 || workgroups == 0) return SYMACCEL_ERR_INVALID_ARG;
+    const size_t steps_per_chain = (frames_per_chain + 3) / 4;
+    const size_t segs = (steps_per_chain + seg_steps - 1) / seg_steps;
+    const size_t items = n_chains * segs;
+    if (items > 0x7fffffffu) return SYMACCEL_ERR_INVALID_ARG;
+    const unsigned grid = (unsigned)(items < workgroups ? items : workgroups);
+    hipLaunchKernelGGL(aac_rows_walk_kernel, dim3(grid), dim3(256), 0, stream, ctx->dev, rows, (unsigned)items, (unsigned)frames_per_chain, seg_steps,
+                       (unsigned)segs);
+    SYM_GPU(ctx, hipGetLastError());
+    return SYMACCEL_OK;
+#else
+    ctx->last_error = "aac: this build has no row-table walk";
+    return SYMACCEL_ERR_INVALID_ARG;
+#endif
+}
+
+}
diff --git a/symphonia_amd/csrc/aac_walk.h b/symphonia_amd/csrc/aac_walk.h
--- /dev/null
+++ b/symphonia_amd/csrc/aac_walk.h
@@ -0,0 +1,118 @@
+#pragma once
+#include <type_traits>
+
+#include "imdct_wave.h"
+
+namespace symaccel {
+
+namespace {
+
+#ifndef SYM_AAC_VARIANT
+#define SYM_AAC_VARIANT 0
+#endif
+#if SYM_AAC_VARIANT == 1
+constexpr int kWaves = 6;
+#define SYM_AAC_WAVES_PER_SIMD 3
+#else
+constexpr int kWaves = 4;
+#endif
+constexpr int kTabTw = 0;
+constexpr int kTabKbd = 1024;
+constexpr int kTabSine = 2048;
+constexpr int kTabKbdShort = 3072;
+constexpr int kTabSineShort = 3200;
+constexpr int kTabFloats = 3328;
+
+enum : int { ONLY_LONG = 0, LONG_START = 1, EIGHT_SHORT = 2, LONG_STOP = 3 };
+constexpr int kP0 = 512 - 64;
+constexpr int kP1 = 512 + 64;
+
+__device__ __forceinline__ void pcm_short4(const float *H, int q0, const float *short_win, const float *prev_short_win,
+                                           float (&acc)[4]) {
+    const int w = q0 >> 7, i0 = q0 & 127;
+    bool have = false;
+    if (w >= 1) {
+        float a[4];
+        ys4(H, w - 1, 128 + i0, a);
+        const float4 wr = *reinterpret_cast<const float4 *>(short_win + 124 - i0);
+        a[0] *= wr.w; a[1] *= wr.z; a[2] *= wr.y; a[3] *= wr.x;
+#pragma unroll
+        for (int q = 0; q < 4; ++q) acc[q] = (w - 1 == 0) ? a[q] : (0.0f + a[q]);
+        have = true;
+    }
+    if (w <= 7) {
+        float bq[4];
+        ys4(H, w, i0, bq);
+        const float4 wf = *reinterpret_cast<const float4 *>((w == 0 ? prev_short_win : short_win) + i0);
+        bq[0] *= wf.x; bq[1] *= wf.y; bq[2] *= wf.z; bq[3] *= wf.w;
+#pragma unroll
+        for (int q = 0; q < 4; ++q) acc[q] = have ? (acc[q] + bq[q]) : bq[q];
+    }
+}
+
+__device__ __forceinline__ void stop_window4(const float *psw, int j0, float *w) {
+    float4 v = make_float4(1.0f, 1.0f, 1.0f, 1.0f);
+    if (j0 >= kP0 && j0 < kP1) v = *reinterpret_cast<const float4 *>(psw + j0 - kP0);
+    w[0] = v.x; w[1] = v.y; w[2] = v.z; w[3] = v.w;
+}
+__device__ __forceinline__ void start_window4(const float *sw, int j0, float *w) {
+    float4 v = make_float4(1.0f, 1.0f, 1.0f, 1.0f);
+    if (j0 >= kP0 && j0 < kP1) {
+        const float4 r = *reinterpret_cast<const float4 *>(sw + 124 - (j0 - kP0));
+        v = make_float4(r.w, r.z, r.y, r.x);
+    }
+    w[0] = v.x; w[1] = v.y; w[2] = v.z; w[3] = v.w;
+}
+
+#if defined(SYM_AAC_WAVES_PER_SIMD) && !defined(SYM_AAC_MIN_WAVES)
+#define SYM_AAC_MIN_WAVES SYM_AAC_WAVES_PER_SIMD
+#endif
+#ifndef SYM_AAC_MIN_WAVES
+#define SYM_AAC_MIN_WAVES 2
+#endif
+#ifndef SYM_AAC_PREFETCH
+#define SYM_AAC_PREFETCH 1
+#endif
+#ifndef SYM_AAC_QUAD
+#define SYM_AAC_QUAD 1
+#endif
+__device__ __forceinline__ float2 ld_line(const float2 *p) { return ld_stream(p); }
+__device__ __forceinline__ void st_slot(float *frame, int m2, const float (&v)[8]) {
+    float4 *o4 = reinterpret_cast<float4 *>(frame);
+    st_stream(o4 + m2, make_float4(v[0], v[1], v[2], v[3]));
+    st_stream(o4 + 255 - m2, make_float4(v[4], v[5], v[6], v[7]));
+}
+
+
+
+
+
+constexpr int kSlotOff = kShortRowsEnd;
+static_assert(kSlotOff + 1024 <= kWaveLds, "delay slot must fit the per-wave LDS behind the short-window rows");
+
+enum : int { kStepHalo = 0, kStepFull = 1, kStepRagged = 2 };
+template <int V> using step_kind = std::integral_constant<int, V>;
+
+__device__ __forceinline__ void settle_prefetch(const float2 (&line)[8]) {
+#if defined(__HIP_DEVICE_COMPILE__)
+    __builtin_amdgcn_sched_barrier(0);
+    asm volatile("" : : "v"(line[0].x), "v"(line[0].y), "v"(line[1].x), "v"(line[1].y), "v"(line[2].x), "v"(line[2].y), "v"(line[3].x), "v"(line[3].y),
+                        "v"(line[4].x), "v"(line[4].y), "v"(line[5].x), "v"(line[5].y), "v"(line[6].x), "v"(line[6].y), "v"(line[7].x), "v"(line[7].y));
+#endif
+}
+
+struct AacJsArgs {
+    const int2 *chain;
+    const int32_t *pair_chains;
+    const symaccel_aac_js_frame *desc;
+    AacBandMaps maps;
+    unsigned n_chains;
+};
+
+#if SYM_AAC_QUAD == 2
+#include "experiments/aac_quad_probe.h"
+#endif
+
+}
+
+}
diff --git a/symphonia_amd/csrc/aac_walk_item.h b/symphonia_amd/csrc/aac_walk_item.h
--- /dev/null
+++ b/symphonia_amd/csrc/aac_walk_item.h
@@ -0,0 +1,266 @@
+    LaneTables lt;
+    load_lane_tables(tb, lane, lt);
+
+    const bool has_halo = t_begin > 0;
+    if (!has_halo && wave == 3) {
+#pragma unroll
+        for (int ch = 0; ch < CH; ++ch) {
+            const float4 *src = reinterpret_cast<const float4 *>(delay_in + (size_t)(ch ? chain1 : chain) * 1024);
+#pragma unroll
+            for (int q = 0; q < 4; ++q) reinterpret_cast<float4 *>(carry[ch][1])[lane + 64 * q] = src[lane + 64 * q];
+        }
+    }
+    const long t_first = (wave == 3 && has_halo) ? t_begin - 1 : t_begin + wave;
+    float2 line[8];
+    unsigned sb_next = 0;
+    float2 line1[8];
+    uint32_t dq[3] = {0u, 0u, 0u};
+    unsigned sb1_next = 0;
+    uint32_t sfb_long[2] = {0u, 0u};
+    unsigned sfb_short = 0;
+    auto fetch1 = [&](long tf, int ln) {
+        if constexpr (JS) {
+            const float2 *ps = reinterpret_cast<const float2 *>(coeffs + (chain_base1 + (size_t)tf) * 1024);
+            const uint32_t *d = reinterpret_cast<const uint32_t *>(js.desc + (size_t)unit * frames_per_chain + (size_t)tf);
+#pragma unroll
+            for (int s = 0; s < 8; ++s) line1[s] = ld_line(ps + ln + 64 * s);
+            dq[0] = d[ln];
+            dq[1] = d[ln + 64];
+            dq[2] = ln < 33 ? d[ln + 128] : 0u;
+            sb1_next = side[chain_base1 + (size_t)tf];
+        }
+    };
+    if constexpr (JS) {
+#pragma unroll
+        for (int s = 0; s < 8; ++s) sfb_long[s >> 2] |= (uint32_t)js.maps.long4[(lane >> 1) + 32 * s] << (8 * (s & 3));
+        sfb_short = js.maps.short4[(lane >> 1) & 31];
+    }
+    if (t_first < t_end) {
+        const float2 *src = reinterpret_cast<const float2 *>(coeffs + (chain_base0 + (size_t)t_first) * 1024);
+#pragma unroll
+        for (int s = 0; s < 8; ++s) line[s] = ld_line(src + lane + 64 * s);
+        sb_next = side[chain_base0 + (size_t)t_first];
+        fetch1(t_first, lane);
+    } else {
+#pragma unroll
+        for (int s = 0; s < 8; ++s) line[s] = make_float2(0.0f, 0.0f);
+        if constexpr (JS) {
+#pragma unroll
+            for (int s = 0; s < 8; ++s) line1[s] = make_float2(0.0f, 0.0f);
+        }
+    }
+    __syncthreads();
+
+    const int lane_of_wave = lane;
+    auto step = [&](auto kind_c, int i, long t, bool active) __attribute__((always_inline)) {
+        constexpr int KIND = decltype(kind_c)::value;
+        int lane = lane_of_wave;
+        if constexpr (JS) {
+#if defined(__HIP_DEVICE_COMPILE__)
+            asm volatile("" : "+v"(lane));
+#endif
+        }
+        const unsigned sb0 = (unsigned)__builtin_amdgcn_readfirstlane((int)sb_next);
+        const unsigned sb1 = JS ? (unsigned)__builtin_amdgcn_readfirstlane((int)sb1_next) : 0u;
+        if constexpr (JS) {
+            if (active) {
+                uint32_t *dl = reinterpret_cast<uint32_t *>(ldsf);
+                dl[lane] = dq[0];
+                dl[lane + 64] = dq[1];
+                if (lane < 33) dl[lane + 128] = dq[2];
+                wave_sync();
+                const unsigned hdr = dl[0];
+                const bool one = (hdr & 255u) == 1u;
+                const int max_sfb = (int)((hdr >> 8) & 255u);
+                const uint8_t *mode = reinterpret_cast<const uint8_t *>(dl + 1);
+                const float *scale = reinterpret_cast<const float *>(dl + 33);
+#pragma unroll
+                for (int s = 0; s < 8; ++s) {
+                    const float2 l = line[s], r = line1[s];
+                    const int sfb = one ? (int)((sfb_long[s >> 2] >> (8 * (s & 3))) & 255u) : (int)sfb_short;
+                    const int slot = one ? sfb : 16 * s + sfb;
+                    const bool coded = sfb < max_sfb && slot < 128;
+                    const int sl = slot < 127 ? slot : 127;
+                    const unsigned m = mode[sl];
+                    const float sc = scale[sl];
+                    const bool ms = coded && m == SYMACCEL_AAC_JS_MS, is = coded && m == SYMACCEL_AAC_JS_INTENSITY;
+                    line[s] = ms ? make_float2(l.x + r.x, l.y + r.y) : l;
+                    line1[s] = ms ? make_float2(l.x - r.x, l.y - r.y) : (is ? make_float2(sc * l.x, sc * l.y) : r);
+                }
+                wave_sync();
+            }
+        }
+        const long tn = KIND == kStepHalo ? t_begin + 3 : (t + 4 < t_end ? t + 4 : t);
+        const bool fetch = KIND == kStepFull || (KIND == kStepHalo && tn < t_end);
+#pragma unroll 1
+        for (int ch = 0; ch < CH; ++ch) {
+        if constexpr (JS) {
+#if defined(__HIP_DEVICE_COMPILE__)
+            asm volatile("" : "+v"(lane));
+#endif
+        }
+        const unsigned sb = ch ? sb1 : sb0;
+        const size_t chain_base = ch ? chain_base1 : chain_base0;
+        const int seq = (int)(sb & 3u);
+        const int shape = (int)((sb >> 2) & 1u), prev_shape = (int)((sb >> 3) & 1u);
+        float *my_slot = wave == 3 ? carry[ch][i & 1] : ldsf + kSlotOff;
+        float *prev_slot = wave == 0 ? carry[ch][(i + 1) & 1] : wave_lds[wave > 0 ? wave - 1 : 0] + kSlotOff;
+        float xw[2][8];
+        auto ln_at = [&](int s) -> float2 {
+            if constexpr (JS) return ch ? line1[s] : line[s];
+            else return line[s];
+        };
+        auto long_tail = [&](auto seq_c) __attribute__((always_inline)) {
+            constexpr int SEQ = decltype(seq_c)::value;
+            const float *wprev = tabs + (prev_shape ? kTabKbd : kTabSine);
+            const float *wcur = tabs + (shape ? kTabKbd : kTabSine);
+#pragma unroll
+            for (int h = 0; h < 2; ++h) {
+                const int m2 = lane + 64 * h;
+                float x[8], x2[8];
+                post_slot(lds, tw, m2, x, x2);
+                float wo[8];
+                if constexpr (SEQ == LONG_STOP) {
+                    const float *psw = tabs + (prev_shape ? kTabKbdShort : kTabSineShort);
+                    stop_window4(psw, 4 * m2, wo);
+                    stop_window4(psw, 1020 - 4 * m2, wo + 4);
+                } else {
+                    load_slot(wprev, m2, wo);
+                }
+#pragma unroll
+                for (int q = 0; q < 8; ++q) xw[h][q] = x[q] * wo[q];
+                float wd[8], nd[8];
+                if constexpr (SEQ == LONG_START) {
+                    const float *sw = tabs + (shape ? kTabKbdShort : kTabSineShort);
+                    start_window4(sw, 4 * m2, wd);
+                    start_window4(sw, 1020 - 4 * m2, wd + 4);
+                } else {
+                    float wr[8];
+                    if (SEQ == ONLY_LONG && shape == prev_shape) {
+#pragma unroll
+                        for (int q = 0; q < 8; ++q) wr[q] = wo[q];
+                    } else {
+                        load_slot(wcur, m2, wr);
+                    }
+#pragma unroll
+                    for (int q = 0; q < 8; ++q) wd[q] = wr[7 - q];
+                }
+#pragma unroll
+                for (int q = 0; q < 8; ++q) {
+                    const int j = q < 4 ? 4 * m2 + q : 1020 - 4 * m2 + (q - 4);
+                    const float v = x2[q] * wd[q];
+                    nd[q] = (SEQ == LONG_START && j >= kP1) ? 0.0f : v;
+                }
+                store_slot(my_slot, m2, nd);
+            }
+        };
+
+        if (active) {
+            c32 z[8];
+            if (seq != EIGHT_SHORT) {
+                const int mirror = (63 - lane) * 4;
+#pragma unroll
+                for (int s = 0; s < 8; ++s) {
+                    const float mirrored = __int_as_float(__builtin_amdgcn_ds_bpermute(mirror, __float_as_int(ln_at(7 - s).y)));
+                    z[s] = pre_twiddle(ln_at(s).x, mirrored, tw[lane + 64 * s]);
+                }
+            } else {
+#pragma unroll
+                for (int s = 0; s < 8; ++s) {
+                    ldsf[short_row(s) + 2 * lane] = ln_at(s).x;
+                    ldsf[short_row(s) + 2 * lane + 1] = ln_at(s).y;
+                }
+                wave_sync();
+            }
+            if (fetch) {
+                if (ch == 0) {
+                    sb_next = side[chain_base0 + (size_t)tn];
+                    const float2 *src = reinterpret_cast<const float2 *>(coeffs + (chain_base0 + (size_t)tn) * 1024);
+#pragma unroll
+                    for (int s = 0; s < 8; ++s) line[s] = ld_line(src + lane + 64 * s);
+                }
+                if (ch == CH - 1) fetch1(tn, lane);
+            }
+            if (seq != EIGHT_SHORT) {
+                fft512_wave(z, lane, lds, lt);
+                if (seq == ONLY_LONG) long_tail(step_kind<ONLY_LONG>{});
+                else if (seq == LONG_START) long_tail(step_kind<LONG_START>{});
+                else long_tail(step_kind<LONG_STOP>{});
+            } else {
+                imdct_short_wave(lane, ldsf, tb.aac_tw_short, lt);
+                const float *sw = tabs + (shape ? kTabKbdShort : kTabSineShort);
+                const float *psw = tabs + (prev_shape ? kTabKbdShort : kTabSineShort);
+#pragma unroll 1
+                for (int e = 0; e < 4; ++e) {
+                    const int j0 = 4 * lane + 256 * e;
+                    float nd[4] = {0.0f, 0.0f, 0.0f, 0.0f};
+                    if (j0 < kP1) pcm_short4(ldsf, j0 + kP1, sw, psw, nd);
+                    *reinterpret_cast<float4 *>(my_slot + j0) = make_float4(nd[0], nd[1], nd[2], nd[3]);
+                }
+            }
+        }
+        if constexpr (KIND == kStepHalo) {
+            wave_sync();
+        } else {
+        wg_sync_lds();
+
+        if (active) {
+            float *frame_out = pcm + (chain_base + (size_t)t) * 1024;
+            float dst[2][8];
+            if (seq != EIGHT_SHORT) {
+#pragma unroll
+                for (int h = 0; h < 2; ++h) {
+                    const int m2 = lane + 64 * h;
+                    float dl[8];
+                    load_slot(prev_slot, m2, dl);
+#pragma unroll
+                    for (int q = 0; q < 8; ++q) dst[h][q] = dl[q] + xw[h][q];
+                    if (seq == LONG_STOP) {
+#pragma unroll
+                        for (int q = 0; q < 8; ++q) {
+                            const int j = q < 4 ? 4 * m2 + q : 1020 - 4 * m2 + (q - 4);
+                            dst[h][q] = j < kP0 ? dl[q] : dst[h][q];
+                        }
+                    }
+                }
+            } else {
+                const float *sw = tabs + (shape ? kTabKbdShort : kTabSineShort);
+                const float *psw = tabs + (prev_shape ? kTabKbdShort : kTabSineShort);
+#pragma unroll 1
+                for (int e = 0; e < 4; ++e) {
+                    const int j0 = 4 * lane + 256 * e;
+                    const float4 d = *reinterpret_cast<const float4 *>(prev_slot + j0);
+                    float o[4] = {d.x, d.y, d.z, d.w};
+                    if (j0 >= kP0) {
+                        float ps[4];
+                        pcm_short4(ldsf, j0 - kP0, sw, psw, ps);
+#pragma unroll
+                        for (int q = 0; q < 4; ++q) o[q] = o[q] + ps[q];
+                    }
+                    *reinterpret_cast<float4 *>(prev_slot + j0) = make_float4(o[0], o[1], o[2], o[3]);
+                }
+                wave_sync();
+#pragma unroll
+                for (int h = 0; h < 2; ++h) load_slot(prev_slot, lane + 64 * h, dst[h]);
+            }
+#pragma unroll
+            for (int h = 0; h < 2; ++h) st_slot(frame_out, lane + 64 * h, dst[h]);
+            if constexpr (KIND == kStepFull && !JS) settle_prefetch(line);
+            if (t + 1 == (long)frames_per_chain) {
+                float4 *d = reinterpret_cast<float4 *>(delay_out + (size_t)(ch ? chain1 : chain) * 1024);
+#pragma unroll
+                for (int q = 0; q < 4; ++q) d[lane + 64 * q] = reinterpret_cast<const float4 *>(my_slot)[lane + 64 * q];
+            }
+        }
+        wg_sync_lds();
+        }
+        }
+    };
+
+    if (has_halo && wave == 3) step(step_kind<kStepHalo>{}, -1, t_begin - 1, true);
+    if constexpr (!JS) settle_prefetch(line);
+    const int n_full = (int)((t_end - t_begin) >> 2);
+    long t = t_begin + wave;
+#pragma unroll 1
+    for (int i = 0; i < n_full; ++i, t += 4) step(step_kind<kStepFull>{}, i, t, true);
+    if ((t_end - t_begin) & 3) step(step_kind<kStepRagged>{}, n_full, t, t < t_end);
diff --git a/symphonia_amd/csrc/batch_copy.hip b/symphonia_amd/csrc/batch_copy.hip
--- a/symphonia_amd/csrc/batch_copy.hip
+++ b/symphonia_amd/csrc/batch_copy.hip
@@ -312,3 +312,5 @@
 #include "adpcm.hip"
 
 #include "pcm_decode.hip"
+
+#include "aac_rows.hip"
diff --git a/symphonia_amd/csrc/batcher.cpp b/symphonia_amd/csrc/batcher.cpp
--- a/symphonia_amd/csrc/batcher.cpp
+++ b/symphonia_amd/csrc/batcher.cpp
@@ -230,6 +230,7 @@
     size_t dma_bytes = 0;
     size_t chunk_div = 2;
     size_t chunk_min = (size_t)8192 << 10;
+    unsigned walk_workgroups = kAacRowsWorkgroups;
 };
 
 struct Group {
@@ -249,6 +250,9 @@
     const uint64_t *done_flag = nullptr;
     uint64_t done_seq = 0;
     char *d_in[kMaxIn] = {}, *d_state_in[kMaxState] = {}, *d_state_out[kMaxState] = {}, *d_out = nullptr;
+    bool aac_rows = false, aac_rows_split = false;
+    AacRow *h_rows = nullptr;
+    float *h_delay_in = nullptr;
     size_t row_pitch = 0;
     LaunchKnobs knobs;
     std::vector<VorbisUsed> used;
@@ -442,6 +446,14 @@
     return SYMACCEL_OK;
 }
 
+int check_aac_side(const PlaneSizes &ps, size_t units, const TicketView &v) {
+    const uint8_t *side = v.in<const uint8_t>(1);
+    uint8_t all = 0;
+    for (size_t i = 0, n = (size_t)v.n_chains * units; i < n; ++i) all |= side[i];
+    (void)ps;
+    return (all & 0xf0u) ? SYMACCEL_ERR_INVALID_ARG : SYMACCEL_OK;
+}
+
 int check_mpa12(size_t units, int param, TicketView &v) {
     const size_t rb = symaccel_mpa12_record_bytes(param);
     uint8_t *r = v.in<uint8_t>(1);
@@ -486,6 +498,7 @@
         if (g->kind == SYMACCEL_BATCH_ALAC_PREDICT) v.status = check_alac(g->param, v);
         if (g->kind == SYMACCEL_BATCH_ADPCM_DECODE) v.status = check_adpcm(g->units, g->param, v);
         if (g->kind == SYMACCEL_BATCH_MPA12_DECODE) v.status = check_mpa12(g->units, g->param, v);
+        if (g->kind == SYMACCEL_BATCH_AAC_SYNTH) v.status = check_aac_side(g->ps, g->units, v);
         if (v.status == SYMACCEL_OK) v.status = v.fmt_status;
         if (g->kind == SYMACCEL_BATCH_FLAC_RESTORE && flac_verify_param(g->param).verify && v.status != SYMACCEL_OK) {
             symaccel_md5_state *st = v.state<symaccel_md5_state>(0);
@@ -530,6 +543,15 @@
 void request_block(Group *g, size_t bound, BatchCopyDesc **descs, Carver &dev, Carver &host) {
     const PlaneSizes &ps = g->ps;
     host.want(descs, bound * sizeof(BatchCopyDesc));
+    if (g->aac_rows) {
+        for (int i = 0; i < ps.n_in; ++i) g->d_in[i] = nullptr;
+        g->d_state_in[0] = g->d_state_out[0] = nullptr;
+        g->d_out = nullptr;
+        host.want(&g->h_rows, g->chains * sizeof(AacRow));
+        host.want(&g->h_delay_in, g->aac_rows_split ? g->chains * ps.state[0] : 0);
+        g->mp3.request(dev, host, g->tickets);
+        return;
+    }
     for (int i = 0; i < ps.n_in; ++i) {
         g->d_in[i] = nullptr;
         if (ps.in_host_only[i]) continue;
@@ -583,7 +605,7 @@
     return SYMACCEL_OK;
 }
 
-Chunk next_chunk(const Group *g, size_t t0) {
+Chunk chunk_span(const Group *g, size_t t0) {
     const PlaneSizes &ps = g->ps;
     const size_t per_chain = std::max<size_t>(1, in_bytes_per_chain(ps));
     const size_t chunk_bytes = std::min<size_t>((size_t)32 << 20, std::max<size_t>(g->knobs.chunk_min, g->chains * per_chain / g->knobs.chunk_div));
@@ -594,6 +616,12 @@
     size_t t1 = t0;
     while (t1 < g->tickets && (ch.nc == 0 || ch.nc + g->views[t1].n_chains <= chunk_chains)) ch.nc += g->views[t1++].n_chains;
     ch.nt = t1 - t0;
+    return ch;
+}
+
+Chunk next_chunk(const Group *g, size_t t0) {
+    const PlaneSizes &ps = g->ps;
+    Chunk ch = chunk_span(g, t0);
     for (int i = 0; i < ps.n_in; ++i)
         if (g->d_in[i]) ch.in[i] = g->d_in[i] + (ps.in_per_ticket[i] ? t0 * ps.in[i] : (ch.c0 / ps.in_div[i]) * (i == 0 && g->row_pitch ? g->row_pitch : ps.in[i]));
     for (int i = 0; i < ps.n_state; ++i) {
@@ -753,12 +781,71 @@
     return launch_batch_copy(ctx, s, first, (size_t)(pw.w - first), scatter, pcm_stride, widening);
 }
 
+int launch_aac_rows_group(symaccel_ctx *ctx, Group *g, uint64_t *n_chunks, uint64_t *api_ns, uint64_t *n_allocs) {
+    const PlaneSizes &ps = g->ps;
+    const unsigned wgs = std::max(1u, g->knobs.walk_workgroups);
+    const size_t steps_per_chain = (g->units + 3) / 4;
+    struct Cut {
+        Chunk ch;
+        unsigned seg_steps;
+    };
+    std::vector<Cut> cuts;
+    g->aac_rows_split = false;
+    for (size_t t0 = 0; t0 < g->tickets;) {
+        const Chunk ch = chunk_span(g, t0);
+        size_t live_chains = 0;
+        for (size_t ti = ch.t0; ti < ch.t0 + ch.nt; ++ti) {
+            const TicketView &v = g->views[ti];
+            if (v.status != SYMACCEL_OK) continue;
+            live_chains += v.n_chains;
+        }
+        const unsigned seg_steps = aac_rows_seg_steps(ctx, live_chains, g->units, wgs);
+        g->aac_rows_split |= seg_steps < steps_per_chain;
+        cuts.push_back({ch, seg_steps});
+        t0 += ch.nt;
+    }
+    const size_t bound = piece_bound(g);
+    BatchCopyDesc *descs = nullptr;
+    SYM_TRY(carve_block(ctx, g, bound, &descs, n_allocs));
+    size_t n = 0;
+    for (const Cut &cut : cuts) {
+        const size_t n0 = n;
+        const bool split = cut.seg_steps < steps_per_chain;
+        for (size_t ti = cut.ch.t0; ti < cut.ch.t0 + cut.ch.nt; ++ti) {
+            const TicketView &v = g->views[ti];
+            if (v.status != SYMACCEL_OK) continue;
+            for (size_t c = 0; c < v.n_chains; ++c, ++n) {
+                AacRow &r = g->h_rows[n];
+                float *state = reinterpret_cast<float *>(v.slot + v.lay.state[0] + c * ps.state[0]);
+                r.coeffs = reinterpret_cast<const float *>(v.slot + v.lay.in[0] + c * ps.in[0]);
+                r.side = reinterpret_cast<const uint8_t *>(v.slot + v.lay.in[1] + c * ps.in[1]);
+                r.delay_in = state;
+                if (split) {
+                    float *copy = g->h_delay_in + n * 1024;
+                    std::memcpy(copy, state, ps.state[0]);
+                    r.delay_in = copy;
+                }
+                r.delay_out = state;
+                r.pcm = reinterpret_cast<float *>(v.slot + v.lay.out + c * ps.out);
+            }
+        }
+        const Clock::time_point api0 = Clock::now();
+        SYM_TRY(launch_aac_rows(ctx, ctx->stage_out, g->h_rows + n0, n - n0, g->units, cut.seg_steps, wgs));
+        *api_ns += ns_since(api0);
+        *n_chunks += 1;
+    }
+    return SYMACCEL_OK;
+}
+
 int launch_group_inner(Lane *lane, Group *g, uint64_t *n_chunks, uint64_t *api_ns, uint64_t *n_allocs) {
     symaccel_ctx *ctx = lane->ctx;
     if (!ctx->stage_in) SYM_GPU(ctx, hipStreamCreate(&ctx->stage_in));
     if (!ctx->stage_out) SYM_GPU(ctx, hipStreamCreate(&ctx->stage_out));
     prepare_views(g);
     validate_and_count(g);
+    g->aac_rows = g->kind == SYMACCEL_BATCH_AAC_SYNTH && !g->ps.in_place && aac_rows_available();
+    for (const TicketView &v : g->views) g->aac_rows = g->aac_rows && v.out_fmt == 0;
+    if (g->aac_rows) return launch_aac_rows_group(ctx, g, n_chunks, api_ns, n_allocs);
     const size_t bound = piece_bound(g);
     BatchCopyDesc *descs = nullptr;
     SYM_TRY(carve_block(ctx, g, bound, &descs, n_allocs));
@@ -1063,6 +1150,13 @@
     Locked l(b);
     if (lanes) b->want_lanes = (size_t)lanes;
     if (hint_bytes) b->hint_bytes = hint_bytes;
+    return SYMACCEL_OK;
+}
+
+int symaccel_batcher_set_walk_workgroups(symaccel_batcher *b, int workgroups) {
+    if (!b || workgroups < 0 || workgroups > 4096) return SYMACCEL_ERR_INVALID_ARG;
+    Locked l(b);
+    b->knobs.walk_workgroups = workgroups ? (unsigned)workgroups : kAacRowsWorkgroups;
     return SYMACCEL_OK;
 }
 
diff --git a/symphonia_amd/csrc/ctx.cpp b/symphonia_amd/csrc/ctx.cpp
--- a/symphonia_amd/csrc/ctx.cpp
+++ b/symphonia_amd/csrc/ctx.cpp
@@ -53,13 +53,13 @@
 }
 
 unsigned choose_segment(const symaccel_ctx *ctx, size_t n_chains, size_t frames_per_chain, unsigned waves_per_cu,
-                        unsigned items_per_wave, unsigned halo, unsigned min_seg) {
+                        unsigned items_per_wave, unsigned halo, unsigned min_seg, unsigned capped_slots) {
     if (frames_per_chain == 0) return 1;
     if (ctx->segment > 0) {
         unsigned s = (unsigned)ctx->segment < min_seg ? min_seg : (unsigned)ctx->segment;
         return s > frames_per_chain ? (unsigned)frames_per_chain : s;
     }
-    const double slots = (double)ctx->n_cus * waves_per_cu * items_per_wave;
+    const double slots = capped_slots ? (double)capped_slots : (double)ctx->n_cus * waves_per_cu * items_per_wave;
     const unsigned lo = min_seg, hi = frames_per_chain < 256 ? (unsigned)frames_per_chain : 256u;
     if (hi <= lo) return hi < 1 ? 1 : hi;
     unsigned best = hi;
diff --git a/symphonia_amd/csrc/symaccel_internal.h b/symphonia_amd/csrc/symaccel_internal.h
--- a/symphonia_amd/csrc/symaccel_internal.h
+++ b/symphonia_amd/csrc/symaccel_internal.h
@@ -132,7 +132,7 @@
 int ctx_upload(symaccel_ctx *ctx, const void *src, size_t bytes, const void **out);
 int get_imdct_plan(symaccel_ctx *ctx, int n, double scale, const ImdctPlan **out);
 unsigned choose_segment(const symaccel_ctx *ctx, size_t n_chains, size_t frames_per_chain, unsigned waves_per_cu,
-                        unsigned items_per_wave, unsigned halo, unsigned min_seg);
+                        unsigned items_per_wave, unsigned halo, unsigned min_seg, unsigned capped_slots = 0);
 int get_vorbis_window(symaccel_ctx *ctx, int bs, const float **out);
 
 class DeviceGuard {
@@ -189,6 +189,18 @@
                float *d_delay_out, float *d_pcm, size_t n_chains, size_t frames_per_chain, const AacBandMaps *maps = nullptr,
                const int32_t *d_pair_chains = nullptr, const symaccel_aac_js_frame *d_js_desc = nullptr, size_t n_pairs = 0,
                void *d_js_scratch = nullptr);
+struct AacRow {
+    const float *coeffs;
+    const uint8_t *side;
+    const float *delay_in;
+    float *delay_out;
+    float *pcm;
+};
+constexpr unsigned kAacRowsWorkgroups = 64;
+bool aac_rows_available();
+unsigned aac_rows_seg_steps(const symaccel_ctx *ctx, size_t n_chains, size_t frames_per_chain, unsigned workgroups);
+int launch_aac_rows(symaccel_ctx *ctx, hipStream_t stream, const AacRow *rows, size_t n_chains, size_t frames_per_chain, unsigned seg_steps,
+                    unsigned workgroups);
 inline size_t aac_js_scratch_bytes(size_t n_chains, size_t n_pairs, size_t frames_per_chain) {
     (void)n_pairs;
     (void)frames_per_chain;
```

Result: no change. 337.2 million (-0.2%).
